# praateekmahajan/moving-mnist-vae

Measured on AMD Instinct MI355X. Metric: frames/sec/GPU VAE train step, 20×64×64 batch; ELBO vs CPU ref, higher is better.
Workload: dtype bf16; 1 GPU; BASELINE configs[1]: 256 clips x 20 frames x 64x64 per GPU per step (=5120 frames), conv-VAE z=128, Gaussian NLL sigma=0.1 + KL (normal_vae_1_kl_0_mmd), Adam, random-init weights, Bernoulli(0.0521) q=2 labels; parallelism=dp1, rccl_ranks=1, grad_exchange=none, bn=per-rank batch statistics

## Files before the change

moving-mnist-vae_amd/csrc/capi.cpp:

```cpp
#include <cstring>
#include <new>

#include "../../include/mmvae.h"
#include "conv_ops.hpp"
#include "pixel_net.hpp"
#include "vae_net.hpp"

namespace mmvae { const char* last_error(); }
using namespace mmvae;

struct mmvae_net { Net* net; };
struct mmvae_comm { Comm* c; };

static inline hipStream_t S(void* s) { return static_cast<hipStream_t>(s); }
static inline hipStream_t S_(void* s) { return static_cast<hipStream_t>(s); }

extern "C" {

int mmvae_abi_version(void) { return MMVAE_ABI_VERSION; }
const char* mmvae_last_error(void) { return last_error(); }

int mmvae_net_create(mmvae_net** out, int in_channels, int z, int out_channels, int image_size, int need_logvar, int dtype) {
  return mmvae_net_create_ex(out, in_channels, z, out_channels, image_size, need_logvar, dtype, 1);
}
// ... 187 lines not shown
  return launch_rsample_fwd(DT_F32, mu, lv, eps, enc, nullptr, (long)n, S(st));
}
int mmvae_rsample_bwd(const float* d_enc, const float* lv, const float* eps, float* d_mu, float* d_lv, int64_t n, void* st) {
  return launch_rsample_bwd(d_enc, lv, eps, d_mu, d_lv, (long)n, S(st));
}
static bool aligned16(const void* p) { return reinterpret_cast<uintptr_t>(p) % 16 == 0; }
int mmvae_kl_fwd_ex(const float* mu, const float* lv, int64_t n, double* acc, double* partials, void* st) {
  if (n > 0 && (!mu || !lv || !acc || !partials)) { set_error("kl_fwd: bad argument"); return MMVAE_ERR_ARG; }
  return launch_kl_fwd(mu, lv, (long)n, acc, partials, S(st));
}
int mmvae_kl_fwd(const float* mu, const float* lv, int64_t n, double* acc, void* st) {
  if (n > 0 && (!mu || !lv || !acc)) { set_error("kl_fwd: bad argument"); return MMVAE_ERR_ARG; }
  return launch_kl_fwd(mu, lv, (long)n, acc, nullptr, S(st));
}
int mmvae_kl_bwd(const float* mu, const float* lv, float coef, const float* gscale, float* d_mu, float* d_lv, int64_t n, void* st) {
  return launch_kl_bwd(mu, lv, coef, gscale, d_mu, d_lv, (long)n, S(st));
}
static int gauss_nll_fwd(const float* r, const float* t, int64_t n, float sigma, double* acc, double* partials, bool need_partials, void* st) {
  if (!(sigma > 0.f)) { set_error("gauss_nll: sigma must be > 0"); return MMVAE_ERR_ARG; }
  if (n > 0 && (!r || !t || !acc || (need_partials && !partials))) { set_error("gauss_nll_fwd: bad argument"); return MMVAE_ERR_ARG; }
  if (n > 0 && (!aligned16(r) || !aligned16(t))) { set_error("gauss_nll_fwd: recon and target must be 16-byte aligned"); return MMVAE_ERR_ARG; }
  return launch_gauss_nll_fwd(r, t, (long)n, sigma, acc, partials, S(st));
}
int mmvae_gauss_nll_fwd_ex(const float* r, const float* t, int64_t n, float sigma, double* acc, double* partials, void* st) {
  return gauss_nll_fwd(r, t, n, sigma, acc, partials, true, st);
}
int mmvae_gauss_nll_fwd(const float* r, const float* t, int64_t n, float sigma, double* acc, void* st) {
  return gauss_nll_fwd(r, t, n, sigma, acc, nullptr, false, st);
}
int mmvae_gauss_nll_bwd(const float* r, const float* t, int64_t n, float sigma, float coef, const float* gscale, float* d_r, void* st) {
  if (!(sigma > 0.f)) { set_error("gauss_nll: sigma must be > 0"); return MMVAE_ERR_ARG; }
  return launch_gauss_nll_bwd(r, t, (long)n, sigma, coef, gscale, d_r, S(st));
}
int mmvae_ce_fwd_ex(const float* r, const int64_t* t, const float* w, int N, int Q, int HW, double* acc, double* partials, void* st) {
  if ((long)N * HW > 0 && (!r || !t || !acc || !partials || Q < 1)) { set_error("ce_fwd: bad argument"); return MMVAE_ERR_ARG; }
  return launch_ce_fwd(r, reinterpret_cast<const long long*>(t), w, N, Q, HW, acc, partials, S(st));
}
int mmvae_ce_fwd(const float* r, const int64_t* t, const float* w, int N, int Q, int HW, double* acc, void* st) {
  if ((long)N * HW > 0 && (!r || !t || !acc || Q < 1)) { set_error("ce_fwd: bad argument"); return MMVAE_ERR_ARG; }
  return launch_ce_fwd(r, reinterpret_cast<const long long*>(t), w, N, Q, HW, acc, nullptr, S(st));
}
int mmvae_ce_bwd(const float* r, const int64_t* t, const float* w, int N, int Q, int HW, float coef, const float* gscale, float* d_r,
                 void* st) {
  return launch_ce_bwd(r, reinterpret_cast<const long long*>(t), w, N, Q, HW, coef, gscale, d_r, S(st));
}
static int mmd_fwd(const float* x, const float* y, int n, int d, float* scratch, double* acc, double* partials, bool need_partials, void* st) {
  if (n > 0 && (!x || !y || !acc || (need_partials && !partials) || d < 1)) { set_error("mmd_fwd: bad argument"); return MMVAE_ERR_ARG; }
  if (n > 0 && scratch && (!aligned16(x) || !aligned16(y))) { set_error("mmd_fwd: x and y must be 16-byte aligned"); return MMVAE_ERR_ARG; }
  return scratch ? launch_mmd_fwd_mfma(x, y, n, d, scratch, acc, partials, S(st)) : launch_mmd_fwd(x, y, n, d, acc, partials, S(st));
}
int mmvae_mmd_fwd_ex(const float* x, const float* y, int n, int d, float* scratch, double* acc, double* partials, void* st) {
  return mmd_fwd(x, y, n, d, scratch, acc, partials, true, st);
}
int mmvae_mmd_fwd(const float* x, const float* y, int n, int d, float* scratch, double* acc, void* st) {
  return mmd_fwd(x, y, n, d, scratch, acc, nullptr, false, st);
}
int mmvae_mmd_bwd(const float* x, const float* y, int n, int d, float coef, const float* gscale, float* d_y, void* st) {
  return launch_mmd_bwd(x, y, n, d, coef, gscale, d_y, S(st));
}
int mmvae_rbf_kernel(const float* x, const float* y, int n, int m, int d, float* out, void* st) {
  if (!x || !y || !out) { set_error("rbf_kernel: bad argument"); return MMVAE_ERR_ARG; }
  return launch_rbf_matrix(x, y, n, m, d, out, S(st));
}
int mmvae_loss_finish(const double* acc, float* out, float nll, float kl_coef, float mmd_coef, float n, void* st) {
  return launch_loss_finish(acc, out, nll, kl_coef, mmd_coef, n, S(st));
}

int mmvae_normalise_labels(const int64_t* labels, int64_t n, float mean, float stdv, float* image, void* st) {
  return launch_normalise(DT_F32, labels, 8, (long)n, mean, stdv, nullptr, image, S(st));
}
int mmvae_quantise_normalise(const uint8_t* frames, int64_t n, const float* centres, int q, float mean, float stdv, int64_t* labels,
                             float* image, void* st) {
  return launch_quantise_normalise(frames, (long)n, centres, q, mean, stdv, reinterpret_cast<long long*>(labels), image, S(st));
}
int mmvae_adam_step(float* p, const float* g, float* m, float* v, int64_t n, float lr, float b1, float b2, float eps, float wd, float bc1,
                    float bc2_sqrt, float grad_scale, void* st) {
  AdamArgs a{p, g, m, v, (long)n, lr, b1, b2, eps, wd, bc1, bc2_sqrt, grad_scale};
  return launch_adam(a, S(st));
}

int mmvae_adam_step_dev(float* p, const float* g, float* m, float* v, int64_t n, float lr, float b1, float b2, float eps, float wd,
                        double* step_dev, float grad_scale, void* st) {
  if (!step_dev) { set_error("adam_step_dev: step counter required"); return MMVAE_ERR_ARG; }
  AdamArgs a{p, g, m, v, (long)n, lr, b1, b2, eps, wd, 1.f, 1.f, grad_scale};
  return launch_adam_dev(a, step_dev, S(st));
}

static inline ConvGeom geom_for(int transposed, int Cin, int Cout, int k, int s, int p) {
  return transposed ? ConvGeom{Cin, Cout, k, s, p} : ConvGeom{Cout, Cin, k, s, p};
}
static inline long numel_w(int Cin, int Cout, int k) { return (long)Cin * Cout * k * k; }
static inline int out_size(int transposed, int H, int k, int s, int p) { return transposed ? (H - 1) * s - 2 * p + k : conv_down_size(H, k, s, p); }

int mmvae_conv2d_fwd(int dt, int transposed, const void* x, const float* w, void* y, int N, int H, int W, int Cin, int Cout, int k,
                     int s, int p, const float* ps, const float* pb, int relu, float* stats, void* scratch, void* st) {
  const ConvGeom g = geom_for(transposed, Cin, Cout, k, s, p);
  const int Ho = out_size(transposed, H, k, s, p), Wo = out_size(transposed, W, k, s, p);
  SecondSrc q;
  if (!transposed && conv3_stream_ok(dt, Cin, Cout, k, s, p, H, W)) {
    if (w) { int rc = op_pack_down(dt, g, w, scratch, S(st)); if (rc < 0) return rc; }
    return launch_conv3_stream(dt, s, x, scratch, nullptr, y, nullptr, ps, pb, relu, stats, nullptr, N, Ho, S(st));
  }
  if (!transposed) {
    q.wfrag = op_deep2_down_ok(dt, g, H, W);
    if (w) { int rc = op_pack_down(dt, g, w, scratch, S(st), 1.f, 0, q.wfrag); if (rc < 0) return rc; }
    return op_run_down(dt, dt, g, scratch, N, x, H, W, y, Ho, Wo, ps, pb, relu, stats, 0, S(st), q);
  }
  if (convT4_stream_ok(dt, Cin, Cout, k, s, p, H, W)) {
    if (w) { int rc = op_pack_up(dt, g, w, scratch, S(st)); if (rc < 0) return rc; }
    return launch_convT4_stream(dt, x, scratch, y, ps, pb, relu, stats, N, H, S(st));
  }
  q.wfrag = op_deep2_up_ok(dt, g, Ho, Wo);
  if (w) { int rc = op_pack_up(dt, g, w, scratch, S(st), 1.f, 0, q.wfrag); if (rc < 0) return rc; }
  return op_run_up(dt, g, scratch, N, x, H, W, y, Ho, Wo, ps, pb, relu, stats, 0, S(st), q);
}
int mmvae_conv2d_dgrad(int dt, int transposed, const void* dy, const float* w, void* dx, int N, int H, int W, int Cin, int Cout, int k,
                       int s, int p, void* scratch, void* st) {
  const ConvGeom g = geom_for(transposed, Cin, Cout, k, s, p);
  const int Ho = out_size(transposed, H, k, s, p), Wo = out_size(transposed, W, k, s, p);
  SecondSrc q;
  if (!transposed && s == 1 && conv3_stream_ok(dt, Cin, Cout, k, s, p, H, W)) {
    PackArgs pf; std::memset(&pf, 0, sizeof(pf));
    pf.src = w; pf.dst = scratch; pf.cols = Cin; pf.K = Cout; pf.ntaps = 9; pf.s_col = 9; pf.s_k = Cin * 9; pf.scale = 1.f;
    for (int t = 0; t < 9; ++t) pf.tap_off[t] = 8 - t;
    int rc = launch_pack(dt, pf, S(st)); if (rc < 0) return rc;
    rc = launch_conv3_stream(dt, 1, dy, scratch, nullptr, dx, nullptr, nullptr, nullptr, 0, nullptr, nullptr, N, H, S(st));
    return rc < 0 ? rc : MMVAE_OK;
  }
  if (!transposed) {
    q.wfrag = op_deep2_up_ok(dt, g, H, W);
    int rc = op_pack_up(dt, g, w, scratch, S(st), 1.f, 0, q.wfrag); if (rc < 0) return rc;
    return op_run_up(dt, g, scratch, N, dy, Ho, Wo, dx, H, W, nullptr, nullptr, 0, nullptr, 0, S(st), q);
  }
  q.wfrag = op_deep2_down_ok(dt, g, Ho, Wo);
  int rc = op_pack_down(dt, g, w, scratch, S(st), 1.f, 0, q.wfrag); if (rc < 0) return rc;
  return op_run_down(dt, dt, g, scratch, N, dy, Ho, Wo, dx, H, W, nullptr, nullptr, 0, nullptr, 0, S(st), q);
}
int mmvae_conv2d_wgrad(int dt, int transposed, const void* x, const void* dy, float* dw, int N, int H, int W, int Cin, int Cout, int k,
                       int s, int p, const float* ps, const float* pb, int relu, void* scratch, void* st) {
  const ConvGeom g = geom_for(transposed, Cin, Cout, k, s, p);
  const int Ho = out_size(transposed, H, k, s, p), Wo = out_size(transposed, W, k, s, p);
  if (!scratch) { set_error("conv2d_wgrad: scratch (MMVAE_WGRAD_SCRATCH_BYTES) required"); return MMVAE_ERR_ARG; }
  static_assert(MMVAE_WGRAD_SCRATCH_BYTES == kWgradScratchBytes, "public scratch size out of sync");
  float* sc = static_cast<float*>(scratch);
  if (!transposed) return op_run_wgrad(dt, g, N, dy, Ho, Wo, nullptr, nullptr, 0, x, H, W, ps, pb, relu, dw, S(st), sc);
  return op_run_wgrad(dt, g, N, x, H, W, ps, pb, relu, dy, Ho, Wo, nullptr, nullptr, 0, dw, S(st), sc);
}
int mmvae_conv2d_wgrad_pair(int dt, const void* x, const void* dy, const void* dy_sc, float* dw, float* dw_sc, int N, int H, int W, int Cin, int Cout,
                            const float* ps, const float* pb, int relu, void* scratch, void* st) {
  if (!scratch || !x || !dy || !dy_sc || !dw || !dw_sc || N < 1) { set_error("conv2d_wgrad_pair: bad argument"); return MMVAE_ERR_ARG; }
  const ConvGeom g = geom_for(0, Cin, Cout, 3, 2, 1), gs = geom_for(0, Cin, Cout, 1, 2, 0);
  const int Ho = out_size(0, H, 3, 2, 1), Wo = out_size(0, W, 3, 2, 1);
  const int rc = op_run_wgrad_pair(dt, g, gs, N, dy, dy_sc, Ho, Wo, x, H, W, ps, pb, relu, dw, dw_sc, S(st), static_cast<float*>(scratch), 1.f, 1.f);
  if (rc == 0) { set_error("conv2d_wgrad_pair: shape not supported (bf16, 32 -> 32 channels, 32x32 -> 16x16)"); return MMVAE_ERR_UNSUPPORTED; }
  return rc < 0 ? rc : MMVAE_OK;
}
int mmvae_convT_bwd_fused(int dt, const void* x, const void* dy, const float* w, float* dw, void* dx, int N, int H, int W, int Cin, int Cout, int k,
                          int s, int p, const float* ps, const float* pb, int relu, const void* x2, const float* w2, float* dw2, void* scratch,
                          void* wscratch, void* st) {
  const ConvGeom g = geom_for(1, Cin, Cout, k, s, p);
  const int Ho = out_size(1, H, k, s, p), Wo = out_size(1, W, k, s, p);
  if (!scratch || !wscratch) { set_error("convT_bwd_fused: scratch buffers required"); return MMVAE_ERR_ARG; }
  if (!op_bwd_fusable(dt, g, N, H, W, Ho, Wo)) { set_error("convT_bwd_fused: shape not supported (bf16, 16 / 32 -> 16 channels, k4 s2 p1, 32x32 -> 64x64 or 16x16 -> 32x32)"); return MMVAE_ERR_UNSUPPORTED; }
  char* sc = static_cast<char*>(scratch);
  int rc = op_pack_down(dt, g, w, sc, S(st)); if (rc < 0) return rc;
  const void* w2p = nullptr;
  if (x2 && w2) {
    PackArgs pa; std::memset(&pa, 0, sizeof(pa));
    pa.src = w2; pa.dst = sc + (size_t)Cin * Cout * k * k * dtype_size(dt); pa.cols = Cin; pa.K = 16; pa.ntaps = 1; pa.s_col = 16; pa.s_k = 1; pa.scale = 1.f; pa.tap_off[0] = 0;
    rc = launch_pack(dt, pa, S(st)); if (rc < 0) return rc;
    w2p = pa.dst;
  }
  if (dw2 && !w2p) { set_error("convT_bwd_fused: dw2 needs x2 and w2"); return MMVAE_ERR_ARG; }
  rc = op_run_bwd_fused(dt, g, N, x, H, W, ps, pb, relu, dy, Ho, Wo, sc, dx, w2p ? x2 : nullptr, w2p, dw, S(st), static_cast<float*>(wscratch), 1.f,
                        nullptr, dw2, 1.f);
  if (rc == 0) { set_error("convT_bwd_fused: not taken"); return MMVAE_ERR_UNSUPPORTED; }
  return rc < 0 ? rc : MMVAE_OK;
}
static_assert(MMVAE_BN_SCRATCH_BYTES >= (1024u * 3 * 512 + 8 * 512) * 4, "BatchNorm scratch: 1024 partial rows x 3 x C<=512 + coefficient rows");
int mmvae_batchnorm_fwd(int dt, const void* y, int64_t npix, int C, const float* gamma, const float* beta, float* rm, float* rv, int64_t* nbt,
                        float momentum, float eps, int relu, void* out, float* save_mean, float* save_istd, void* scratch, void* st) {
  if (!scratch || !save_mean || !save_istd || C < 1 || C > 512 || npix < 1) { set_error("batchnorm_fwd: bad arguments (C <= 512, scratch and save_* required)"); return MMVAE_ERR_ARG; }
  float* part = static_cast<float*>(scratch);
  float* coef = part + 1024L * 3 * 512;
  const int np = launch_chan_stats_nhwc(dt, y, npix, C, part, S(st));
  if (np < 0) return np;
  BnFinalizeArgs f;
  f.partials = part; f.nparts = np; f.C = C; f.count = (double)npix; f.gamma = gamma; f.beta = beta; f.running_mean = rm; f.running_var = rv;
  f.nbt = reinterpret_cast<long long*>(nbt); f.mean = save_mean; f.istd = save_istd; f.scale = coef; f.shift = coef + C; f.momentum = momentum; f.eps = eps;
  int rc = launch_bn_finalize(f, S(st));
  if (rc < 0) return rc;
  return launch_affine_act(dt, y, coef, coef + C, relu, out, npix, C, S(st));
}
int mmvae_batchnorm_bwd(int dt, const void* dout, const void* y, const void* out, int64_t npix, int C, const float* gamma, const float* save_mean,
                        const float* save_istd, void* dy, float* dgamma, float* dbeta, void* scratch, void* st) {
  if (!scratch || C < 1 || C > 512 || npix < 1) { set_error("batchnorm_bwd: bad arguments (C <= 512, scratch required)"); return MMVAE_ERR_ARG; }
  float* part = static_cast<float*>(scratch);
  float* coef = part + 1024L * 3 * 512;
  const int np = launch_bn_bwd_reduce(dt, dout, out, nullptr, nullptr, y, nullptr, npix, C, part, S(st));
  if (np < 0) return np;
  BnBwdFinalizeArgs f; std::memset(&f, 0, sizeof(f));
  f.partials = part; f.nparts = np; f.C = C; f.which = 0; f.ny = 1; f.count = (double)npix; f.gamma = gamma; f.mean = save_mean; f.istd = save_istd;
  f.dgamma = dgamma; f.dbeta = dbeta; f.coefA = coef; f.coefB = coef + C; f.coefC = coef + 2 * C;
  int rc = launch_bn_bwd_finalize(f, S(st));
  if (rc < 0) return rc;
  return launch_bn_bwd_apply(dt, dout, out, nullptr, nullptr, y, coef, coef + C, coef + 2 * C, dy, nullptr, nullptr, nullptr, nullptr, nullptr, npix, C, S(st));
}
int mmvae_stem_fwd(int dt, const void* x, const float* w, void* y, int N, int Sz, float* stats, void* scratch, void* st) {
  if (!scratch || N < 1 || Sz < 9 || Sz > 64) { set_error("stem_fwd: bad arguments"); return MMVAE_ERR_ARG; }
  if (stem_fwd_stream_ok(dt, Sz)) return launch_stem_fwd_stream(dt, x, w, y, stats, N, Sz, S(st));
  const int H1 = (Sz + 4 - 5) / 2 + 1;
  const int cpad = dt == DT_F32 ? 4 : 8;
  PackArgs pa; std::memset(&pa, 0, sizeof(pa));
  pa.src = w; pa.dst = scratch;
  pa.cols = 32; pa.K = cpad; pa.K_valid = 1; pa.ntaps = 25; pa.s_col = 25; pa.s_k = 25; pa.scale = 1.f;
  for (int t = 0; t < 25; ++t) pa.tap_off[t] = t;
  int rc = launch_pack(dt, pa, S(st));
  if (rc < 0) return rc;
  GatherArgs a; std::memset(&a, 0, sizeof(a));
  a.x = x; a.w = scratch; a.y = y; a.stats = stats;
  a.x_planar = 2; a.x_planes = 1;
  a.N = N; a.Hi = Sz; a.Wi = Sz; a.Cin = cpad; a.Ho = H1; a.Wo = H1; a.Cout = 32; a.SI = 2; a.SO = 1;
  a.nphase = 1; a.phases[0] = Phase{0, 0, H1, H1, 25, 0, 0};
  for (int kh = 0; kh < 5; ++kh) for (int kw = 0; kw < 5; ++kw) a.taps[kh * 5 + kw] = Tap{kh - 2, kw - 2};
  return launch_gather_gemm(dt, dt, a, S(st));
}
int mmvae_stem_bwd(int dt, const void* g, const void* y0, const void* x, const float* w, const float* gamma, const float* bn_scale,
                   const float* bn_shift, const float* save_mean, const float* save_istd, float* dw, float* dgamma, float* dbeta, int N, int Sz,
                   void* scratch, void* st) {
  if (!scratch || N < 1) { set_error("stem_bwd: bad arguments"); return MMVAE_ERR_ARG; }
  if (!stem_bwd_fusable(Sz)) { set_error("stem_bwd: image size %d unsupported (64, 32, 16)", Sz); return MMVAE_ERR_UNSUPPORTED; }
  const int H1 = (Sz + 4 - 5) / 2 + 1;
  double* R = static_cast<double*>(scratch);
  float* gram = reinterpret_cast<float*>(R + 1024);
  const long gram_floats = 1024L * stem_bwd_part_floats();
  float* part = gram + gram_floats;
  const long part_floats = (long)(MMVAE_BN_SCRATCH_BYTES - 1024 * 8) / 4 - gram_floats;
  int rc = launch_stem_gram(dt, x, gram, gram_floats, R, N, Sz, H1, H1, S(st));
  if (rc < 0) return rc;
  const int np = launch_stem_bwd(dt, g, y0, x, bn_scale, bn_shift, part, part_floats, N, Sz, H1, H1, S(st));
  if (np < 0) return np;
  return launch_stem_bwd_finalize(part, np, R, w, nullptr, (double)N * H1 * H1, gamma, save_mean, save_istd, dgamma, dbeta, dw, S(st));
}
int mmvae_tail_join_fwd(int dt, const void* y2, const float* s2, const float* b2, const void* ys, const float* ss, const float* bs,
                        const float* w, const float* bias, float* r_raw, float* stats, int N, int H, int W, void* st) {
  return launch_tail_join_fwd(dt, y2, s2, b2, ys, ss, bs, w, bias, r_raw, stats, N, H, W, S(st));
}
int mmvae_tail_join_fwd_stream(int dt, const void* y2, const float* s2, const float* b2, const void* ys, const float* ss, const float* bs,
                               const float* w, const float* bias, float* r_raw, float* stats, int N, int H, int W, void* st) {
  return launch_tail_fwd_stream(dt, y2, s2, b2, ys, ss, bs, w, bias, r_raw, stats, N, H, W, S(st));
}
int mmvae_tail_join_bwd_reduce(int dt, const float* d_raw, const float* w, int oc, const void* y2, const float* s2, const float* b2,
                               const void* ys, const float* ss, const float* bs, float* partials, float* wpartials, int N, int H, int W,
                               void* st) {
  return launch_tail_join_bwd_reduce(dt, d_raw, w, oc, N, H, W, s2, b2, ss, bs, y2, ys, partials, S(st), wpartials);
}
int mmvae_tail_join_bwd_apply(int dt, const float* d_raw, const float* w, int oc, const void* y2, const float* s2, const float* b2,
                              const void* ys, const float* ss, const float* bs, const float* A2, const float* B2, const float* C2,
                              const float* As, const float* Bs, const float* Cs, void* dy2, void* dys, int N, int H, int W, void* st) {
  return launch_tail_join_bwd_apply(dt, d_raw, w, oc, N, H, W, s2, b2, ss, bs, y2, A2, B2, C2, dy2, ys, As, Bs, Cs, dys, S(st));
}
int mmvae_upblock_bwd_fused(const float* d_raw, const float* tw, const void* y2, const float* s2, const float* b2, const void* ys, const float* ss,
                            const float* bs, const float* A2, const float* B2, const float* C2, const float* As, const float* Bs, const float* Cs,
                            const void* y1, const float* s1, const float* b1, const float* w2, float* dw2, void* da1, float* bn1_sums,
                            const void* xin, const float* sx, const float* bx, const float* wu, float* dwu, void* gin, int N, void* scratch, void* st) {
  if (!scratch || !d_raw || !tw || !y2 || !ys || !y1 || !xin || !w2 || !wu || !dw2 || !dwu || !da1 || !gin || !bn1_sums || N < 1 || ((sx != nullptr) != (bx != nullptr))) {
    set_error("upblock_bwd_fused: bad argument"); return MMVAE_ERR_ARG;
  }
  char* sc = static_cast<char*>(scratch);
  const ConvGeom g = geom_for(1, 16, 16, 4, 2, 1);
  int rc = op_pack_down(DT_BF16, g, w2, sc, S(st)); if (rc < 0) return rc;
  rc = op_pack_down(DT_BF16, g, wu, sc + 8192, S(st)); if (rc < 0) return rc;
  float* parts = reinterpret_cast<float*>(sc + 16384);
  JoinBwdLaunch L;
  L.d_raw = d_raw; L.w_tail = tw; L.y2 = y2; L.ys = ys; L.ms2 = s2; L.mb2 = b2; L.mss = ss; L.mbs = bs;
  L.A2 = A2; L.B2 = B2; L.C2 = C2; L.As = As; L.Bs = Bs; L.Cs = Cs;
  L.y1 = y1; L.p1s = s1; L.p1b = b1; L.wd2 = sc; L.da1 = da1; L.part2 = parts; L.bn_part = parts + 2L * 1024 * 4096;
  L.xin = xin; L.pxs = sx; L.pxb = bx; L.wds = sc + 8192; L.gin = gin; L.parts = parts + 1024L * 4096;
  L.N = N;
  const int nb = launch_join_bwd_stream(L, S(st));
  if (nb < 0) return nb;
  for (int k = 0; k < 2; ++k) {
    WgradReduceArgs u; std::memset(&u, 0, sizeof(u));
    u.part = k ? L.parts : L.part2; u.dW = k ? dwu : dw2; u.Ca = 16; u.Cb = 16; u.ntaps = 16; u.nparts = nb;
    u.Ca_valid = 16; u.Cb_valid = 16; u.sA = 16 * 16; u.sB = 16; u.scale = 1.f;
    for (int t = 0; t < 16; ++t) u.tap_off[t] = t;
    rc = launch_wgrad_reduce(u, S(st)); if (rc < 0) return rc;
  }
  return launch_partial_rowsum(L.bn_part, nb, 32, bn1_sums, S(st));
}
int mmvae_upblock_tail_fwd(const void* y1, const float* s1, const float* b1, const float* w2, const void* xin, const float* sx, const float* bx,
                           const float* wu, const float* s2, const float* b2, const float* ss, const float* bs, const float* tw, const float* bias,
                           float* r_raw, float* stats, int N, void* scratch, void* st) {
  if (!scratch || !y1 || !s1 || !b1 || !w2 || !xin || !wu || !s2 || !b2 || !ss || !bs || !tw || !r_raw || N < 1 || ((sx != nullptr) != (bx != nullptr))) {
    set_error("upblock_tail_fwd: bad argument"); return MMVAE_ERR_ARG;
  }
  char* sc = static_cast<char*>(scratch);
  const ConvGeom g = geom_for(1, 16, 16, 4, 2, 1);
  int rc = op_pack_up(DT_BF16, g, w2, sc, S(st)); if (rc < 0) return rc;
  rc = op_pack_up(DT_BF16, g, wu, sc + 8192, S(st)); if (rc < 0) return rc;
  return launch_up5_tail_fwd(y1, s1, b1, sc, xin, sx, bx, sc + 8192, s2, b2, ss, bs, tw, bias, r_raw, stats, N, S(st));
}
int mmvae_conv1x1_bwd_fused(const void* da1, const void* y1, const float* s1, const float* b1, const float* A1, const float* B1, const float* C1,
                            const void* xin, const float* sx, const float* bx, const float* w1, float* dw1, void* gin, int64_t rows, void* scratch,
                            void* st) {
  if (!scratch || !da1 || !y1 || !s1 || !b1 || !A1 || !B1 || !C1 || !xin || !w1 || !dw1 || !gin || rows < 1 || ((sx != nullptr) != (bx != nullptr))) {
    set_error("conv1x1_bwd_fused: bad argument"); return MMVAE_ERR_ARG;
// ... 25 lines not shown
```

moving-mnist-vae_amd/csrc/conv_gemm.hip:

```cpp
#include <stdlib.h>
#include <string.h>

#include <vector>

#include "kernels.hpp"

namespace mmvae {

constexpr int KV = 8;

__device__ __forceinline__ int lds_slot(int row, int kv) { return row * KV + (kv ^ ((row >> 1) & 7)); }

template <typename T> struct Mma;
template <> struct Mma<bf16_t> {
  __device__ static __forceinline__ f32x4 run(const Vec16& a, const Vec16& b, f32x4 c) {
    return __builtin_amdgcn_mfma_f32_16x16x32_bf16(__builtin_bit_cast(bf16x8, a), __builtin_bit_cast(bf16x8, b), c, 0, 0, 0);
  }
};
template <> struct Mma<float> {
  __device__ static __forceinline__ f32x4 run(const Vec16& a, const Vec16& b, f32x4 c) {
#pragma unroll
    for (int j = 0; j < 4; ++j)
      c = __builtin_amdgcn_mfma_f32_16x16x4f32(__uint_as_float(a.w[j]), __uint_as_float(b.w[j]), c, 0, 0, 0);
    return c;
// ... 503 lines not shown
  if (out_dt == DT_F32) return launch_gather_t<bf16_t, float>(a, gx, s);
  return launch_gather_t<bf16_t, bf16_t>(a, gx, s);
}

template <typename T>
__global__ __launch_bounds__(256) void wgrad_kernel(WgradArgs a) {
  constexpr int VE = Elem<T>::kVec;
  constexpr int PK = KV * VE;
  __shared__ Vec16 sP[64 * KV];
  __shared__ Vec16 sG[256 * KV];
  __shared__ int sPix[PK * 3];
  __shared__ float sProP[2 * 256];
  __shared__ float sProG[2 * 256];

  const int t = threadIdx.x, lane = t & 63, wv = t >> 6, g = lane >> 4, r = lane & 15;
  const int TA = a.TA16 * 16, TB = a.TB16 * 16, TG = a.TG;
  const int nb_tiles = (a.Cb + TB - 1) / TB;
  const int a0 = (blockIdx.y / nb_tiles) * TA, b0 = (blockIdx.y % nb_tiles) * TB;
  const int tap0 = blockIdx.z * TG;
  const int tg_n = min(TG, a.ntaps - tap0);
  const T* __restrict__ P = reinterpret_cast<const T*>(a.P);
  const T* __restrict__ G = reinterpret_cast<const T*>(a.G);
  T* sPe = reinterpret_cast<T*>(sP);
  T* sGe = reinterpret_cast<T*>(sG);
  const bool proP = a.proP_scale != nullptr, proG = a.proG_scale != nullptr;
  if (proP) for (int i = t; i < TA; i += 256) {
    const bool ok = a0 + i < a.Ca;
    sProP[i] = ok ? a.proP_scale[a0 + i] : 0.f; sProP[256 + i] = ok ? a.proP_shift[a0 + i] : 0.f;
  }
  if (proG) for (int i = t; i < TB; i += 256) {
    const bool ok = b0 + i < a.Cb;
    sProG[i] = ok ? a.proG_scale[b0 + i] : 0.f; sProG[256 + i] = ok ? a.proG_shift[b0 + i] : 0.f;
  }

  const int units = a.TA16 * a.TB16 * tg_n;
  f32x4 acc[16];
  int rowA[16], rowB[16];
#pragma unroll
  for (int i = 0; i < 16; ++i) {
    acc[i] = (f32x4){0, 0, 0, 0};
    const int u = wv + 4 * i;
    const int tg = u % tg_n, q = u / tg_n;
    const int tb = q % a.TB16, ta = q / a.TB16;
    rowA[i] = 16 * ta + r;
    rowB[i] = tg * TB + 16 * tb + r;
  }

  const long m_begin = (long)blockIdx.x * a.pix_per_block;
  const long m_end = min((long)a.M, m_begin + a.pix_per_block);
  const int HpWp = a.Hp * a.Wp;
  const int pvecs = TA / VE, gvecs = TB / VE;

  for (long m0 = m_begin; m0 < m_end; m0 += PK) {
    __syncthreads();
    if (t < PK) {
      const long m = m0 + t;
      if (m < m_end) {
        const int n = (int)(m / HpWp), rem = (int)(m - (long)n * HpWp);
        const int hp = rem / a.Wp, wp = rem - hp * a.Wp;
        sPix[3 * t] = n * a.Hg * a.Wg;
        sPix[3 * t + 1] = hp * a.stride - a.pad;
        sPix[3 * t + 2] = wp * a.stride - a.pad;
      } else {
        sPix[3 * t] = -1; sPix[3 * t + 1] = 0; sPix[3 * t + 2] = 0;
      }
    }
    __syncthreads();
    for (int v = t; v < PK * pvecs; v += 256) {
      const int pk = v / pvecs, cv = v - pk * pvecs;
      const int ch = cv * VE;
      float f[VE];
      const bool ok = (m0 + pk) < m_end && (a0 + ch) < a.Ca;
      if (ok) {
        const Vec16 q = *reinterpret_cast<const Vec16*>(P + ((m0 + pk) * a.Ca + a0 + ch));
        Elem<T>::unpack(q, f);
        if (proP) {
#pragma unroll
          for (int j = 0; j < VE; ++j) {
            float x = f[j] * sProP[ch + j] + sProP[256 + ch + j];
            f[j] = a.proP_relu ? fmaxf(x, 0.f) : x;
          }
        }
      } else {
#pragma unroll
        for (int j = 0; j < VE; ++j) f[j] = 0.f;
      }
#pragma unroll
      for (int j = 0; j < VE; ++j) {
        const int row = ch + j;
        Elem<T>::store(sPe + (long)lds_slot(row, pk / VE) * VE + (pk % VE), f[j]);
      }
    }
    for (int v = t; v < tg_n * PK * gvecs; v += 256) {
      const int tg = v / (PK * gvecs), rem = v - tg * (PK * gvecs);
      const int pk = rem / gvecs, cv = rem - pk * gvecs;
      const int ch = cv * VE;
      const int tap = tap0 + tg, kh = tap / a.ksz, kw = tap - kh * a.ksz;
      const int base = sPix[3 * pk], hg = sPix[3 * pk + 1] + kh, wg = sPix[3 * pk + 2] + kw;
      const bool ok = base >= 0 && hg >= 0 && hg < a.Hg && wg >= 0 && wg < a.Wg && (b0 + ch) < a.Cb;
      float f[VE];
      if (ok) {
        const Vec16 q = *reinterpret_cast<const Vec16*>(G + ((long)(base + hg * a.Wg + wg) * a.Cb + b0 + ch));
        Elem<T>::unpack(q, f);
        if (proG) {
#pragma unroll
          for (int j = 0; j < VE; ++j) {
            float x = f[j] * sProG[ch + j] + sProG[256 + ch + j];
            f[j] = a.proG_relu ? fmaxf(x, 0.f) : x;
          }
        }
      } else {
#pragma unroll
        for (int j = 0; j < VE; ++j) f[j] = 0.f;
      }
#pragma unroll
      for (int j = 0; j < VE; ++j) {
        const int row = tg * TB + ch + j;
        Elem<T>::store(sGe + (long)lds_slot(row, pk / VE) * VE + (pk % VE), f[j]);
      }
    }
    __syncthreads();
#pragma unroll
    for (int i = 0; i < 16; ++i) {
      const int u = wv + 4 * i;
      if (u < units) {
#pragma unroll
        for (int k2 = 0; k2 < 2; ++k2) {
          const int kvs = 4 * k2 + g;
          const Vec16 af = sP[lds_slot(rowA[i], kvs)];
          const Vec16 bf = sG[lds_slot(rowB[i], kvs)];
          acc[i] = Mma<T>::run(af, bf, acc[i]);
        }
      }
    }
  }
#pragma unroll
  for (int i = 0; i < 16; ++i) {
    const int u = wv + 4 * i;
    if (u < units) {
      const int tg = u % tg_n, q = u / tg_n;
      const int tb = q % a.TB16, ta = q / a.TB16;
      const int bb = b0 + 16 * tb + r;
      if (bb < a.Cb_valid) {
#pragma unroll
        for (int j = 0; j < 4; ++j) {
          const int aa = a0 + 16 * ta + 4 * g + j;
          if (aa < a.Ca) a.scratch[(((long)blockIdx.x * a.ntaps + tap0 + tg) * a.Ca + aa) * a.Cb + bb] = acc[i][j];
        }
      }
    }
  }
}

static int try_wgrad2(int dt, const WgradArgs& a, hipStream_t s) {
  if (a.Ca % 16 || a.Cb % 16 || a.ntaps > 25) return 0;
  if (a.proP_scale && a.proG_scale) return 0;
  if (a.P_planar && (a.Ca != 16 || a.P_planes > 16 || a.proP_scale)) return 0;
  auto pick = [](int c) { return c >= 64 ? 64 : c; };
  int TA = pick(a.Ca), TB = pick(a.Cb);
  if (!(TA == 16 || TA == 32 || TA == 64) || !(TB == 16 || TB == 32 || TB == 64)) return 0;
  if (a.Ca % TA || a.Cb % TB) return 0;
  if (a.ntaps < 4 && TB == 64 && !a.P_planar) {
    Wgrad2Args probe; memset(&probe, 0, sizeof(probe));
    probe.TG = wgrad2_taps_per_block(TA / 16, 4, a.ntaps); probe.nw = 4;
    if (make_tile_geom(probe.g, a.N, a.Hp, a.Wp, a.Hg, a.Wg, a.stride, -a.pad, -a.pad, a.ksz, a.ksz, 128, 1) &&
        (wgrad2_lds_bytes(probe, dt, TA, 64) > kV2MaxLds || wgrad2_patch_slots(probe, dt, 64) > 16)) TB = 32;
  }
  const int ta16 = TA / 16, tb16 = TB / 16;
  Wgrad2Args b; memset(&b, 0, sizeof(b));
  b.P = a.P; b.G = a.G;
  b.proP_scale = a.proP_scale; b.proP_shift = a.proP_shift; b.proP_relu = a.proP_relu;
  b.proG_scale = a.proG_scale; b.proG_shift = a.proG_shift; b.proG_relu = a.proG_relu;
  b.TG = wgrad2_taps_per_block(ta16, tb16, a.ntaps);
  b.nw = 4;
  if (!a.P_planar && ta16 >= 2 && tb16 >= 2 && (a.ntaps == 9 || a.ntaps == 16) && b.TG < a.ntaps &&
      !(a.ntaps == 16 && ta16 * tb16 >= 16)) {
    b.nw = a.ntaps; b.TG = a.ntaps;
  } else if (!a.P_planar && a.ntaps == 16 && ta16 == 4 && tb16 == 4) {
    b.nw = 8; b.TG = 16;
  }
  bool fits = false;
  size_t lds = 0;
  for (int TP = 128; TP >= 32 && !fits; TP >>= 1) {
    if (TP < 128 && a.ntaps < 4) break;
    if (!make_tile_geom(b.g, a.N, a.Hp, a.Wp, a.Hg, a.Wg, a.stride, -a.pad, -a.pad, a.ksz, a.ksz, TP, 1)) continue;
    lds = wgrad2_lds_bytes(b, dt, TA, TB);
    fits = lds <= kV2MaxLds && wgrad2_patch_slots(b, dt, TB) <= (b.nw == 4 ? 16 : 8);
  }
  if (!fits) return 0;
  b.Ca = a.Ca; b.Cb = a.Cb; b.Cb_valid = a.Cb_valid; b.Ca_valid = a.Ca_valid; b.ksz = a.ksz; b.ntaps = a.ntaps;
  b.sA = a.sA; b.sB = a.sB; b.scale = a.scale; b.P_planar = a.P_planar; b.P_planes = a.P_planes;
  for (int t = 0; t < 25; ++t) b.tap_off[t] = a.tap_off[t];
  const int tiles_ab = (a.Ca / TA) * (a.Cb / TB);
  const int zg = (a.ntaps + b.TG - 1) / b.TG;
  const long wsize = (long)a.Ca * a.Cb * a.ntaps;
  const long op_bytes = ((long)a.N * a.Hp * a.Wp * a.Ca + (long)a.N * a.Hg * a.Wg * a.Cb) * (long)dtype_size(dt);
  int occ = (int)((160 * 1024) / lds); if (occ > 6) occ = 6; if (occ < 1) occ = 1;
  long gx = (op_bytes < (200L << 20) ? 176L : 256L * occ) / ((long)tiles_ab * zg); if (gx < 1) gx = 1;
  if (!a.scratch) { set_error("wgrad: the partial-image scratch is required (no atomic flush path)"); return MMVAE_ERR_ARG; }
  {
    long budget = op_bytes > (8L << 20) ? op_bytes : (8L << 20);
    if (budget > (long)kWgradScratchBytes) budget = (long)kWgradScratchBytes;
    const long cap = budget / (wsize * 4);
    if (cap < 1) return 0;
    if (gx > cap) gx = cap;
  }
  if (gx > b.g.ntiles) gx = b.g.ntiles;
  if (gx >= 8) gx &= ~7L;
  b.dW = a.scratch; b.partial = 1;
  const int rc = launch_wgrad2(dt, b, (int)gx, tiles_ab, zg, ta16, tb16, s);
  if (rc < 0) return rc;
  WgradReduceArgs u; memset(&u, 0, sizeof(u));
  u.part = a.scratch; u.dW = a.dW; u.Ca = a.Ca; u.Cb = a.Cb; u.ntaps = a.ntaps; u.nparts = (int)gx;
  u.Ca_valid = a.Ca_valid; u.Cb_valid = a.Cb_valid; u.sA = a.sA; u.sB = a.sB; u.scale = a.scale;
  for (int t = 0; t < 25; ++t) u.tap_off[t] = a.tap_off[t];
  const int rc2 = launch_wgrad_reduce(u, s);
  return rc2 < 0 ? rc2 : 1;
}

#define MM_CHECK_RC(expr) do { const int rc__ = (expr); if (rc__ < 0) return rc__; } while (0)
int launch_wgrad(int dt, WgradArgs a, hipStream_t s) {
  const int VE = dt == DT_F32 ? 4 : 8;
  if (a.Ca % VE != 0 || a.Cb % VE != 0 || a.ntaps > 25 || a.ntaps < 1) {
    set_error("wgrad: unsupported Ca=%d Cb=%d ntaps=%d", a.Ca, a.Cb, a.ntaps);
    return MMVAE_ERR_UNSUPPORTED;
  }
  a.M = a.N * a.Hp * a.Wp;
  note_launch_bytes((double)a.N * ((double)a.Hp * a.Wp * (a.P_planar ? a.P_planes * 4.0 : a.Ca * (double)dtype_size(dt)) +
                                   (double)a.Hg * a.Wg * a.Cb * (double)dtype_size(dt)));
  if (a.Cb_valid <= 0 || a.Cb_valid > a.Cb) a.Cb_valid = a.Cb;
  if (a.Ca_valid <= 0 || a.Ca_valid > a.Ca) a.Ca_valid = a.Ca;
  if (a.M <= 0) return MMVAE_OK;
  {
    const int rcs = try_wgrad_stream(dt, a, s);
    if (rcs != 0) return rcs < 0 ? rcs : MMVAE_OK;
    const int rcp = try_wgrad_pos(dt, a, s);
    if (rcp != 0) return rcp < 0 ? rcp : MMVAE_OK;
    const int rc2 = try_wgrad2(dt, a, s);
    if (rc2 != 0) return rc2 < 0 ? rc2 : MMVAE_OK;
    if (a.P_planar) { set_error("wgrad: planar operands need the patch-tile kernel"); return MMVAE_ERR_UNSUPPORTED; }
  }
  const int TA = a.Ca >= 64 ? 64 : ((a.Ca + 15) / 16) * 16;
  const int TB = a.Cb >= 64 ? 64 : ((a.Cb + 15) / 16) * 16;
  a.TA16 = TA / 16; a.TB16 = TB / 16;
  int tg = 256 / TB;
  const int max_units_tg = 64 / (a.TA16 * a.TB16);
  if (tg > max_units_tg) tg = max_units_tg;
  if (tg > a.ntaps) tg = a.ntaps;
  if (tg < 1) tg = 1;
  a.TG = tg;
  const int tiles = ((a.Ca + TA - 1) / TA) * ((a.Cb + TB - 1) / TB);
  const int zg = (a.ntaps + tg - 1) / tg;
  const int PK = KV * VE;
  const long ksteps = ((long)a.M + PK - 1) / PK;
  long want = 1024 / ((long)tiles * zg);
  const long wsize = (long)a.Ca * a.Cb * a.ntaps;
  if (!a.scratch) { set_error("wgrad: the partial-image scratch is required (no atomic flush path)"); return MMVAE_ERR_ARG; }
  {
    long cap = (long)(kWgradScratchBytes / 4) / (wsize > 0 ? wsize : 1);
    const long cap2 = (16L << 20) / (wsize > 0 ? wsize : 1);
    if (cap > cap2 && cap2 >= 8) cap = cap2;
    if (cap < 1) { set_error("wgrad: one partial image (%ld floats) exceeds the scratch", wsize); return MMVAE_ERR_UNSUPPORTED; }
    if (want > cap) want = cap;
  }
  if (want < 1) want = 1;
  if (want > ksteps) want = ksteps;
  long steps_per = (ksteps + want - 1) / want;
  a.pix_per_block = (int)(steps_per * PK);
  const int gx = (int)(((long)a.M + a.pix_per_block - 1) / a.pix_per_block);
  dim3 grid(gx, tiles, zg), block(256);
  if (dt == DT_F32) hipLaunchKernelGGL((wgrad_kernel<float>), grid, block, 0, s, a);
  else hipLaunchKernelGGL((wgrad_kernel<bf16_t>), grid, block, 0, s, a);
  MM_CHECK_RC(check_launch("wgrad"));
  WgradReduceArgs u; memset(&u, 0, sizeof(u));
  u.part = a.scratch; u.dW = a.dW; u.Ca = a.Ca; u.Cb = a.Cb; u.ntaps = a.ntaps; u.nparts = gx;
  u.Ca_valid = a.Ca_valid; u.Cb_valid = a.Cb_valid; u.sA = a.sA; u.sB = a.sB; u.scale = a.scale;
  for (int t = 0; t < 25; ++t) u.tap_off[t] = a.tap_off[t];
  return launch_wgrad_reduce(u, s);
}

template <typename T>
__device__ __forceinline__ long frag_index(int col, int kk, int Ktot) {
  constexpr int VE = Elem<T>::kVec, CK = 4 * VE;
  const int chunk = kk / CK, in = kk - chunk * CK;
  const int q = col & 31;
  const int blk = 2 * (col >> 5) + ((q >> 2) & 1), r = 4 * (q >> 3) + (q & 3);
  return (((long)blk * (Ktot / CK) + chunk) * 64 + (in / VE) * 16 + r) * VE + (in % VE);
}
__device__ __forceinline__ long frag_index_f8(int col, int kk, int Ktot) {
  const int chunk = kk >> 6, in = kk & 63, half = in >> 5, w = in & 31;
  const int q = col & 31;
  const int blk = 2 * (col >> 5) + ((q >> 2) & 1), r = 4 * (q >> 3) + (q & 3);
  return (((long)blk * (Ktot >> 6) + chunk) * 64 + (w >> 3) * 16 + r) * 16 + half * 8 + (w & 7);
}
template <typename T>
__global__ void pack_kernel(PackArgs a) {
  const long total = (long)a.cols * a.ntaps * a.K;
  for (long i = (long)blockIdx.x * blockDim.x + threadIdx.x; i < total; i += (long)gridDim.x * blockDim.x) {
    const int k = (int)(i % a.K);
    const long q = i / a.K;
    const int tp = (int)(q % a.ntaps);
    const int col = (int)(q / a.ntaps);
    const bool real = (a.cols_valid <= 0 || col < a.cols_valid) && (a.K_valid <= 0 || k < a.K_valid);
    const float v = real ? a.src[(long)col * a.s_col + (long)k * a.s_k + a.tap_off[tp]] * a.scale : 0.f;
    Elem<T>::store(reinterpret_cast<T*>(a.dst) + (a.frag ? frag_index<T>(col, tp * a.K + k, a.ntaps * a.K) : i), v);
  }
}

struct PackJob {
  const float* src; void* dst; int cols, K, ntaps, s_col, s_k, cols_valid, K_valid; float scale; unsigned char tap_off[26]; unsigned char frag; unsigned char fp8;
};
__device__ __forceinline__ unsigned char f32_to_e4m3(float v) {
  v = fminf(fmaxf(v, -448.f), 448.f);
  return (unsigned char)(__builtin_amdgcn_cvt_pk_fp8_f32(v, 0.f, 0, false) & 0xff);
}
constexpr int kPackJobsPerLaunch = 48;
struct PackMulti { int njobs; int pad; PackJob jobs[kPackJobsPerLaunch]; };

template <typename T>
__global__ void pack_multi_kernel(PackMulti m) {
  const PackJob& a = m.jobs[blockIdx.y];
  const long total = (long)a.cols * a.ntaps * a.K;
  for (long i = (long)blockIdx.x * blockDim.x + threadIdx.x; i < total; i += (long)gridDim.x * blockDim.x) {
    const int k = (int)(i % a.K);
    const long q = i / a.K;
    const int tp = (int)(q % a.ntaps);
    const int col = (int)(q / a.ntaps);
    const bool real = (a.cols_valid <= 0 || col < a.cols_valid) && (a.K_valid <= 0 || k < a.K_valid);
    const float v = real ? a.src[(long)col * a.s_col + (long)k * a.s_k + a.tap_off[tp]] * a.scale : 0.f;
    if (a.fp8) reinterpret_cast<unsigned char*>(a.dst)[a.frag ? frag_index_f8(col, tp * a.K + k, a.ntaps * a.K) : i] = f32_to_e4m3(v);
    else Elem<T>::store(reinterpret_cast<T*>(a.dst) + (a.frag ? frag_index<T>(col, tp * a.K + k, a.ntaps * a.K) : i), v);
  }
}

static thread_local bool g_pack_batching = false;
static thread_local int g_pack_n = 0;
static thread_local std::vector<PackJob> g_pack_jobs;

void pack_batch_begin() { g_pack_batching = true; g_pack_n = 0; }

int pack_batch_flush(int dt, hipStream_t s) {
  g_pack_batching = false;
  for (int j0 = 0; j0 < g_pack_n; j0 += kPackJobsPerLaunch) {
    PackMulti m; m.njobs = g_pack_n - j0 < kPackJobsPerLaunch ? g_pack_n - j0 : kPackJobsPerLaunch; m.pad = 0;
    for (int j = 0; j < m.njobs; ++j) m.jobs[j] = g_pack_jobs[j0 + j];
    dim3 grid(128, m.njobs), block(256);
    if (dt == DT_F32) hipLaunchKernelGGL((pack_multi_kernel<float>), grid, block, 0, s, m);
    else hipLaunchKernelGGL((pack_multi_kernel<bf16_t>), grid, block, 0, s, m);
    int rc = check_launch("pack_multi");
    if (rc) { g_pack_n = 0; return rc; }
  }
  g_pack_n = 0;
  return MMVAE_OK;
}

int launch_pack(int dt, const PackArgs& a, hipStream_t s) {
  const long total = (long)a.cols * a.ntaps * a.K;
  if (total <= 0) return MMVAE_OK;
  if (g_pack_batching) {
    if (a.ntaps > 26) { set_error("pack: %d taps > 26", a.ntaps); return MMVAE_ERR_ARG; }
    if ((size_t)g_pack_n >= g_pack_jobs.size()) g_pack_jobs.resize(g_pack_jobs.size() + 256);
    PackJob& j = g_pack_jobs[g_pack_n++];
    j.src = a.src; j.dst = a.dst; j.cols = a.cols; j.K = a.K; j.ntaps = a.ntaps; j.s_col = a.s_col; j.s_k = a.s_k;
    j.cols_valid = a.cols_valid; j.K_valid = a.K_valid; j.scale = a.scale; j.fp8 = (unsigned char)(a.fp8 ? 1 : 0); j.frag = (unsigned char)(a.frag ? 1 : 0);
    for (int t = 0; t < a.ntaps; ++t) j.tap_off[t] = (unsigned char)a.tap_off[t];
    return MMVAE_OK;
  }
  if (a.fp8) { set_error("pack: fp8 packing is available in batched mode only"); return MMVAE_ERR_UNSUPPORTED; }
  int blocks = (int)((total + 255) / 256);
  if (blocks > 2048) blocks = 2048;
// ... 7 lines not shown
```

moving-mnist-vae_amd/csrc/conv_ops.cpp:

```cpp
#include "conv_ops.hpp"

#include <cstdlib>
#include <cstring>

namespace mmvae {

#define MM_TRY(expr)            \
  do {                          \
    int rc__ = (expr);          \
    if (rc__ < 0) return rc__;  \
  } while (0)

struct UpPhase { int ph, pw; int ntaps; int kh[16], kw[16], dh[16], dw[16]; };
static int up_phases(int k, int s, int p, UpPhase* out) {
  int n = 0;
  for (int ph = 0; ph < s; ++ph)
    for (int pw = 0; pw < s; ++pw) {
      UpPhase& u = out[n++];
      u.ph = ph; u.pw = pw; u.ntaps = 0;
      for (int kh = 0; kh < k; ++kh) {
        const int th = ph + p - kh;
        if (((th % s) + s) % s != 0) continue;
        for (int kw = 0; kw < k; ++kw) {
          const int tw = pw + p - kw;
          if (((tw % s) + s) % s != 0) continue;
          u.kh[u.ntaps] = kh; u.kw[u.ntaps] = kw;
          u.dh[u.ntaps] = th / s; u.dw[u.ntaps] = tw / s;
          ++u.ntaps;
        }
      }
    }
  return n;
}


int op_pack_down(int dt, const ConvGeom& g, const float* w, void* dst, hipStream_t s, float scale, int fp8, int frag) {
  PackArgs a; std::memset(&a, 0, sizeof(a));
  const int kk = g.k * g.k;
  if (kk > kMaxTaps) { set_error("pack_down: k=%d too large", g.k); return MMVAE_ERR_UNSUPPORTED; }
  a.src = w; a.dst = dst;
  a.cols = g.D0; a.K = g.D1; a.ntaps = kk; a.s_col = g.D1 * kk; a.s_k = kk; a.scale = scale; a.fp8 = fp8; a.frag = frag;
  for (int t = 0; t < kk; ++t) a.tap_off[t] = t;
  return launch_pack(dt, a, s);
}

int op_pack_up(int dt, const ConvGeom& g, const float* w, void* dst, hipStream_t s, float scale, int fp8, int frag) {
  if (g.s > 2 || g.k * g.k > kMaxTaps) { set_error("pack_up: k=%d s=%d unsupported", g.k, g.s); return MMVAE_ERR_UNSUPPORTED; }
  UpPhase ph[4];
  const int np = up_phases(g.k, g.s, g.p, ph);
  const int kk = g.k * g.k;
  const long e = fp8 ? 1 : (long)dtype_size(dt);
  long off = 0;
  for (int i = 0; i < np; ++i) {
    if (ph[i].ntaps == 0) continue;
    PackArgs a; std::memset(&a, 0, sizeof(a));
    a.src = w; a.dst = static_cast<char*>(dst) + off * e;
    a.cols = g.D1; a.K = g.D0; a.ntaps = ph[i].ntaps; a.s_col = kk; a.s_k = g.D1 * kk; a.scale = scale; a.fp8 = fp8; a.frag = frag;
    for (int t = 0; t < ph[i].ntaps; ++t) a.tap_off[t] = ph[i].kh[t] * g.k + ph[i].kw[t];
    MM_TRY(launch_pack(dt, a, s));
    off += (long)g.D1 * ph[i].ntaps * g.D0;
  }
  return MMVAE_OK;
}

int op_deep2_down_ok(int dt, const ConvGeom& g, int Hl, int Wl, int fp8) {
  const int Hs = conv_down_size(Hl, g.k, g.s, g.p), Ws = conv_down_size(Wl, g.k, g.s, g.p);
  return deep2_shape_ok(dt, g.D1, g.D0, Hs, Ws, Hl, Wl, g.k * g.k, fp8) ? 1 : 0;
}
int op_deep2_up_ok(int dt, const ConvGeom& g, int Hl, int Wl, int allow_empty_phases, int fp8) {
  if (g.s > 2 || g.k * g.k > kMaxTaps) return 0;
  const int Hs = conv_down_size(Hl, g.k, g.s, g.p), Ws = conv_down_size(Wl, g.k, g.s, g.p);
  UpPhase ph[4];
  const int np = up_phases(g.k, g.s, g.p, ph);
  int ntaps = 0;
  for (int i = 0; i < np; ++i) { if (ph[i].ntaps == 0 && !allow_empty_phases) return 0; ntaps += ph[i].ntaps; }
  return deep2_shape_ok(dt, g.D0, g.D1, (Hl + g.s - 1) / g.s, (Wl + g.s - 1) / g.s, Hs, Ws, ntaps, fp8) ? 1 : 0;
}
bool op_pos_fwd_takes(const ConvGeom& g, int Hl, bool transposed) {
  const int Hs = conv_down_size(Hl, g.k, g.s, g.p);
  const int Hi = transposed ? Hs : Hl, Ho = transposed ? Hl : Hs;
  const int Cin = transposed ? g.D0 : g.D1, Cout = transposed ? g.D1 : g.D0;
  if (Cout % 32 != 0 || Cin % 8 != 0 || (Hi >= 8 && Cout < 128)) return false;
  if (transposed && g.s > 1 && g.k < g.s) return false;
  const int nw = Cout / 32 < 8 ? Cout / 32 : 8;
  if ((Cout / 32) % nw != 0 || (64 * nw) % (Cin / 8) != 0) return false;
  return pos_conv_takes(g.k, g.s, g.p, transposed ? 1 : 0, Hi, Ho, Cin);
}

int op_run_down(int dt, int out_dt, const ConvGeom& g, const void* packed, int N, const void* L, int Hl, int Wl, void* S, int Hs, int Ws,
                const float* pro_s, const float* pro_b, int relu, float* stats, int accumulate, hipStream_t s, const SecondSrc& x2) {
  GatherArgs a; std::memset(&a, 0, sizeof(a));
  if (g.k * g.k > kMaxTaps) { set_error("run_down: k=%d too large", g.k); return MMVAE_ERR_UNSUPPORTED; }
  if (x2.x2) { a.x2 = x2.x2; a.w2 = x2.w2; a.Cin2 = x2.Cin2; a.x2_ph = 0; a.x2_pw = 0; }
  a.fp8 = x2.fp8; a.wfrag = x2.wfrag; a.wfrag2 = x2.wfrag2;
  a.x = L; a.w = packed; a.y = S;
  a.pro_scale = pro_s; a.pro_shift = pro_b; a.pro_relu = relu; a.stats = stats; a.accumulate = accumulate;
  a.N = N; a.Hi = Hl; a.Wi = Wl; a.Cin = g.D1; a.Ho = Hs; a.Wo = Ws; a.Cout = g.D0; a.SI = g.s; a.SO = 1;
  a.gk = g.k; a.gs = g.s; a.gp = g.p; a.gup = 1;
  a.nphase = 1;
  a.phases[0] = Phase{0, 0, Hs, Ws, g.k * g.k, 0, 0};
  for (int kh = 0; kh < g.k; ++kh)
    for (int kw = 0; kw < g.k; ++kw) a.taps[kh * g.k + kw] = Tap{kh - g.p, kw - g.p};
  return launch_gather_gemm(dt, out_dt, a, s);
}

int op_run_up(int dt, const ConvGeom& g, const void* packed, int N, const void* S, int Hs, int Ws, void* L, int Hl, int Wl,
              const float* pro_s, const float* pro_b, int relu, float* stats, int accumulate, hipStream_t s, const SecondSrc& x2) {
  if (g.s > 2 || g.k * g.k > kMaxTaps) { set_error("run_up: k=%d s=%d unsupported", g.k, g.s); return MMVAE_ERR_UNSUPPORTED; }
  GatherArgs a; std::memset(&a, 0, sizeof(a));
  if (x2.x2) { a.x2 = x2.x2; a.w2 = x2.w2; a.Cin2 = x2.Cin2; a.x2_ph = 0; a.x2_pw = 0; }
  a.fp8 = x2.fp8; a.wfrag = x2.wfrag; a.wfrag2 = x2.wfrag2;
  a.x = S; a.w = packed; a.y = L;
  a.pro_scale = pro_s; a.pro_shift = pro_b; a.pro_relu = relu; a.stats = stats; a.accumulate = accumulate;
  a.N = N; a.Hi = Hs; a.Wi = Ws; a.Cin = g.D0; a.Ho = Hl; a.Wo = Wl; a.Cout = g.D1; a.SI = 1; a.SO = g.s;
  a.gk = g.k; a.gs = g.s; a.gp = g.p; a.gup = 2;
  UpPhase ph[4];
  const int np = up_phases(g.k, g.s, g.p, ph);
  long off = 0; int tap0 = 0; a.nphase = 0;
  for (int i = 0; i < np; ++i) {
    const int Hq = Hl > ph[i].ph ? (Hl - ph[i].ph + g.s - 1) / g.s : 0;
    const int Wq = Wl > ph[i].pw ? (Wl - ph[i].pw + g.s - 1) / g.s : 0;
    const bool skip = (ph[i].ntaps == 0 && accumulate) || Hq == 0 || Wq == 0;
    if (!skip) {
      a.phases[a.nphase++] = Phase{ph[i].ph, ph[i].pw, Hq, Wq, ph[i].ntaps, tap0, off};
      for (int t = 0; t < ph[i].ntaps; ++t) a.taps[tap0 + t] = Tap{ph[i].dh[t], ph[i].dw[t]};
      tap0 += ph[i].ntaps;
    }
    off += (long)g.D1 * ph[i].ntaps * g.D0;
  }
  if (a.nphase == 0) return 1;
  return launch_gather_gemm(dt, dt, a, s);
}

int op_run_wgrad(int dt, const ConvGeom& g, int N, const void* P, int Hs, int Ws, const float* proP_s, const float* proP_b, int proP_relu,
                 const void* G, int Hl, int Wl, const float* proG_s, const float* proG_b, int proG_relu, float* dW, hipStream_t s,
                 float* scratch, float scale, WgradReduceArgs* defer) {
  WgradArgs a; std::memset(&a, 0, sizeof(a));
  const int kk = g.k * g.k;
  if (kk > 25) { set_error("wgrad: k=%d too large", g.k); return MMVAE_ERR_UNSUPPORTED; }
  if (defer) defer->nparts = 0;
  a.P = P; a.G = G; a.dW = dW; a.scratch = scratch; a.defer = defer;
  a.proP_scale = proP_s; a.proP_shift = proP_b; a.proP_relu = proP_relu;
  a.proG_scale = proG_s; a.proG_shift = proG_b; a.proG_relu = proG_relu;
  a.N = N; a.Hp = Hs; a.Wp = Ws; a.Ca = g.D0; a.Hg = Hl; a.Wg = Wl; a.Cb = g.D1; a.Cb_valid = g.D1;
  a.stride = g.s; a.pad = g.p; a.ksz = g.k; a.sA = g.D1 * kk; a.sB = kk; a.ntaps = kk; a.scale = scale;
  for (int t = 0; t < kk; ++t) a.tap_off[t] = t;
  return launch_wgrad(dt, a, s);
}

static void wgrad_args(WgradArgs& a, const ConvGeom& g, int N, const void* P, int Hs, int Ws, const float* proP_s, const float* proP_b, int proP_relu,
                       const void* G, int Hl, int Wl, const float* proG_s, const float* proG_b, int proG_relu, float* dW, float* scratch, float scale) {
  std::memset(&a, 0, sizeof(a));
  const int kk = g.k * g.k;
  a.P = P; a.G = G; a.dW = dW; a.scratch = scratch;
  a.proP_scale = proP_s; a.proP_shift = proP_b; a.proP_relu = proP_relu;
  a.proG_scale = proG_s; a.proG_shift = proG_b; a.proG_relu = proG_relu;
  a.N = N; a.Hp = Hs; a.Wp = Ws; a.Ca = g.D0; a.Hg = Hl; a.Wg = Wl; a.Cb = g.D1; a.Cb_valid = g.D1; a.Ca_valid = g.D0;
  a.stride = g.s; a.pad = g.p; a.ksz = g.k; a.sA = g.D1 * kk; a.sB = kk; a.ntaps = kk; a.scale = scale;
  for (int t = 0; t < kk && t < 25; ++t) a.tap_off[t] = t;
}

int op_run_wgrad_pair(int dt, const ConvGeom& g, const ConvGeom& gs, int N, const void* P, const void* P2, int Hs, int Ws, const void* G, int Hl, int Wl,
                      const float* proG_s, const float* proG_b, int proG_relu, float* dW, float* dW2, hipStream_t s, float* scratch, float scale,
                      float scale2) {
  if (g.k != 3 || g.p != 1 || gs.k != 1 || gs.p != 0 || gs.s != g.s || gs.D0 != g.D0 || gs.D1 != g.D1) return 0;
  WgradArgs a;
  wgrad_args(a, g, N, P, Hs, Ws, nullptr, nullptr, 0, G, Hl, Wl, proG_s, proG_b, proG_relu, dW, scratch, scale);
  return try_wgrad_stream_pair(dt, a, P2, dW2, scale2, s);
}

bool op_wgrad_is_stream(int dt, const ConvGeom& g, int N, int Hs, int Ws, int Hl, int Wl, bool proP, bool proG) {
  if (g.k * g.k > 25) return false;
  WgradArgs a;
  float dummy = 0.f;
  wgrad_args(a, g, N, nullptr, Hs, Ws, proP ? &dummy : nullptr, proP ? &dummy : nullptr, 1, nullptr, Hl, Wl, proG ? &dummy : nullptr, proG ? &dummy : nullptr, 1,
             nullptr, &dummy, 1.f);
  return wgrad_stream_shape(dt, a);
}

bool op_bwd_fusable(int dt, const ConvGeom& g, int N, int Hs, int Ws, int Hl, int Wl) {
  if (g.k * g.k > 25) return false;
  WgradArgs a;
  float dummy = 0.f;
  wgrad_args(a, g, N, nullptr, Hs, Ws, nullptr, nullptr, 0, nullptr, Hl, Wl, nullptr, nullptr, 0, nullptr, &dummy, 1.f);
  return dgrad_wgrad_stream_shape(dt, a);
}

int op_run_bwd_fused(int dt, const ConvGeom& g, int N, const void* P, int Hs, int Ws, const float* proP_s, const float* proP_b, int proP_relu,
                     const void* G, int Hl, int Wl, const void* packed_down, void* dP, const void* x2, const void* w2_packed, float* dW,
                     hipStream_t s, float* scratch, float scale, float* bn_part, float* dW2, float scale2, const JoinGrad* jg) {
  if (g.k * g.k > 25) return 0;
  WgradArgs a;
  wgrad_args(a, g, N, P, Hs, Ws, proP_s, proP_b, proP_relu, G, Hl, Wl, nullptr, nullptr, 0, dW, scratch, scale);
  a.M = a.N * a.Hp * a.Wp;
  return try_dgrad_wgrad_stream(dt, a, packed_down, dP, x2, w2_packed, bn_part, s, dW2, scale2, jg);
}

bool op_bwd_fusable_jg(int dt, const ConvGeom& g, int N, int Hs, int Ws, int Hl, int Wl, bool proP, bool has_x2, bool bn_sums) {
  if (g.k * g.k > 25) return false;
  WgradArgs a;
  float dummy = 0.f;
  wgrad_args(a, g, N, nullptr, Hs, Ws, proP ? &dummy : nullptr, proP ? &dummy : nullptr, 1, nullptr, Hl, Wl, nullptr, nullptr, 0, nullptr, &dummy, 1.f);
  return dgrad_wgrad_stream_jg_shape(dt, a, has_x2, bn_sums);
}

}
```

moving-mnist-vae_amd/csrc/conv_wgrad.hip:

```cpp
#include <cstdlib>
#include "kernels.hpp"

namespace mmvae {

int launch_wgrad2_bf16(const Wgrad2Args& a, dim3 grid, int ta16, int tb16, int maxg, hipStream_t s);
int launch_wgrad2_f32(const Wgrad2Args& a, dim3 grid, int ta16, int tb16, int maxg, hipStream_t s);

int wgrad2_taps_per_block(int ta16, int tb16, int ntaps) {
  int mt = 12 / (ta16 * tb16); if (mt < 1) mt = 1; if (mt > 4) mt = 4;
  const int tg = ntaps >= 4 ? 4 * mt : mt;
  return tg < ntaps ? tg : ntaps;
}

size_t wgrad2_lds_bytes(const Wgrad2Args& a, int dt, int TA, int TB) {
  const size_t es = dtype_size(dt);
  const size_t stage = (size_t)a.g.TP * TA * es + (size_t)a.g.segs * a.g.PR * a.g.PW * TB * es + 32 * 4;
  const size_t acc1 = (size_t)TA * TB * 4;
  return stage > acc1 ? stage : acc1;
}

int wgrad2_patch_slots(const Wgrad2Args& a, int dt, int TB) {
  const int cvg = TB * (int)dtype_size(dt) / 16;
  const int nt = 64 * (a.nw > 0 ? a.nw : 4);
  const int per_round = nt / cvg;
  const int npatch = a.g.segs * a.g.PR * a.g.PW;
  return (npatch + per_round - 1) / per_round;
}

int launch_wgrad2(int dt, const Wgrad2Args& a, int gx, int tiles_ab, int zg, int ta16, int tb16, hipStream_t s) {
  dim3 grid(gx, tiles_ab, zg);
  const int slots = wgrad2_patch_slots(a, dt, tb16 * 16);
  if (slots > 16) { set_error("wgrad2: %d staging slots > 16", slots); return MMVAE_ERR_UNSUPPORTED; }
  return dt == DT_F32 ? launch_wgrad2_f32(a, grid, ta16, tb16, slots, s) : launch_wgrad2_bf16(a, grid, ta16, tb16, slots, s);
}

template <int LANES>
__global__ __launch_bounds__(256) void wgrad_reduce_kernel(WgradReduceArgs a) {
  constexpr int RG = 256 / LANES;
  __shared__ float4 sSum[256];
  const int ab = a.Ca * a.Cb;
  const long wsize = a.part_stride;
  const int l = threadIdx.x % LANES, rg = threadIdx.x / LANES;
  const float* src = a.part + (long)blockIdx.x * (4 * LANES) + l * 4;
  float4 s[4];
#pragma unroll
  for (int k = 0; k < 4; ++k) s[k] = make_float4(0.f, 0.f, 0.f, 0.f);
  int p = rg;
  for (; p + 3 * RG < a.nparts; p += 4 * RG) {
#pragma unroll
    for (int k = 0; k < 4; ++k) {
      const float4 v = *reinterpret_cast<const float4*>(src + (long)(p + k * RG) * wsize);
      s[k].x += v.x; s[k].y += v.y; s[k].z += v.z; s[k].w += v.w;
    }
  }
  for (; p < a.nparts; p += RG) {
    const float4 v = *reinterpret_cast<const float4*>(src + (long)p * wsize);
    s[0].x += v.x; s[0].y += v.y; s[0].z += v.z; s[0].w += v.w;
  }
  sSum[threadIdx.x] = make_float4((s[0].x + s[1].x) + (s[2].x + s[3].x), (s[0].y + s[1].y) + (s[2].y + s[3].y),
                                  (s[0].z + s[1].z) + (s[2].z + s[3].z), (s[0].w + s[1].w) + (s[2].w + s[3].w));
  __syncthreads();
#pragma unroll
  for (int st = RG / 2; st >= 1; st >>= 1) {
    if (rg < st) {
      const float4 o = sSum[threadIdx.x + st * LANES];
      float4& m = sSum[threadIdx.x];
      m.x += o.x; m.y += o.y; m.z += o.z; m.w += o.w;
    }
    __syncthreads();
  }
  if (rg == 0) {
    const float4 m = sSum[l];
    const float v[4] = {m.x, m.y, m.z, m.w};
#pragma unroll
    for (int j = 0; j < 4; ++j) {
      const long i = (long)blockIdx.x * (4 * LANES) + l * 4 + j;
      const int t = (int)(i / ab), rem = (int)(i - (long)t * ab);
      const int aa = rem / a.Cb, bb = rem - aa * a.Cb;
      if (aa < a.Ca_valid && bb < a.Cb_valid) a.dW[(long)aa * a.sA + (long)bb * a.sB + a.tap_off[t]] += v[j] * a.scale;
    }
  }
}

int launch_wgrad_reduce(WgradReduceArgs a, hipStream_t s) {
  if (a.nparts < 1) return MMVAE_OK;
  bool distinct = true;
  for (int t = 0; t < a.ntaps && distinct; ++t)
    for (int u = 0; u < t; ++u) if (a.tap_off[u] == a.tap_off[t]) { distinct = false; break; }
  if (a.part_stride <= 0) a.part_stride = (long)a.ntaps * a.Ca * a.Cb;
  if (!distinct) {
    for (int t = 1; t < a.ntaps; ++t)
      if (a.tap_off[t] != a.tap_off[0]) { set_error("wgrad_reduce: taps share some destinations but not all"); return MMVAE_ERR_UNSUPPORTED; }
    if (a.part_stride != (long)a.ntaps * a.Ca * a.Cb) { set_error("wgrad_reduce: shared destinations need densely packed partial images"); return MMVAE_ERR_UNSUPPORTED; }
    a.nparts *= a.ntaps; a.ntaps = 1; a.part_stride = (long)a.Ca * a.Cb;
  }
  const long wsize = (long)a.ntaps * a.Ca * a.Cb;
  if (wsize % 256) { set_error("wgrad_reduce: %ld elements not a multiple of 256", wsize); return MMVAE_ERR_ARG; }
  a.exclusive = 1;
  note_launch_bytes((double)a.nparts * a.part_stride * 4.0);
  int lanes = 64;
  while (lanes > 8 && wsize / (4 * lanes) < 256) lanes >>= 1;
  const dim3 grid((unsigned)(wsize / (4 * lanes)));
  switch (lanes) {
    case 64: hipLaunchKernelGGL(wgrad_reduce_kernel<64>, grid, dim3(256), 0, s, a); break;
    case 32: hipLaunchKernelGGL(wgrad_reduce_kernel<32>, grid, dim3(256), 0, s, a); break;
    case 16: hipLaunchKernelGGL(wgrad_reduce_kernel<16>, grid, dim3(256), 0, s, a); break;
    default: hipLaunchKernelGGL(wgrad_reduce_kernel<8>, grid, dim3(256), 0, s, a); break;
  }
  return check_launch("wgrad_reduce");
}

int launch_patch_conv_f32(const PatchArgs& a, int gx, hipStream_t s);
int launch_patch_conv_bf16(const PatchArgs& a, int gx, hipStream_t s);
int launch_patch_conv_bf16_f32(const PatchArgs& a, int gx, hipStream_t s);

size_t patch_conv_lds_bytes(const PatchArgs& a, int dt) {
  const int VE = dt == DT_F32 ? 4 : 8;
  const int cin_vecs = a.Cin / VE;
  int ct16 = (a.Cout + 15) / 16; if (ct16 == 3) ct16 = 4;
  size_t b = (size_t)a.w_vecs * 16 + (size_t)a.g.segs * a.g.PR * a.g.PW * cin_vecs * 16 + (size_t)a.koff_total * 4 + (size_t)8 * ct16 * 16 * 4 +
             (a.uni ? (size_t)4 * a.out_wave_bytes : 0);
  b = (b + 15) & ~(size_t)15;
  if (a.x2) b += (size_t)ct16 * 16 * (a.kvp2 + 1) * 16 + ((size_t)a.g.segs * a.g.qr * a.g.Wq * (a.Cin2 / VE) + 8) * 16;
  return b;
}
void patch_conv_x2_carve(PatchArgs& a, int dt) {
  PatchArgs z = a; z.x2 = nullptr;
  const size_t base = patch_conv_lds_bytes(z, dt);
  int ct16 = (a.Cout + 15) / 16; if (ct16 == 3) ct16 = 4;
  a.w2_vec0 = (int)(base / 16);
  a.x2_vec0 = a.w2_vec0 + ct16 * 16 * (a.kvp2 + 1);
}

int patch_conv_slots(const PatchArgs& a, int dt) {
  const int VE = dt == DT_F32 ? 4 : 8;
  const int npatch = a.g.segs * a.g.PR * a.g.PW;
  const int per_round = a.x_planar ? 256 : 256 / (a.Cin / VE);
  return (npatch + per_round - 1) / per_round;
}

int launch_patch_conv(int dt, int out_dt, const PatchArgs& a, int gx, hipStream_t s) {
  if (dt == DT_F32) return launch_patch_conv_f32(a, gx, s);
  if (out_dt == DT_F32) return launch_patch_conv_bf16_f32(a, gx, s);
  return launch_patch_conv_bf16(a, gx, s);
}

int launch_deep2_conv_f32(const DeepArgs& a, int gx, hipStream_t s);
int launch_deep2_conv_bf16(const DeepArgs& a, int gx, hipStream_t s);
int launch_deep2_conv_bf16_f32(const DeepArgs& a, int gx, hipStream_t s);

size_t deep2_conv_lds_bytes(const DeepArgs& a, int dt) {
  const size_t pitch = a.fp8 ? (size_t)a.Cin + 16 : (size_t)a.Cin * dtype_size(dt) + 32;
  return (size_t)(a.ipt * a.Hi * a.Wi + 1) * pitch + (size_t)a.npt * 16 * 4 + (size_t)a.nw * 64 * 4 + (size_t)a.ntaps_all * a.npt * 16 * 2;
}

int launch_deep2_conv(int dt, int out_dt, const DeepArgs& a, int gx, hipStream_t s) {
  if (dt == DT_F32) return launch_deep2_conv_f32(a, gx, s);
  if (out_dt == DT_F32) return launch_deep2_conv_bf16_f32(a, gx, s);
  return launch_deep2_conv_bf16(a, gx, s);
}

}
```

moving-mnist-vae_amd/csrc/conv_wgrad.inc:

```

namespace mmvae {

template <int TA16, int TB16> struct Wgrad2Cfg {
  static constexpr int kUnits = TA16 * TB16;
  static constexpr int kMaxT = (12 / kUnits) < 1 ? 1 : ((12 / kUnits) > 4 ? 4 : (12 / kUnits));
};

constexpr int kSlotInvalid = 0x40000000;

template <typename T, int VE>
__device__ __forceinline__ Vec16 apply_pro(const Vec16& q, const float* sc, const float* sh, int relu) {
  float f[VE];
  Elem<T>::unpack(q, f);
#pragma unroll
  for (int j = 0; j < VE; ++j) {
    const float x = f[j] * sc[j] + sh[j];
    f[j] = relu ? fmaxf(x, 0.f) : x;
  }
  return Elem<T>::pack(f);
}

template <typename T, int TA16, int TB16, bool TS, int MAXG, bool PPL, int NW = 4>
__global__ __launch_bounds__(64 * NW, NW == 16 ? 4 : (NW == 9 ? 3 : (NW == 8 ? 2 : (MAXG <= 8 ? 3 : 2) - (TA16 * TB16 > 2 ? 1 : 0)))) void wgrad2_kernel(Wgrad2Args a) {
  static_assert(NW == 4 || TS, "one-tap-per-wave blocks are tap-split");
  constexpr int NT = 64 * NW;
  constexpr int VE = Elem<T>::kVec;
  constexpr int ES = sizeof(T);
  constexpr int TA = TA16 * 16, TB = TB16 * 16;
  constexpr int MAXT = NW > 4 ? (NW == 8 ? 2 : 1) : Wgrad2Cfg<TA16, TB16>::kMaxT;
  constexpr int NKS = TS ? 4 : 1;
  constexpr int CVG = TB / VE, PSG = NT / CVG;
  constexpr int CVP = TA / VE, PSP = NT / CVP;
  constexpr int MAXP = (128 + PSP - 1) / PSP;
  extern __shared__ __attribute__((aligned(16))) char smem[];
  const TileGeom g = a.g;
  const int t = threadIdx.x, lane = t & 63, wv = t >> 6, gq = lane >> 4, r = lane & 15;
  const int nb_tiles = a.Cb / TB;
  const int a0 = (blockIdx.y / nb_tiles) * TA, b0 = (blockIdx.y % nb_tiles) * TB;
  const int tap0 = blockIdx.z * a.TG;
  const int tg_n = min(a.TG, a.ntaps - tap0);
  const int npatch = g.segs * g.PR * g.PW;
  char* sP = smem;
  char* sG = sP + g.TP * TA * ES;
  int* sToff = reinterpret_cast<int*>(sG + npatch * TB * ES);
  const T* __restrict__ Pp = reinterpret_cast<const T*>(a.P);
  const T* __restrict__ Gp = reinterpret_cast<const T*>(a.G);
  const bool proP = a.proP_scale != nullptr, proG = a.proG_scale != nullptr;
  const bool multi = g.tiles_per_img == 0;
  if (t < tg_n) {
    const int tap = tap0 + t, kh = tap / a.ksz, kw = tap - kh * a.ksz;
    sToff[t] = (kh * g.PW + kw) * TB * ES;
  }
  const int cvp = t % CVP, pp0 = t / CVP, cvg = t % CVG, gp0 = t / CVG;
  float xsc[VE], xsh[VE];
#pragma unroll
  for (int j = 0; j < VE; ++j) {
    xsc[j] = proP ? a.proP_scale[a0 + cvp * VE + j] : (proG ? a.proG_scale[b0 + cvg * VE + j] : 1.f);
    xsh[j] = proP ? a.proP_shift[a0 + cvp * VE + j] : (proG ? a.proG_shift[b0 + cvg * VE + j] : 0.f);
  }
  int goff[MAXG], gchk[MAXG];
#pragma unroll
  for (int k = 0; k < MAXG; ++k) {
    const int pp = gp0 + k * PSG;
    goff[k] = 0; gchk[k] = kSlotInvalid;
    if (pp < npatch) {
      const int row = pp / g.PW, pc = pp - row * g.PW;
      const int seg = row / g.PR, pr = row - seg * g.PR;
      const int wi = g.ow + pc;
      bool ok = wi >= 0 && wi < g.Wi;
      if (multi) ok = ok && g.oh + pr >= 0 && g.oh + pr < g.Hi;
      goff[k] = ((seg * g.Hi + pr) * g.Wi + wi) * a.Cb + b0 + cvg * VE;
      if (ok) gchk[k] = multi ? seg : pr;
    }
  }
  const unsigned lim = multi ? g.N : g.Hi;
  f32x4 acc[MAXT][TA16][TB16];
#pragma unroll
  for (int tl = 0; tl < MAXT; ++tl)
#pragma unroll
    for (int ta = 0; ta < TA16; ++ta)
#pragma unroll
      for (int tb = 0; tb < TB16; ++tb) acc[tl][ta][tb] = (f32x4){0, 0, 0, 0};
  const int npix_tile = g.segs * g.qr * g.Wq;
  int offP[NKS][2], offG[NKS][2];
  if constexpr (sizeof(T) == 2) {
#pragma unroll
    for (int i = 0; i < NKS; ++i)
#pragma unroll
      for (int b = 0; b < 2; ++b) {
        int p = 32 * (TS ? i : wv) + 16 * b + 4 * gq + (r >> 2);
        offP[i][b] = p * TA * ES + (r & 3) * 8;
        if (p >= npix_tile) p = 0;
        offG[i][b] = patch_index(g, p) * TB * ES + (r & 3) * 8;
      }
  }
  int my_tap[MAXT];
#pragma unroll
  for (int tl = 0; tl < MAXT; ++tl) my_tap[tl] = TS ? wv + NW * tl : tl;

  Vec16 gv[MAXG], pv[MAXP];
  int tb_c = 0, nv_c = 0;
  long m0_c = 0;
  const long pplane = (long)g.Hq * g.Wq;
  auto issue = [&](int tile) {
    int n, hq0;
    tile_origin(g, tile, 0, n, hq0);
    const long m0 = ((long)n * g.Hq + hq0) * g.Wq;
    const long mend = !multi ? ((long)n * g.Hq + min(g.Hq, hq0 + g.qr)) * g.Wq : (long)min(g.N, n + g.segs) * g.Hq * g.Wq;
    nv_c = (int)(mend - m0);
    const int h_base = hq0 * g.SI + g.oh;
    tb_c = multi ? n : h_base;
    const T* gsrc = Gp + ((long)n * g.Hi + h_base) * g.Wi * a.Cb;
#pragma unroll
    for (int k = 0; k < MAXG; ++k) {
      gv[k] = Vec16{{0, 0, 0, 0}};
      if ((unsigned)(tb_c + gchk[k]) < lim) gv[k] = *reinterpret_cast<const Vec16*>(gsrc + goff[k]);
    }
    if constexpr (!PPL) {
      const T* psrc = Pp + m0 * a.Ca + a0 + cvp * VE;
#pragma unroll
      for (int k = 0; k < MAXP; ++k) {
        const int pix = pp0 + k * PSP;
        pv[k] = Vec16{{0, 0, 0, 0}};
        if (pix < nv_c) pv[k] = *reinterpret_cast<const Vec16*>(psrc + (long)pix * a.Ca);
      }
    } else {
      m0_c = m0;
#pragma unroll
      for (int k = 0; k < MAXP; ++k) {
        const int pix = pp0 + k * PSP;
        pv[k] = Vec16{{0, 0, 0, 0}};
        if (pix < nv_c && cvp == 0 && a.P_planes <= 2) {
          long nn = n, rem = (long)hq0 * g.Wq + pix;
          if (multi) { const long m = m0 + pix; nn = m / pplane; rem = m - nn * pplane; }
          const float* src = reinterpret_cast<const float*>(a.P) + nn * a.P_planes * pplane + rem;
          pv[k].w[0] = __float_as_uint(src[0]);
          if (a.P_planes > 1) pv[k].w[1] = __float_as_uint(src[pplane]);
        }
      }
    }
  };
  auto commit = [&]() {
#pragma unroll
    for (int k = 0; k < MAXG; ++k) {
      const int pp = gp0 + k * PSG;
      if (pp < npatch) {
        Vec16 q = gv[k];
        if (proG && (unsigned)(tb_c + gchk[k]) < lim) q = apply_pro<T, VE>(q, xsc, xsh, a.proG_relu);
        reinterpret_cast<Vec16*>(sG)[pp * CVG + cvg] = q;
      }
    }
#pragma unroll
    for (int k = 0; k < MAXP; ++k) {
      const int pix = pp0 + k * PSP;
      if (pix < g.TP) {
        Vec16 q = pv[k];
        if constexpr (PPL) {
          float f[VE];
#pragma unroll
          for (int j = 0; j < VE; ++j) f[j] = 0.f;
          if (pix < nv_c && cvp * VE < a.P_planes) {
            if (a.P_planes <= 2) { f[0] = __uint_as_float(q.w[0]); f[1] = __uint_as_float(q.w[1]); }
            else {
              const long m = m0_c + pix, nn = m / pplane, rem = m - nn * pplane;
              const float* src = reinterpret_cast<const float*>(a.P) + nn * a.P_planes * pplane + rem;
#pragma unroll
              for (int j = 0; j < VE; ++j) if (cvp * VE + j < a.P_planes) f[j] = src[(long)(cvp * VE + j) * pplane];
            }
          }
          q = Elem<T>::pack(f);
        } else { if (proP && pix < nv_c) q = apply_pro<T, VE>(q, xsc, xsh, a.proP_relu); }
        reinterpret_cast<Vec16*>(sP)[pix * CVP + cvp] = q;
      }
    }
  };

  const int nks_tile = g.TP >> 5;
#pragma unroll
  for (int j = 0; j < VE; ++j) {
    asm volatile("" ::"v"(xsc[j])); asm volatile("" ::"v"(xsh[j]));
  }
  const TileWalk walk = xcd_tile_walk(g.ntiles);
  int tile = walk.first;
  if (tile < walk.end) issue(tile);
  for (; tile < walk.end; tile += walk.step) {
    __syncthreads();
    commit();
    __syncthreads();
    if (tile + walk.step < walk.end) issue(tile + walk.step);
    if constexpr (sizeof(T) == 2) {
#pragma unroll
      for (int i = 0; i < NKS; ++i) {
        if (TS && i >= nks_tile) break;
        Vec16 af[TA16];
#pragma unroll
        for (int ta = 0; ta < TA16; ++ta) af[ta] = FragOps<bf16_t>::load(sP, offP[i][0] + ta * 32, offP[i][1] + ta * 32);
#pragma unroll
        for (int tl = 0; tl < MAXT; ++tl) {
          if (my_tap[tl] < tg_n) {
            const int toff = sToff[my_tap[tl]];
#pragma unroll
            for (int tb = 0; tb < TB16; ++tb) {
              const Vec16 bf = FragOps<bf16_t>::load(sG, offG[i][0] + toff + tb * 32, offG[i][1] + toff + tb * 32);
#pragma unroll
              for (int ta = 0; ta < TA16; ++ta) acc[tl][ta][tb] = mma_bf16(af[ta], bf, acc[tl][ta][tb]);
            }
          }
        }
      }
    } else {
      for (int i = 0; i < NKS; ++i) {
        if (TS && i >= nks_tile) break;
        const int ks = TS ? i : wv;
        for (int j = 0; j < 8; ++j) {
          int p = 32 * ks + 4 * j + gq;
          const int oP = p * TA * ES + r * 4;
          if (p >= npix_tile) p = 0;
          const int oG = patch_index(g, p) * TB * ES + r * 4;
          float av[TA16];
#pragma unroll
          for (int ta = 0; ta < TA16; ++ta) av[ta] = *reinterpret_cast<const float*>(sP + oP + ta * 64);
#pragma unroll
          for (int tl = 0; tl < MAXT; ++tl) {
            if (my_tap[tl] < tg_n) {
              const int toff = sToff[my_tap[tl]];
#pragma unroll
              for (int tb = 0; tb < TB16; ++tb) {
                const float bv = *reinterpret_cast<const float*>(sG + oG + toff + tb * 64);
#pragma unroll
                for (int ta = 0; ta < TA16; ++ta)
                  acc[tl][ta][tb] = __builtin_amdgcn_mfma_f32_16x16x4f32(av[ta], bv, acc[tl][ta][tb], 0, 0, 0);
              }
            }
          }
        }
      }
    }
  }
  if (TS && a.partial) {
#pragma unroll
    for (int tl = 0; tl < MAXT; ++tl) {
      if (my_tap[tl] < tg_n) {
        float* dst = a.dW + (((long)blockIdx.x * a.ntaps + tap0 + my_tap[tl]) * a.Ca + a0) * a.Cb + b0;
#pragma unroll
        for (int ta = 0; ta < TA16; ++ta)
#pragma unroll
          for (int tb = 0; tb < TB16; ++tb)
#pragma unroll
            for (int jj = 0; jj < 4; ++jj) dst[(long)(16 * ta + 4 * gq + jj) * a.Cb + 16 * tb + r] = acc[tl][ta][tb][jj];
      }
    }
    return;
  }
  __syncthreads();
  float* sAcc = reinterpret_cast<float*>(smem);
#pragma unroll
  for (int tl = 0; tl < MAXT; ++tl) {
    for (int w = 0; w < (TS ? NW : 1); ++w) {
      const int tap_l = TS ? w + NW * tl : tl;
      if (tap_l >= tg_n) continue;
      for (int src = 0; src < (TS ? 1 : NW); ++src) {
        if (TS ? (wv == w) : (wv == src)) {
#pragma unroll
          for (int ta = 0; ta < TA16; ++ta)
#pragma unroll
            for (int tb = 0; tb < TB16; ++tb)
#pragma unroll
              for (int jj = 0; jj < 4; ++jj) {
                float* q = &sAcc[(16 * ta + 4 * gq + jj) * TB + 16 * tb + r];
                *q = (src == 0 ? 0.f : *q) + acc[tl][ta][tb][jj];
              }
        }
        __syncthreads();
      }
      float* dst = a.dW + (((long)blockIdx.x * a.ntaps + tap0 + tap_l) * a.Ca + a0) * a.Cb + b0;
      for (int i = t; i < TA * TB; i += NT) dst[(long)(i / TB) * a.Cb + (i % TB)] = sAcc[i];
      __syncthreads();
    }
  }
}

template <typename T>
static int launch_wgrad2_t(Wgrad2Args a, int dt, dim3 grid, int ta16, int tb16, int maxg, hipStream_t s) {
  const size_t lds = wgrad2_lds_bytes(a, dt, ta16 * 16, tb16 * 16);
  dim3 block(64 * a.nw);
  const bool ts = a.ntaps >= 4;
  if (a.nw != 4) {
    if (a.nw == 8) {
      if (ta16 != 4 || tb16 != 4 || a.P_planar || !ts || maxg > 8) { set_error("wgrad2: nw=8 needs the 64x64 tile"); return MMVAE_ERR_UNSUPPORTED; }
      if (maxg <= 4) hipLaunchKernelGGL((wgrad2_kernel<T, 4, 4, true, 4, false, 8>), grid, block, lds, s, a);
      else hipLaunchKernelGGL((wgrad2_kernel<T, 4, 4, true, 8, false, 8>), grid, block, lds, s, a);
      return check_launch("wgrad2");
    }
    if (a.P_planar || !ts || maxg > 8 || (a.nw != 9 && a.nw != 16)) { set_error("wgrad2: nw=%d unsupported here", a.nw); return MMVAE_ERR_UNSUPPORTED; }
#define MMVAE_W2N(A_, B_) do { \
    if (a.nw == 9) { if (maxg <= 4) hipLaunchKernelGGL((wgrad2_kernel<T, A_, B_, true, 4, false, 9>), grid, block, lds, s, a); \
                     else hipLaunchKernelGGL((wgrad2_kernel<T, A_, B_, true, 8, false, 9>), grid, block, lds, s, a); } \
    else { if (maxg <= 4) hipLaunchKernelGGL((wgrad2_kernel<T, A_, B_, true, 4, false, 16>), grid, block, lds, s, a); \
           else hipLaunchKernelGGL((wgrad2_kernel<T, A_, B_, true, 8, false, 16>), grid, block, lds, s, a); } } while (0)
    if (ta16 == 4 && tb16 == 4) MMVAE_W2N(4, 4);
    else if (ta16 == 4 && tb16 == 2) MMVAE_W2N(4, 2);
    else if (ta16 == 2 && tb16 == 4) MMVAE_W2N(2, 4);
    else if (ta16 == 2 && tb16 == 2) MMVAE_W2N(2, 2);
    else { set_error("wgrad2: tile %dx%d unsupported with nw=%d", ta16, tb16, a.nw); return MMVAE_ERR_UNSUPPORTED; }
#undef MMVAE_W2N
    return check_launch("wgrad2");
  }
#define MMVAE_W2G(A_, B_, G_) do { if (ts) hipLaunchKernelGGL((wgrad2_kernel<T, A_, B_, true, G_, false>), grid, block, lds, s, a); \
                                   else hipLaunchKernelGGL((wgrad2_kernel<T, A_, B_, false, G_, false>), grid, block, lds, s, a); } while (0)
#define MMVAE_W2(A_, B_) do { if (maxg <= 8) MMVAE_W2G(A_, B_, 8); else MMVAE_W2G(A_, B_, 16); } while (0)
  if (a.P_planar) {
    if (ta16 != 1 || tb16 != 1 || !ts) { set_error("wgrad2: planar P needs the 16x16 tap-split tile"); return MMVAE_ERR_UNSUPPORTED; }
    if (maxg <= 8) hipLaunchKernelGGL((wgrad2_kernel<T, 1, 1, true, 8, true>), grid, block, lds, s, a);
    else hipLaunchKernelGGL((wgrad2_kernel<T, 1, 1, true, 16, true>), grid, block, lds, s, a);
  } else if (ta16 == 1 && tb16 == 1) MMVAE_W2(1, 1);
  else if (ta16 == 1 && tb16 == 2) MMVAE_W2(1, 2);
  else if (ta16 == 2 && tb16 == 1) MMVAE_W2(2, 1);
  else if (ta16 == 2 && tb16 == 2) MMVAE_W2(2, 2);
  else if (ta16 == 4 && tb16 == 2) MMVAE_W2(4, 2);
  else if (ta16 == 2 && tb16 == 4) MMVAE_W2(2, 4);
  else if (ta16 == 4 && tb16 == 4) MMVAE_W2(4, 4);
  else if (ta16 == 4 && tb16 == 1) MMVAE_W2(4, 1);
  else if (ta16 == 1 && tb16 == 4) MMVAE_W2(1, 4);
  else { set_error("wgrad2: tile %dx%d unsupported", ta16, tb16); return MMVAE_ERR_UNSUPPORTED; }
#undef MMVAE_W2
#undef MMVAE_W2G
  return check_launch("wgrad2");
}

}
```

moving-mnist-vae_amd/csrc/conv_wpos.hip:

```cpp
#include <cstdlib>
#include <cstring>

#include "kernels.hpp"
#include "tile_common.hpp"

namespace mmvae {

typedef __attribute__((ext_vector_type(16))) float f32x16;

struct WposArgs {
  const void* P; const void* G; float* part;
  const float* proP_scale; const float* proP_shift; int proP_relu;
  const float* proG_scale; const float* proG_shift; int proG_relu;
  int N, Ca, Cb, HS, HL, K, S, Pd;
  int nsplit, imgs_per_split;
  int nb, prow, grow;
};

template <int KI, int NTHR, int kMaxV, int NFB>
__global__ __launch_bounds__(NTHR, 1) void wgrad_pos_kernel(WposArgs a) {
  extern __shared__ __attribute__((aligned(16))) char smem[];
  constexpr int nthr = NTHR;
  constexpr int TB = 32 * NFB, PXG = TB * 2, VG = TB / 8;
  const int t = threadIdx.x, lane = t & 63, wv = __builtin_amdgcn_readfirstlane(t >> 6);
  const int npos = a.HS * a.HS, npix = a.HL * a.HL;
  const int nPb = a.prow * a.HS, nGb = a.grow * a.HL;
  const int ipP = ((nPb * 128 + 191) & ~255) + 64, ipG = ((nGb * PXG + 191) & ~255) + 64;
  const int stageB = KI * (ipP + ipG);
  const int tiles_b = a.Cb / TB;
  const int a0 = (blockIdx.y / tiles_b) << 6, b0 = (blockIdx.y % tiles_b) * TB;
  const int n_begin = blockIdx.x * a.imgs_per_split;
  const int n_end = min(a.N, n_begin + a.imgs_per_split);
  const bf16_t* __restrict__ Pp = reinterpret_cast<const bf16_t*>(a.P);
  const bf16_t* __restrict__ Gp = reinterpret_cast<const bf16_t*>(a.G);
  const int kh = wv / a.K, kw = wv - kh * a.K;
  auto win0 = [&](int band) {
    int g = band * a.prow * a.S - a.Pd;
    g = g < 0 ? 0 : g;
    return g > a.HL - a.grow ? a.HL - a.grow : g;
  };

  const int slots = nPb * 8 + nGb * VG;
  const int ipr = nthr / slots;
  const bool active = t < ipr * slots;
  const int img_r = t / slots, rem = t - img_r * slots;
  const bool isP = rem < nPb * 8;
  const int px = isP ? rem >> 3 : (rem - nPb * 8) / VG, cg = isP ? rem & 7 : (rem - nPb * 8) % VG;
  const bool pro = isP ? a.proP_scale != nullptr : a.proG_scale != nullptr;
  float* sPro = reinterpret_cast<float*>(smem + 2 * stageB);
  if (t < 128) {
    const bool p = a.proP_scale != nullptr;
    const int c = t & 63, nc = p ? 64 : TB;
    const float* sc = p ? a.proP_scale + a0 : a.proG_scale ? a.proG_scale + b0 : nullptr;
    const float* sh = p ? a.proP_shift + a0 : a.proG_scale ? a.proG_shift + b0 : nullptr;
    sPro[t] = (!sc || c >= nc) ? (t < 64 ? 1.f : 0.f) : t < 64 ? sc[c] : sh[c];
  }
  const float lo = (isP ? a.proP_relu : a.proG_relu) ? 0.f : -__builtin_inff();
  const long istride = isP ? (long)npos * a.Ca : (long)npix * a.Cb;
  const bf16_t* src0 = isP ? Pp + (long)px * a.Ca + a0 + cg * 8 : Gp + (long)px * a.Cb + b0 + cg * 8;
  const int ip_t = isP ? ipP : ipG;
  const int dst0 = (isP ? 0 : KI * ipP) + img_r * ip_t + px * (isP ? 128 : PXG) + cg * 16;
  Vec16 q[kMaxV];
  auto fetch = [&](int n0, int band) {
    const long boff = isP ? (long)band * nPb * a.Ca : (long)win0(band) * a.HL * a.Cb;
#pragma unroll
    for (int k = 0; k < kMaxV; ++k) {
      const int img = k * ipr + img_r;
      q[k] = Vec16{{0, 0, 0, 0}};
      if (active && img < KI && n0 + img < n_end) {
        q[k] = *reinterpret_cast<const Vec16*>(src0 + (long)(n0 + img) * istride + boff);
        if (pro) {
          float f[8];
          Elem<bf16_t>::unpack(q[k], f);
          const float4 s0 = *reinterpret_cast<const float4*>(sPro + cg * 8), s1 = *reinterpret_cast<const float4*>(sPro + cg * 8 + 4);
          const float4 h0 = *reinterpret_cast<const float4*>(sPro + 64 + cg * 8), h1 = *reinterpret_cast<const float4*>(sPro + 64 + cg * 8 + 4);
          const float sc[8] = {s0.x, s0.y, s0.z, s0.w, s1.x, s1.y, s1.z, s1.w}, sh[8] = {h0.x, h0.y, h0.z, h0.w, h1.x, h1.y, h1.z, h1.w};
#pragma unroll
          for (int j = 0; j < 8; ++j) f[j] = fmaxf(f[j] * sc[j] + sh[j], lo);
          q[k] = Elem<bf16_t>::pack(f);
        }
      }
    }
  };
  auto commit = [&](char* buf) {
#pragma unroll
    for (int k = 0; k < kMaxV; ++k)
      if (active && k * ipr + img_r < KI) *reinterpret_cast<Vec16*>(buf + dst0 + k * ipr * ip_t) = q[k];
  };

  f32x16 acc[2][NFB];
#pragma unroll
  for (int i = 0; i < 2; ++i)
#pragma unroll
    for (int j = 0; j < NFB; ++j)
#pragma unroll
      for (int e = 0; e < 16; ++e) acc[i][j][e] = 0.f;

  const int li = lane & 15;
  const int lrow = ((lane >> 5) << 3) + (li >> 2);
  const int lcol = (((lane >> 4) & 1) << 5) + ((li & 3) << 3);
  __syncthreads();
  const int nchunk = (n_end - n_begin + KI - 1) / KI, nstage = nchunk * a.nb;
  fetch(n_begin, 0);
  commit(smem);
  __syncthreads();
  int cur = 0, band = 0, n0 = n_begin;
  for (int st = 0; st < nstage; ++st) {
    int bn = band + 1, nn = n0;
    if (bn == a.nb) { bn = 0; nn = n0 + KI; }
    const bool more = st + 1 < nstage;
    if (more) fetch(nn, bn);
    const char* sP = smem + cur * stageB;
    const char* sG = sP + KI * ipP;
    const int g0 = win0(band);
    for (int hr = 0; hr < a.prow; ++hr) {
      const int hs = band * a.prow + hr;
      const int hl = hs * a.S - a.Pd + kh;
      if (hl < g0 || hl >= g0 + a.grow || hl < 0 || hl >= a.HL) continue;
      for (int ws = 0; ws < a.HS; ++ws) {
        const int wl = ws * a.S - a.Pd + kw;
        if (wl < 0 || wl >= a.HL) continue;
        const char* pb = sP + (hr * a.HS + ws) * 128 + lcol;
        const char* gb = sG + ((hl - g0) * a.HL + wl) * PXG + lcol;
#pragma unroll
        for (int ks = 0; ks < KI / 16; ++ks) {
          bf16x8 fa[2], fb[NFB];
          typedef __attribute__((ext_vector_type(8))) short s16x8;
#pragma unroll
          for (int f = 0; f < 2; ++f) {
            const char* pa = pb + (ks * 16 + lrow) * ipP + f * 64;
            const s16x4 a_lo = __builtin_amdgcn_ds_read_tr16_b64_v4i16((__attribute__((address_space(3))) s16x4*)(pa));
            const s16x4 a_hi = __builtin_amdgcn_ds_read_tr16_b64_v4i16((__attribute__((address_space(3))) s16x4*)(pa + 4 * ipP));
            fa[f] = __builtin_bit_cast(bf16x8, (s16x8)__builtin_shufflevector(a_lo, a_hi, 0, 1, 2, 3, 4, 5, 6, 7));
          }
#pragma unroll
          for (int f = 0; f < NFB; ++f) {
            const char* pg = gb + (ks * 16 + lrow) * ipG + f * 64;
            const s16x4 g_lo = __builtin_amdgcn_ds_read_tr16_b64_v4i16((__attribute__((address_space(3))) s16x4*)(pg));
            const s16x4 g_hi = __builtin_amdgcn_ds_read_tr16_b64_v4i16((__attribute__((address_space(3))) s16x4*)(pg + 4 * ipG));
            fb[f] = __builtin_bit_cast(bf16x8, (s16x8)__builtin_shufflevector(g_lo, g_hi, 0, 1, 2, 3, 4, 5, 6, 7));
          }
#pragma unroll
          for (int i = 0; i < 2; ++i)
#pragma unroll
            for (int j = 0; j < NFB; ++j) acc[i][j] = __builtin_amdgcn_mfma_f32_32x32x16_bf16(fa[i], fb[j], acc[i][j], 0, 0, 0);
        }
      }
    }
    if (more) commit(smem + (cur ^ 1) * stageB);
    __syncthreads();
    cur ^= 1; band = bn; n0 = nn;
  }
  const int ntaps = a.K * a.K;
  float* out = a.part + (((long)blockIdx.x * ntaps + wv) * a.Ca + a0) * a.Cb + b0;
#pragma unroll
  for (int i = 0; i < 2; ++i)
#pragma unroll
    for (int j = 0; j < NFB; ++j)
#pragma unroll
      for (int v = 0; v < 16; ++v) {
        const int row = 32 * i + 8 * (v >> 2) + 4 * (lane >> 5) + (v & 3), col = 32 * j + (lane & 31);
        out[(long)row * a.Cb + col] = acc[i][j][v];
      }
}

int try_wgrad_pos(int dt, const WgradArgs& a, hipStream_t s) {
  if (dt != DT_BF16 || a.P_planar || !a.scratch || (a.proP_scale && a.proG_scale)) return 0;
  if (a.Hp != a.Wp || a.Hg != a.Wg || a.Hp < 1 || a.Hp > 4 || a.Hg > 8 || a.Ca % 64 != 0 || a.Cb % 32 != 0) return 0;
  if (a.ksz < 1 || a.ksz > 4 || a.ntaps != a.ksz * a.ksz || a.ksz * a.ksz < 4) return 0;
  if ((a.Ca_valid && a.Ca_valid != a.Ca) || (a.Cb_valid && a.Cb_valid != a.Cb)) return 0;
  for (int t = 0; t < a.ntaps; ++t) if (a.tap_off[t] != t) return 0;
  const int npos = a.Hp * a.Hp, npix = a.Hg * a.Hg;
  if (npos + npix < 8) return 0;
  const int nthr = 64 * a.ntaps;
  const int nfb = (a.Cb % 64 == 0 && (a.Ca / 64) * (a.Cb / 64) >= 8) ? 2 : 1;
  const int TB = 32 * nfb, VG = TB / 8;
  const int tiles = (a.Ca / 64) * (a.Cb / TB);
  int KI = 16, nb = 0, prow = 0, grow = 0, rounds = 0;
  size_t stageB = 0;
  const int maxv = nthr == 1024 ? 4 : 8;
  for (int cand = 1; cand <= a.Hp && !nb; cand *= 2) {
    if (a.Hp % cand) continue;
    const int pr = a.Hp / cand;
    int gr = (pr - 1) * a.stride + a.ksz; if (gr > a.Hg) gr = a.Hg;
    const int nPb = pr * a.Hp, nGb = gr * a.Hg;
    const int ipP = ((nPb * 128 + 191) & ~255) + 64, ipG = ((nGb * TB * 2 + 191) & ~255) + 64;
    const int slots = nPb * 8 + nGb * VG;
    const int ipr = nthr / slots;
    if (ipr < 1) continue;
    for (int ki = (cand == 1 && npos + npix <= 8) ? 32 : 16; ki >= 16; ki -= 16) {
      const size_t sb = (size_t)ki * (ipP + ipG);
      const int rd = (ki + ipr - 1) / ipr;
      if (2 * sb + 512 <= 160 * 1024 && rd <= maxv) { KI = ki; nb = cand; prow = pr; grow = gr; stageB = sb; rounds = rd; break; }
    }
  }
  if (!nb) return 0;
  WposArgs b; std::memset(&b, 0, sizeof(b));
  b.P = a.P; b.G = a.G; b.part = a.scratch;
  b.proP_scale = a.proP_scale; b.proP_shift = a.proP_shift; b.proP_relu = a.proP_relu;
  b.proG_scale = a.proG_scale; b.proG_shift = a.proG_shift; b.proG_relu = a.proG_relu;
  b.N = a.N; b.Ca = a.Ca; b.Cb = a.Cb; b.HS = a.Hp; b.HL = a.Hg; b.K = a.ksz; b.S = a.stride; b.Pd = a.pad;
  b.nb = nb; b.prow = prow; b.grow = grow;
  const long wsize = (long)a.Ca * a.Cb * a.ntaps;
  int nsplit = (256 + tiles - 1) / tiles;
  const int max_split = wsize * 4 * 64 <= (32L << 20) ? 64 : 32;
  if (nsplit > max_split) nsplit = max_split;
  const long cap = (long)(kWgradScratchBytes / 4) / wsize;
  if (cap < 1) return 0;
  if (nsplit > cap) nsplit = (int)cap;
  int per = (a.N + nsplit - 1) / nsplit;
  per = ((per + KI - 1) / KI) * KI;
  if (per < 2 * KI) per = 2 * KI;
  nsplit = (a.N + per - 1) / per;
  b.nsplit = nsplit; b.imgs_per_split = per;
  const size_t lds = 2 * stageB + 512;
  dim3 grid(nsplit, tiles), block(nthr);
  bool launched = false;
#define MMVAE_WPOS(KI_, NT_, MV_, NF_) \
  if (!launched && KI == KI_ && nthr == NT_ && nfb == NF_ && (MV_ == 8 || rounds <= 4)) { \
    static bool attr_set = false; \
    if (!attr_set) { \
      if (hipFuncSetAttribute(reinterpret_cast<const void*>(&wgrad_pos_kernel<KI_, NT_, MV_, NF_>), hipFuncAttributeMaxDynamicSharedMemorySize, 160 * 1024) != hipSuccess) { \
        set_error("wgrad_pos: hipFuncSetAttribute"); return MMVAE_ERR_HIP; } \
      attr_set = true; } \
    hipLaunchKernelGGL((wgrad_pos_kernel<KI_, NT_, MV_, NF_>), grid, block, lds, s, b); launched = true; }
  MMVAE_WPOS(32, 256, 8, 2) MMVAE_WPOS(32, 576, 4, 2) MMVAE_WPOS(32, 576, 8, 2) MMVAE_WPOS(32, 1024, 4, 2)
  MMVAE_WPOS(16, 256, 8, 2) MMVAE_WPOS(16, 576, 4, 2) MMVAE_WPOS(16, 576, 8, 2) MMVAE_WPOS(16, 1024, 4, 2)
  MMVAE_WPOS(16, 256, 8, 1) MMVAE_WPOS(16, 576, 4, 1) MMVAE_WPOS(16, 576, 8, 1) MMVAE_WPOS(16, 1024, 4, 1)
#undef MMVAE_WPOS
  if (!launched) return 0;
  const int rc = check_launch("wgrad_pos");
  if (rc) return rc;
  WgradReduceArgs u; std::memset(&u, 0, sizeof(u));
  u.part = a.scratch; u.dW = a.dW; u.Ca = a.Ca; u.Cb = a.Cb; u.ntaps = a.ntaps; u.nparts = nsplit;
  u.Ca_valid = a.Ca; u.Cb_valid = a.Cb; u.sA = a.sA; u.sB = a.sB; u.scale = a.scale;
  for (int t = 0; t < 25; ++t) u.tap_off[t] = a.tap_off[t];
  const int rr = launch_wgrad_reduce(u, s);
  return rr < 0 ? rr : 1;
}

}
```

moving-mnist-vae_amd/csrc/conv_wstream.hip:

```cpp
#include <hip/hip_runtime.h>

#include <stdlib.h>
#include <string.h>

#include "kernels.hpp"
#include "tile_common.hpp"

namespace mmvae {

struct WStreamArgs {
  const void* P; const void* G; float* part;
  const float* proP_scale; const float* proP_shift; int proP_relu;
  const float* proG_scale; const float* proG_shift; int proG_relu;
  int N, Hp, Hg, Wg;
  int HS;
  int nunits;
  const void* wd;
  void* dx;
  const void* x2; const void* w2;
  float* bn_part;
  const void* P2;
  const void* Jy; const float* jA; const float* jB; const float* jC;
};

// ... 359 lines not shown
        for (int ca = 0; ca < CA16; ++ca)
#pragma unroll
          for (int cb = 0; cb < CB16; ++cb)
#pragma unroll
            for (int j = 0; j < 4; ++j) {
              float* p = img + (k * CA + ca * 16 + 4 * gq + j) * CB + cb * 16 + r;
              *p = (w == 0 ? 0.f : *p) + acc[k][ca][cb][j];
            }
      if constexpr (X2) {
#pragma unroll
        for (int ca = 0; ca < CA16; ++ca)
#pragma unroll
          for (int j = 0; j < 4; ++j) {
            float* p = img + NT * CA * CB + (4 * gq + j) * CA + ca * 16 + r;
            *p = (w == 0 ? 0.f : *p) + acc2[ca][j];
          }
      }
      if constexpr (P2) {
#pragma unroll
        for (int ca = 0; ca < CA16; ++ca)
#pragma unroll
          for (int cb = 0; cb < CB16; ++cb)
#pragma unroll
            for (int j = 0; j < 4; ++j) {
              float* p = img + (NT * CA + ca * 16 + 4 * gq + j) * CB + cb * 16 + r;
              *p = (w == 0 ? 0.f : *p) + accD[ca][cb][j];
            }
      }
    }
    __syncthreads();
  }
  if constexpr (ST) {
    float* sb = img + WSIZE;
#pragma unroll
    for (int j = 0; j < 4; ++j) { bs0[j] = row16_sum(bs0[j]); bs1[j] = row16_sum(bs1[j]); }
    if (r == 0) {
#pragma unroll
      for (int j = 0; j < 4; ++j) { sb[wv * 32 + 4 * gq + j] = bs0[j]; sb[wv * 32 + 16 + 4 * gq + j] = bs1[j]; }
    }
    __syncthreads();
    if (t < 32) {
      float sum = sb[t];
      for (int w = 1; w < NW; ++w) sum += sb[w * 32 + t];
      a.bn_part[(long)blockIdx.x * 32 + t] = sum;
    }
  }
  float* dst = a.part + (long)blockIdx.x * WSIZE;
  for (int i = t; i < WSIZE / 4; i += 64 * NW) reinterpret_cast<float4*>(dst)[i] = reinterpret_cast<const float4*>(img)[i];
}

template <int KS, int S, int PAD, int WP, int CA16, int CB16, bool PRO_P, bool PRO_G, bool DG, bool X2, bool ST = false, int NW = 4, bool P2 = false, bool JG = false>
static int launch_wstream_t(const WStreamArgs& a, int gx, hipStream_t s) {
  constexpr int RP = 32 / WP;
  constexpr int WL = S * (WP - 1) + KS;
  constexpr int NSLOT = S * (RP - 1) + KS + S * RP;
  constexpr size_t rings = NW * (size_t)(NSLOT * WL * CB16 * 32 + 32 * CA16 * 32 + (X2 ? 32 * 32 : 0) + (ST ? 32 * CA16 * 32 : 0) + (P2 ? 32 * CA16 * 32 : 0)) +
                           ((DG && CA16 > 1) ? CA16 * (KS * KS / 2) * 1024 : 0) + (JG ? 3 * CB16 * 16 * 4 : 0) + ((PRO_G && P2) ? 2 * CB16 * 16 * 4 : 0);
  constexpr size_t flush = ((size_t)KS * KS * CA16 * 16 * CB16 * 16 + (X2 ? 16 * CA16 * 16 : 0) + (P2 ? CA16 * 16 * CB16 * 16 : 0)) * 4 + 512;
  constexpr size_t lds = rings > flush ? rings : flush;
  static_assert(lds <= 160 * 1024, "one block must fit the CU's LDS");
  auto kern = &wgrad_stream_kernel<KS, S, PAD, WP, CA16, CB16, PRO_P, PRO_G, DG, X2, ST, NW, P2, JG>;
  static bool attr_set = false;
  if (!attr_set) {
    const hipError_t e = hipFuncSetAttribute(reinterpret_cast<const void*>(kern), hipFuncAttributeMaxDynamicSharedMemorySize, 160 * 1024);
    if (e != hipSuccess) { set_error("wgrad_stream: hipFuncSetAttribute: %s", hipGetErrorString(e)); return MMVAE_ERR_HIP; }
    attr_set = true;
  }
  hipLaunchKernelGGL(kern, dim3(gx), dim3(64 * NW), lds, s, a);
  return check_launch("wgrad_stream");
}

static int wstream_kind(int dt, const WgradArgs& a) {
  if (dt != DT_BF16 || a.P_planar || !a.scratch) return 0;
  if (a.ntaps != a.ksz * a.ksz || a.Cb_valid != a.Cb || a.Ca_valid != a.Ca) return 0;
  for (int t = 0; t < a.ntaps; ++t) if (a.tap_off[t] != t) return 0;
  if (a.Wg != a.stride * a.Wp || a.Hg != a.stride * a.Hp || a.Hp != a.Wp) return 0;
  if (a.ksz == 4 && a.stride == 2 && a.pad == 1 && a.Cb == 16 && (a.Ca == 16 || a.Ca == 32)) return a.Wp == 32 ? 1 : (a.Wp == 16 ? 2 : 0);
  if (a.ksz == 3 && a.pad == 1 && a.Wp == 16 && a.Ca == 32 && a.Cb == 32 && !(a.proP_scale && a.proG_scale)) return a.stride == 1 ? 3 : (a.stride == 2 ? 4 : 0);
  return 0;
}
static int wstream_fill(const WgradArgs& a, WStreamArgs& b, int kind, bool x2 = false, bool p2 = false) {
  memset(&b, 0, sizeof(b));
  b.P = a.P; b.G = a.G; b.part = a.scratch;
  b.proP_scale = a.proP_scale; b.proP_shift = a.proP_shift; b.proP_relu = a.proP_relu;
  b.proG_scale = a.proG_scale; b.proG_shift = a.proG_shift; b.proG_relu = a.proG_relu;
  b.N = a.N; b.Hp = a.Hp; b.Hg = a.Hg; b.Wg = a.Wg;
  b.HS = a.Hp % 16 == 0 ? 16 : a.Hp;
  b.nunits = a.N * (a.Hp / b.HS);
  const int nw = kind == 4 ? 2 : 4;
  int gx = kind == 4 ? 768 : 512;
  while (gx > 8 && (long)gx * nw > b.nunits) gx -= 8;
  const int wsize = (a.ntaps + ((x2 || p2) ? 1 : 0)) * a.Ca * a.Cb;
  if ((size_t)gx * wsize * 4 > kWgradScratchBytes) return 0;
  return gx;
}
static int wstream_reduce(const WgradArgs& a, int gx, hipStream_t s, bool x2 = false, float* dW2 = nullptr, float scale2 = 1.f) {
  WgradReduceArgs u; memset(&u, 0, sizeof(u));
  u.part = a.scratch; u.dW = a.dW; u.Ca = a.Ca; u.Cb = a.Cb; u.ntaps = a.ntaps; u.nparts = gx;
  u.Ca_valid = a.Ca_valid; u.Cb_valid = a.Cb_valid; u.sA = a.sA; u.sB = a.sB; u.scale = a.scale;
  u.part_stride = (long)a.ntaps * a.Ca * a.Cb + (x2 ? 16L * a.Ca : 0);
  for (int t = 0; t < 25; ++t) u.tap_off[t] = a.tap_off[t];
  if (a.defer && !x2) { *a.defer = u; return 0; }
  const int rc = launch_wgrad_reduce(u, s);
  if (rc < 0 || !x2 || !dW2) return rc;
  WgradReduceArgs v; memset(&v, 0, sizeof(v));
  v.part = a.scratch + (long)a.ntaps * a.Ca * a.Cb; v.part_stride = u.part_stride; v.dW = dW2; v.Ca = 16; v.Cb = a.Ca; v.ntaps = 1; v.nparts = gx;
  v.Ca_valid = 16; v.Cb_valid = a.Ca; v.sA = a.Ca; v.sB = 1; v.scale = scale2;
  return launch_wgrad_reduce(v, s);
}

bool wgrad_stream_shape(int dt, const WgradArgs& a) {
  return wstream_kind(dt, a) != 0 && !(a.proP_scale && a.proG_scale);
}

int try_wgrad_stream(int dt, const WgradArgs& a, hipStream_t s) {
  const int kind = wstream_kind(dt, a);
  if (!kind) return 0;
  WStreamArgs b;
  const int gx = wstream_fill(a, b, kind);
  if (gx <= 0) return 0;
  const bool pp = a.proP_scale != nullptr, pg = a.proG_scale != nullptr;
  int rc = 0;
#define MMVAE_WS(KS, S, WP, CA, CB, NW)                                                                                      \
  rc = pp ? (pg ? 0 : launch_wstream_t<KS, S, 1, WP, CA, CB, true, false, false, false, false, NW>(b, gx, s))                \
          : (pg ? launch_wstream_t<KS, S, 1, WP, CA, CB, false, true, false, false, false, NW>(b, gx, s)                     \
                : launch_wstream_t<KS, S, 1, WP, CA, CB, false, false, false, false, false, NW>(b, gx, s))
  if (pp && pg) return 0;
  if (kind == 1) { if (a.Ca == 16) MMVAE_WS(4, 2, 32, 1, 1, 4); else MMVAE_WS(4, 2, 32, 2, 1, 4); }
  else if (kind == 2) { if (a.Ca == 16) MMVAE_WS(4, 2, 16, 1, 1, 4); else MMVAE_WS(4, 2, 16, 2, 1, 4); }
  else if (kind == 3) MMVAE_WS(3, 1, 16, 2, 2, 4);
  else MMVAE_WS(3, 2, 16, 2, 2, 2);
#undef MMVAE_WS
  if (rc < 0) return rc;
  const int rc2 = wstream_reduce(a, gx, s);
  return rc2 < 0 ? rc2 : 1;
}

int try_wgrad_stream_pair(int dt, const WgradArgs& a, const void* P2, float* dW2, float scale2, hipStream_t s) {
  const int kind = wstream_kind(dt, a);
  if (kind != 4 || a.proP_scale || !P2 || !dW2) return 0;
  WStreamArgs b;
  const int gx = wstream_fill(a, b, kind, false, true);
  if (gx <= 0) return 0;
  b.P2 = P2;
  note_launch_bytes((double)a.N * 2.0 * ((double)a.Hp * a.Wp * 2 * a.Ca + (double)a.Hg * a.Wg * a.Cb));
  const int rc = a.proG_scale ? launch_wstream_t<3, 2, 1, 16, 2, 2, false, true, false, false, false, 2, true>(b, gx, s)
                              : launch_wstream_t<3, 2, 1, 16, 2, 2, false, false, false, false, false, 2, true>(b, gx, s);
  if (rc < 0) return rc;
  WgradReduceArgs u; memset(&u, 0, sizeof(u));
  u.part = a.scratch; u.dW = a.dW; u.Ca = a.Ca; u.Cb = a.Cb; u.ntaps = a.ntaps; u.nparts = gx;
  u.Ca_valid = a.Ca_valid; u.Cb_valid = a.Cb_valid; u.sA = a.sA; u.sB = a.sB; u.scale = a.scale;
  u.part_stride = (long)(a.ntaps + 1) * a.Ca * a.Cb;
  for (int t = 0; t < 25; ++t) u.tap_off[t] = a.tap_off[t];
  int rc2 = launch_wgrad_reduce(u, s);
  if (rc2 < 0) return rc2;
  WgradReduceArgs v; memset(&v, 0, sizeof(v));
  v.part = a.scratch + (long)a.ntaps * a.Ca * a.Cb; v.part_stride = u.part_stride; v.dW = dW2; v.Ca = a.Ca; v.Cb = a.Cb; v.ntaps = 1; v.nparts = gx;
  v.Ca_valid = a.Ca; v.Cb_valid = a.Cb; v.sA = a.Cb; v.sB = 1; v.scale = scale2;
  rc2 = launch_wgrad_reduce(v, s);
  return rc2 < 0 ? rc2 : 1;
}

bool dgrad_wgrad_stream_shape(int dt, const WgradArgs& a) {
  const int kind = wstream_kind(dt, a);
  return (kind == 1 || kind == 2) && !a.proG_scale;
}
bool dgrad_wgrad_stream_jg_shape(int dt, const WgradArgs& a, bool has_x2, bool bn_sums) {
  if (!dgrad_wgrad_stream_shape(dt, a) || wstream_kind(dt, a) != 2) return false;
  return (a.Ca == 16 && a.proP_scale && bn_sums && !has_x2) || (a.Ca == 32 && !a.proP_scale && has_x2 && !bn_sums);
}
int try_dgrad_wgrad_stream(int dt, const WgradArgs& a, const void* wd, void* dx, const void* x2, const void* w2, float* bn_part, hipStream_t s,
                           float* dW2, float scale2, const JoinGrad* jg) {
  if (!dgrad_wgrad_stream_shape(dt, a) || !wd || !dx || ((x2 != nullptr) != (w2 != nullptr))) return 0;
  if (jg && !dgrad_wgrad_stream_jg_shape(dt, a, x2 != nullptr, bn_part != nullptr)) { set_error("dgrad_wgrad_stream: no join-gradient form of this shape"); return MMVAE_ERR_UNSUPPORTED; }
  if (bn_part && (x2 || !a.proP_scale || a.Ca != 16)) { set_error("dgrad_wgrad_stream: BatchNorm sums need the prologue'd 16-channel P and no second source"); return MMVAE_ERR_ARG; }
  const int kind = wstream_kind(dt, a);
  WStreamArgs b;
  const int gx = wstream_fill(a, b, kind, x2 != nullptr);
  if (gx <= 0) return 0;
  b.wd = wd; b.dx = dx; b.x2 = x2; b.w2 = w2; b.bn_part = bn_part;
  if (jg) { b.Jy = jg->y; b.jA = jg->A; b.jB = jg->B; b.jC = jg->C; }
  note_launch_bytes((double)a.N * 2.0 * ((double)a.Hp * a.Wp * (2 * a.Ca + (x2 ? 16 : 0)) + (double)a.Hg * a.Wg * a.Cb * (jg ? 2 : 1)));
  const bool pp = a.proP_scale != nullptr;
  int rc;
#define MMVAE_WSD(WP, CA)                                                                                                    \
  do {                                                                                                                        \
    if (x2) rc = pp ? launch_wstream_t<4, 2, 1, WP, CA, 1, true, false, true, true>(b, gx, s)                                 \
                    : launch_wstream_t<4, 2, 1, WP, CA, 1, false, false, true, true>(b, gx, s);                               \
    else rc = pp ? launch_wstream_t<4, 2, 1, WP, CA, 1, true, false, true, false>(b, gx, s)                                   \
                 : launch_wstream_t<4, 2, 1, WP, CA, 1, false, false, true, false>(b, gx, s);                                 \
  } while (0)
  if (jg) rc = bn_part ? launch_wstream_t<4, 2, 1, 16, 1, 1, true, false, true, false, true, 4, false, true>(b, gx, s)
                       : launch_wstream_t<4, 2, 1, 16, 2, 1, false, false, true, true, false, 4, false, true>(b, gx, s);
  else if (bn_part) rc = kind == 1 ? launch_wstream_t<4, 2, 1, 32, 1, 1, true, false, true, false, true>(b, gx, s)
                              : launch_wstream_t<4, 2, 1, 16, 1, 1, true, false, true, false, true>(b, gx, s);
  else if (kind == 1) { if (a.Ca == 16) MMVAE_WSD(32, 1); else MMVAE_WSD(32, 2); }
  else { if (a.Ca == 16) MMVAE_WSD(16, 1); else MMVAE_WSD(16, 2); }
#undef MMVAE_WSD
  if (rc < 0) return rc;
  const int rc2 = wstream_reduce(a, gx, s, x2 != nullptr, dW2, scale2);
  return rc2 < 0 ? rc2 : gx;
}

}
```

moving-mnist-vae_amd/csrc/kernels.hpp:

```cpp
#pragma once
#include "common.hpp"

namespace mmvae {

enum DType : int { DT_F32 = 0, DT_BF16 = 1 };
inline size_t dtype_size(int dt) { return dt == DT_F32 ? 4 : 2; }

struct Tap { int dh, dw; };
constexpr int kMaxTaps = 25;
constexpr int kMaxPhases = 4;
struct Phase { int ph, pw, Hq, Wq, ntaps, tap0; long w_off;  };
struct GatherArgs {
  const void* x; const void* w; void* y;
  const float* pro_scale; const float* pro_shift; int pro_relu;
  const float* bias;
  float* stats;
  int accumulate;
  int N, Hi, Wi, Cin, Ho, Wo, Cout;
  int SI, SO;
  int nphase; Phase phases[kMaxPhases]; Tap taps[kMaxTaps];
  int cin_vecs;
  int x_planar, x_planes;
  int y_planes;
  const void* x2; const void* w2; int Cin2, x2_ph, x2_pw;
  int fp8;
  int wfrag, wfrag2;
  int gk, gs, gp, gup;
};
bool deep2_shape_ok(int dt, int Cin, int Cout, int Hq, int Wq, int Hi, int Wi, int ntaps_all, int fp8 = 0);
int launch_gather_gemm(int dt, int out_dt, GatherArgs a, hipStream_t s);
constexpr int kGatherMaxGridX = 1024;

struct WgradArgs {
  const void* P; const void* G; float* dW;
  const float* proP_scale; const float* proP_shift; int proP_relu;
  const float* proG_scale; const float* proG_shift; int proG_relu;
  int N, Hp, Wp, Ca, Hg, Wg, Cb;
  int Cb_valid;
  int Ca_valid;
  int P_planar, P_planes;
  float* scratch;
  int stride, pad, ksz;
  int sA, sB; int ntaps; int tap_off[25];
  float scale;
  int M, pix_per_block;
  int TA16, TB16, TG;
  struct WgradReduceArgs* defer;
};
int launch_wgrad(int dt, WgradArgs a, hipStream_t s);
int try_wgrad_pos(int dt, const WgradArgs& a, hipStream_t s);
bool wgrad_stream_shape(int dt, const WgradArgs& a);
int try_wgrad_stream(int dt, const WgradArgs& a, hipStream_t s);
int try_wgrad_stream_pair(int dt, const WgradArgs& a, const void* P2, float* dW2, float scale2, hipStream_t s);
bool dgrad_wgrad_stream_shape(int dt, const WgradArgs& a);
struct JoinGrad { const void* y; const float* A; const float* B; const float* C; };
bool dgrad_wgrad_stream_jg_shape(int dt, const WgradArgs& a, bool has_x2, bool bn_sums);
int try_dgrad_wgrad_stream(int dt, const WgradArgs& a, const void* wd, void* dx, const void* x2, const void* w2, float* bn_part, hipStream_t s,
                           float* dW2 = nullptr, float scale2 = 1.f, const JoinGrad* jg = nullptr);

struct JoinBwdLaunch {
  const float* d_raw; const float* w_tail; const void* y2; const void* ys;
  const float* ms2; const float* mb2; const float* mss; const float* mbs;
  const float* A2; const float* B2; const float* C2; const float* As; const float* Bs; const float* Cs;
  const void* y1; const float* p1s; const float* p1b; const void* wd2; void* da1; float* part2; float* bn_part;
  const void* xin; const float* pxs; const float* pxb; const void* wds; void* gin; float* parts;
  int N;
  int f8in = 0;
};
bool join_bwd_stream_ok(int dt, int OC, int C, int Hp, int Hg);
int launch_join_bwd_stream(const JoinBwdLaunch& L, hipStream_t s);
struct Conv1BwdLaunch {
  const void* da1; const void* y1; const float* ms; const float* mb; const float* A; const float* B; const float* C;
  const void* xin; const float* pxs; const float* pxb; const void* w1u; void* gin; float* part; long nrows;
  int mask_out = 0;
};
int launch_conv1_bwd_stream(const Conv1BwdLaunch& L, hipStream_t s);
bool join_conv1_fwd_ok(int dt, int C, int Cout_next, long npix);
int launch_join_conv1_fwd(int C, const void* y2, const float* s2, const float* b2, const void* ys, const float* ss, const float* bs, const void* w1_down,
                          void* out, void* y1, float* stats, long npix, hipStream_t s);

struct TileGeom { int N, Hq, Wq, Hi, Wi, SI, oh, ow, segs, qr, PR, PW, tiles_per_img, ntiles, TP, sub, sub_j, sub_seg, sub_pix; };
bool make_tile_geom(TileGeom& g, int N, int Hq, int Wq, int Hi, int Wi, int SI, int oh, int ow, int span_h, int span_w, int TP = 128,
                    int sub = 1);
struct Wgrad2Args {
  const void* P; const void* G; float* dW;
  const float* proP_scale; const float* proP_shift; int proP_relu;
  const float* proG_scale; const float* proG_shift; int proG_relu;
  TileGeom g;
  int Ca, Cb, Cb_valid, Ca_valid, ksz, ntaps, TG;
  int sA, sB; int tap_off[25]; float scale;
  int P_planar, P_planes;
  int nw;
  int partial;
};
size_t wgrad2_lds_bytes(const Wgrad2Args& a, int dt, int TA, int TB);
int wgrad2_patch_slots(const Wgrad2Args& a, int dt, int TB);
int wgrad2_taps_per_block(int ta16, int tb16, int ntaps);
int launch_wgrad2(int dt, const Wgrad2Args& a, int gx, int tiles_ab, int zg, int ta16, int tb16, hipStream_t s);
size_t gather3_lds_bytes(const GatherArgs& a, int dt, int CT);
int launch_gather3(int dt, int out_dt, const GatherArgs& a, int gx, hipStream_t s);
struct WgradReduceArgs { const float* part; float* dW; int Ca, Cb, ntaps, nparts, Ca_valid, Cb_valid, sA, sB; int tap_off[25]; float scale; int exclusive;
                         long part_stride;  };
int launch_wgrad_reduce(WgradReduceArgs a, hipStream_t s);
constexpr size_t kWgradScratchBytes = 64u << 20;
struct PatchPhase { int ph, pw, Hq, Wq, ntaps, tap0; long w_off; int w_vec0, koff0; };
struct PatchArgs {
  const void* x; const void* w; void* y;
  const float* pro_scale; const float* pro_shift; int pro_relu;
  const float* bias; float* stats; int accumulate;
  int Cin, Cout, Ho, Wo, SO;
  TileGeom g;
  int nphase; PatchPhase phases[kMaxPhases]; Tap taps[kMaxTaps];
  int w_vecs, koff_total;
  int x_planar, x_planes, y_planes;
  int npt, wq_shift;
  int uni, out_wave_bytes;
  int phase_of[4];
  unsigned x_bytes;
  const void* x2; const void* w2; int Cin2, x2_phase, kvp2, w2_vec0, x2_vec0, x2_slots; unsigned x2_bytes;
};
size_t patch_conv_lds_bytes(const PatchArgs& a, int dt);
void patch_conv_x2_carve(PatchArgs& a, int dt);
int patch_conv_slots(const PatchArgs& a, int dt);
int launch_patch_conv(int dt, int out_dt, const PatchArgs& a, int gx, hipStream_t s);
struct DeepPhase { int ph, pw, Hq, Wq, ntaps, tap0; long w_off; };
struct DeepArgs {
  const void* x; const void* w; void* y;
  const float* pro_scale; const float* pro_shift; int pro_relu;
  const float* bias; float* stats; int accumulate;
  int N, Hi, Wi, Cin, Ho, Wo, Cout, SI, SO;
  int Hq, Wq;
  int nphase; DeepPhase phases[kMaxPhases]; Tap taps[kMaxTaps]; int ntaps_all;
  int ipt, ntiles;
  int ct16, npt;
  int fp8;
  int nw, cpt_log2;
  int wfrag;
};
size_t deep2_conv_lds_bytes(const DeepArgs& a, int dt);
int launch_deep2_conv(int dt, int out_dt, const DeepArgs& a, int gx, hipStream_t s);
struct PosArgs {
  const void* x; const void* w; void* y;
  const float* pro_scale; const float* pro_shift; int pro_relu;
  float* stats; int accumulate;
  int N, Cout;
  int nw;
  int ntiles;
};
int launch_pos_conv(int K, int S, int P, int up, int HI, int HO, int CIN, const PosArgs& a, hipStream_t s);
bool pos_conv_takes(int K, int S, int P, int up, int HI, int HO, int CIN);

struct PackArgs {
  const float* src; void* dst; int cols, K, ntaps; int s_col, s_k; int tap_off[kMaxTaps]; float scale;
  int cols_valid, K_valid;
  int fp8;
  int frag;
};
int launch_pack(int dt, const PackArgs& a, hipStream_t s);
void pack_batch_begin();
int pack_batch_flush(int dt, hipStream_t s);

int launch_stem_im2col(int dt, const void* x, void* col, int N, int H, int W, int Ho, int Wo, hipStream_t s);

bool stem_bwd_fusable(int S);
bool conv3_stream_ok(int dt, int Cin, int Cout, int k, int s, int p, int Hin, int Win);
int launch_conv3_stream_bwd(int dt, const void* dy, const void* w_flipped, void* dx, const void* ym, const float* ms, const float* mb, float* sums,
                            int N, int H, hipStream_t s);
int launch_conv3_stream(int dt, int stride, const void* x, const void* w, const void* wsc, void* y, void* ysc, const float* pro_scale,
                        const float* pro_shift, int pro_relu, float* stats, float* stats_sc, int N, int Ho, hipStream_t s);
bool convT4_stream_ok(int dt, int Cin, int Cout, int k, int s, int p, int Hin, int Win);
int launch_convT4_stream(int dt, const void* x, const void* w_up, void* y, const float* pro_scale, const float* pro_shift, int pro_relu, float* stats,
                         int N, int Hin, hipStream_t s, int f8out = 0);
bool tail_fwd_stream_ok(int dt, int OC, int H, int W);
int launch_tail_fwd_stream(int dt, const void* y2, const float* s2, const float* b2, const void* ys, const float* ss, const float* bs, const float* w,
                           const float* bias, float* r_raw, float* stats, int N, int H, int W, hipStream_t s, int f8in = 0);
bool up5_tail_fwd_ok(int dt, int OC, int C, int Cin, int Hin, int Hout);
int launch_up5_tail_fwd(const void* y1, const float* p1s, const float* p1b, const void* w2_up, const void* xin, const float* pxs, const float* pxb,
                        const void* wu_up, const float* s2, const float* b2, const float* ss, const float* bs, const float* w, const float* bias,
                        float* r_raw, float* stats, int N, hipStream_t s);
bool stem_fwd_stream_ok(int dt, int S);
int launch_stem_fwd_stream(int dt, const void* x, const float* w, void* y, float* stats, int N, int S, hipStream_t s);
int stem_bwd_part_floats();
int launch_stem_gram(int dt, const void* x, float* scratch, long scratch_cap_floats, double* R, int N, int S, int Ho, int Wo, hipStream_t s);
int launch_stem_bwd(int dt, const void* g, const void* y0, const void* x, const float* ms, const float* mb, float* partials,
                    long partials_cap_floats, int N, int S, int Ho, int Wo, hipStream_t s);
bool stem_bwd_dg_ok(int dt, int S);
int launch_stem_bwd_dg(const void* dy1, const void* dys, const void* wd1, const void* wds, const void* y0, const void* x, const float* ms, const float* mb,
                       float* partials, long partials_cap_floats, int N, int S, int Ho, int Wo, hipStream_t s);
int launch_stem_bwd_finalize(const float* partials, int nparts, const double* R, const float* w, const float* global_sums, double count,
                             const float* gamma, const float* mean, const float* istd, float* dgamma, float* dbeta, float* dW, hipStream_t s);

int launch_chan_stats_nhwc(int dt, const void* y, long npix, int C, float* partials, hipStream_t s);
int chan_stats_parts(long npix, int C);
struct BnFinalizeArgs {
  float in_scale = 1.f;
  const float* partials; int nparts; int C; double count;
  const float* gamma; const float* beta; float* running_mean; float* running_var; long long* nbt;
  float* mean; float* istd; float* scale; float* shift; float momentum, eps;
};
int launch_bn_finalize(const BnFinalizeArgs& a, hipStream_t s);
int launch_partial_rowsum(const float* partials, int nparts, int width, float* out, hipStream_t s, int row_stride = 0);
struct BnFoldEntry { int g_off, b_off, rm_off, rv_off, scale_off, shift_off, C; float in_scale; };
constexpr int kBnFoldMax = 96;
struct BnFoldTable { BnFoldEntry e[kBnFoldMax]; };
int launch_bn_fold_eval(const BnFoldEntry* entries, int n, const float* params, const float* bnbuf, float* bnws, float eps, hipStream_t s);
int launch_join_fwd(int dt, const void* a, const float* sa, const float* ba, const void* b, const float* sb, const float* bb,
                    void* out, long npix, int C, hipStream_t s);
int launch_affine_act(int dt, const void* a, const float* sa, const float* ba, int relu, void* out, long npix, int C,
                      hipStream_t s);
int launch_bn_bwd_reduce(int dt, const void* dout, const void* out, const float* msk_scale, const float* msk_shift,
                         const void* y0, const void* y1, long npix, int C, float* partials, hipStream_t s,
                         const float* msk_scale1 = nullptr, const float* msk_shift1 = nullptr);
struct BnBwdFinalizeArgs {
  const float* partials; int nparts; int C; int which ; int ny; double count;
  const float* gamma; const float* mean; const float* istd; float* dgamma; float* dbeta; float* coefA; float* coefB; float* coefC;
  float* dbias_conv = nullptr; float dbias_scale = 1.f;
};
int launch_bn_bwd_finalize(const BnBwdFinalizeArgs& a, hipStream_t s);
int launch_bn_bwd_finalize2(const BnBwdFinalizeArgs& a0, const BnBwdFinalizeArgs& a1, hipStream_t s);
int launch_bn_bwd_apply(int dt, const void* dout, const void* out, const float* msk_scale, const float* msk_shift,
                        const void* y0, const float* A0, const float* B0, const float* C0, void* dy0,
                        const void* y1, const float* A1, const float* B1, const float* C1, void* dy1,
                        long npix, int C, hipStream_t s, const float* msk_scale1 = nullptr, const float* msk_shift1 = nullptr);
bool tail_join_fusable(int dt, int OC, int N, int H, int W);
int launch_tail_join_bwd_reduce(int dt, const float* d_raw, const float* w, int OC, int N, int H, int W, const float* ms, const float* mb,
                                const float* ms1, const float* mb1, const void* y0, const void* y1, float* partials, hipStream_t s,
                                float* wpartials = nullptr, int f8in = 0);
int launch_tail_wgrad_finalize(const float* wpartials, int nparts, float* dW, hipStream_t s);
int launch_tail_join_bwd_apply(int dt, const float* d_raw, const float* w, int OC, int N, int H, int W, const float* ms, const float* mb,
                               const float* ms1, const float* mb1, const void* y0, const float* A0, const float* B0, const float* C0, void* dy0,
                               const void* y1, const float* A1, const float* B1, const float* C1, void* dy1, hipStream_t s);
bool tail_fwd_fusable(int dt, int OC, int N, int H, int W);
int launch_tail_join_fwd(int dt, const void* y0, const float* ms, const float* mb, const void* y1, const float* ms1, const float* mb1,
                         const float* w, const float* bias, float* r_raw, float* stats, int N, int H, int W, hipStream_t s);
int launch_affine_nchw(const float* raw, const float* scale, const float* shift, float* out, int N, int C, int HW, hipStream_t s);
int launch_bn_bwd_reduce_nchw(const float* dout, const float* y, int N, int C, int HW, float* partials, hipStream_t s);
int launch_bn_bwd_apply_nchw(const float* dout, const float* y, const float* A, const float* B, const float* Cc, float* dy,
                             int N, int C, int HW, hipStream_t s);
int launch_gauss_tail_reduce(const float* raw, const float* target, const float* scale, const float* shift, float sigma, float coef, const float* gscale,
                             int N, int C, int HW, float* partials, hipStream_t s);
int launch_gauss_tail_apply(const float* raw, const float* target, const float* scale, const float* shift, float sigma, float coef, const float* gscale,
                            const float* A, const float* B, const float* Cc, float* dy, int N, int C, int HW, hipStream_t s);

int launch_inorm_planar_fwd(int dt, const float* x, void* xn16, float* stats, int N, int C, int HW, hipStream_t s);
int launch_inorm_planar2_fwd(int dt, const float* xa, int Ca, const float* xb, int Cb, void* xn16, float* stats, int N, int HW, hipStream_t s);
int launch_inorm_planar_bwd(int dt, const void* g16, const float* x, const float* stats, float* dx, int N, int C, int HW, hipStream_t s);
int launch_inorm_nhwc_fwd(int dt, const void* h, void* a, float* stats, int N, int C, int HW, int relu, hipStream_t s);
int launch_inorm_nhwc_bwd(int dt, const void* g, const void* h, const float* stats, void* dh, int N, int C, int HW, int relu, hipStream_t s);
int launch_nhwc16_to_planar(int dt, const void* o16, float* out, int N, int C, int HW, hipStream_t s);
int launch_planar_to_nhwc16(int dt, const float* in, void* o16, int N, int C, int HW, hipStream_t s);
int launch_planar_to_nhwc16(int dt, const void* in, int in_dt, void* o16, int N, int C, int HW, hipStream_t s);

struct PixelHeadArgs {
  const void* a;
  const void* w;
// ... 39 lines not shown
```

moving-mnist-vae_amd/csrc/vae_net.cpp:

```cpp
#include "vae_net.hpp"

#include <algorithm>
#include <cmath>
#include <cstdlib>
#include <cstring>

#include "conv_ops.hpp"

namespace mmvae {

#define MM_TRY(expr)            \
  do {                          \
    int rc__ = (expr);          \
    if (rc__ < 0) return rc__;  \
  } while (0)

static inline long align_up(long v, long a) { return (v + a - 1) / a * a; }
static inline int down_size(int H, int k, int s, int p) { return conv_down_size(H, k, s, p); }

void Net::add_entry(const std::string& name, std::initializer_list<int> shape, int kind, long off) {
  Entry e; e.name = name; e.ndim = (int)shape.size(); e.kind = kind; e.offset = off;
  int i = 0; for (int d : shape) e.shape[i++] = d;
  for (; i < 4; ++i) e.shape[i] = 1;
  entries.push_back(e);
// ... 120 lines not shown
  tail = add_conv("decoder.conv2.weight", c.out_ch, 16, 3, 1, 1, false);
  tail_bias = n_params; add_entry("decoder.conv2.bias", {c.out_ch}, EK_PARAM, n_params); n_params += c.out_ch;
  bn_out = add_bn("decoder.bn2", c.out_ch);
}

Net::~Net() {
  if (side_state_ != 1) return;
  if (side_) { (void)hipStreamSynchronize(side_); (void)hipStreamDestroy(side_); }
  for (hipEvent_t e : ev_) if (e) (void)hipEventDestroy(e);
  for (hipEvent_t e : blk_ev_) if (e) (void)hipEventDestroy(e);
  if (gram_ev_) (void)hipEventDestroy(gram_ev_);
  (void)hipGetLastError();
}

size_t Net::workspace_bytes(int N) { return plan(N).bytes; }

const Plan& Net::plan(int N) {
  if (plan_.N == N) return plan_;
  Plan P; P.N = N;
  long cur = 0, maxact = 0;
  const long e = (long)esz();
  auto take = [&](long bytes) { long o = cur; cur = align_up(cur + std::max(bytes, 16L), 256); return o; };
  auto act = [&](long elems) { maxact = std::max(maxact, elems * e); return take(elems * e); };
  P.x_t = act((long)N * cfg.in_ch * cfg.S * cfg.S);
  P.y0 = act((long)N * H1 * W1 * 32);
  for (Block& B : enc) {
    const long n = (long)N * B.Hout * B.Wout * B.C;
    B.y1 = act(n); B.y2 = act(n); B.ys = B.identity ? 0 : act(n); B.out = act(n);
  }
  P.enc_t = act((long)N * cfg.z);
  P.y0d = act((long)N * 4 * 128);
  P.act0d = cfg.blocks > 1 ? act((long)N * 4 * 128) : 0;
  for (Block& B : dec) {
    const long n = (long)N * B.Hout * B.Wout * B.C;
    B.y1 = act((long)N * B.Hin * B.Win * B.C); B.y2 = act(n); B.ys = B.identity ? 0 : act(n); B.out = act(n);
  }
  P.cvec = take(512 * 4);
  P.r_raw = take((long)N * cfg.out_ch * Sd * Sd * 4);
  P.d_raw = take((long)N * cfg.out_ch * Sd * Sd * 4);
  P.col = act(cfg.in_ch == 1 ? (long)N * H1 * W1 * 32 : (long)N * cfg.S * cfg.S * 16);
  P.packed = take(n_packed * e);
  P.bnws = take(n_bnws * 4);
  P.partials = take(2 * kPartialFloats * 4);
  P.syncbuf = take(2 * 1024 * 4);
  for (int i = 0; i < 2; ++i) P.g[i] = take(maxact);
  for (int i = 0; i < 2; ++i) { P.dy1[i] = take(maxact); P.dy2[i] = take(maxact); P.dys[i] = take(maxact); }
  for (int i = 0; i < 2; ++i) {
    const Block& B = enc[enc.size() - 2 + i];
    const long nb = (long)N * B.Hout * B.Wout * B.C * e;
    P.edy1[i] = take(nb); P.edy2[i] = take(nb); P.edys[i] = take(nb);
  }
  P.da1 = take(maxact);
  P.dh = take((long)N * 2 * cfg.z * e);
  P.wscratch = take((long)kWgradScratchBytes);
  P.wscratch2 = take(2L * 1024 * 4096 * 4);
  P.stem_R = take(1024 * 8);
  P.stem_gram = take(1024L * stem_bwd_part_floats() * 4);
  P.bytes = (size_t)cur;
  plan_ = P;
  return plan_;
}

int Net::fill_consts(char* base, hipStream_t s) {
  float* c = reinterpret_cast<float*>(base + plan_.cvec);
  MM_TRY(launch_fill_f32(c, 1.f, 256, s));
  return launch_fill_f32(c + 256, 0.f, 256, s);
}

float* Net::bnf(const Bn& bn, char* base, int which) const {
  return reinterpret_cast<float*>(base + plan_.bnws) + bn.ws + (long)which * align_up(bn.C, 4);
}

static inline ConvGeom geom(const ConvW& w) { return ConvGeom{w.D0, w.D1, w.k, w.s, w.p}; }

int Net::frag_down(const ConvW& w) const { return w.Hl > 0 ? op_deep2_down_ok(dt(), geom(w), w.Hl, w.Hl, (w.fp8 && !w.tr) ? 1 : 0) : 0; }
int Net::frag_up(const ConvW& w) const { return w.Hl > 0 ? op_deep2_up_ok(dt(), geom(w), w.Hl, w.Hl, 1, (w.fp8 && w.tr) ? 1 : 0) : 0; }
int Net::pack_down(const ConvW& w, const float* params, char* base, hipStream_t s) {
  return op_pack_down(dt(), geom(w), params + w.off, base + plan_.packed + w.packD * (long)esz(), s, w.wscale, (w.fp8 && !w.tr) ? 1 : 0,
                      frag_down(w));
}
int Net::pack_up(const ConvW& w, const float* params, char* base, hipStream_t s) {
  return op_pack_up(dt(), geom(w), params + w.off, base + plan_.packed + w.packU * (long)esz(), s, w.wscale, (w.fp8 && w.tr) ? 1 : 0,
                    frag_up(w));
}
int Net::run_down(const ConvW& w, char* base, int N, const void* L, int Hl, int Wl, void* S, int Hs, int Ws,
                  const float* pro_s, const float* pro_b, int relu, float* stats, int accumulate, int out_dt, hipStream_t s,
                  const ConvW* w2, const void* x2) {
  SecondSrc q;
  if (w2) { q.x2 = x2; q.w2 = base + plan_.packed + w2->packU * (long)esz(); q.Cin2 = w2->D0; }
  q.fp8 = (w.fp8 && !w.tr) ? 1 : 0;
  q.wfrag = frag_down(w); q.wfrag2 = w2 ? frag_up(*w2) : 0;
  return op_run_down(dt(), out_dt, geom(w), base + plan_.packed + w.packD * (long)esz(), N, L, Hl, Wl, S, Hs, Ws, pro_s, pro_b, relu,
                     stats, accumulate, s, q);
}
int Net::run_up(const ConvW& w, char* base, int N, const void* S, int Hs, int Ws, void* L, int Hl, int Wl,
                const float* pro_s, const float* pro_b, int relu, float* stats, int accumulate, hipStream_t s,
                const ConvW* w2, const void* x2) {
  SecondSrc q;
  if (w2) { q.x2 = x2; q.w2 = base + plan_.packed + w2->packU * (long)esz(); q.Cin2 = w2->D0; }
  q.fp8 = (w.fp8 && w.tr) ? 1 : 0;
  q.wfrag = frag_up(w); q.wfrag2 = w2 ? frag_up(*w2) : 0;
  return op_run_up(dt(), geom(w), base + plan_.packed + w.packU * (long)esz(), N, S, Hs, Ws, L, Hl, Wl, pro_s, pro_b, relu, stats,
                   accumulate, s, q);
}
hipStream_t Net::wgrad_stream(hipStream_t s) {
  if (side_state_ == 0) {
    side_state_ = 1;
    bool ok = hipStreamCreateWithFlags(&side_, hipStreamNonBlocking) == hipSuccess;
    for (int i = 0; i < kForkEvents && ok; ++i) ok = hipEventCreateWithFlags(&ev_[i], hipEventDisableTiming) == hipSuccess;
    for (int i = 0; i < 16 && ok; ++i) ok = hipEventCreateWithFlags(&blk_ev_[i], hipEventDisableTiming) == hipSuccess;
    if (ok) ok = hipEventCreateWithFlags(&gram_ev_, hipEventDisableTiming) == hipSuccess;
    if (!ok) { (void)hipGetLastError(); side_state_ = -1; }
  }
  return side_state_ == 1 ? side_ : s;
}
int Net::side_fork(hipStream_t s) {
  if (wgrad_stream(s) == s) return MMVAE_OK;
  hipEvent_t e = ev_[evi_++ % kForkEvents];
  bool ok = hipEventRecord(e, s) == hipSuccess && hipStreamWaitEvent(side_, e, 0) == hipSuccess;
  if (!ok) { set_error("side stream fork failed"); return MMVAE_ERR_HIP; }
  return MMVAE_OK;
}
int Net::side_join(hipStream_t s) {
  if (wgrad_stream(s) == s) return MMVAE_OK;
  hipEvent_t e = ev_[evi_++ % kForkEvents];
  bool ok = hipEventRecord(e, side_) == hipSuccess && hipStreamWaitEvent(s, e, 0) == hipSuccess;
  if (!ok) { set_error("side stream join failed"); return MMVAE_ERR_HIP; }
  return MMVAE_OK;
}

bool Net::stem_bwd_fused() const {
  return cfg.in_ch == 1 && stem_bwd_fusable(cfg.S);
}

int Net::side_mark(int slot) {
  if (side_state_ != 1) return MMVAE_OK;
  bool ok = hipEventRecord(blk_ev_[slot & 15], side_) == hipSuccess;
  if (!ok) { set_error("side stream mark failed"); return MMVAE_ERR_HIP; }
  return MMVAE_OK;
}
int Net::side_wait_mark(int slot, hipStream_t s) {
  if (side_state_ != 1) return MMVAE_OK;
  bool ok = hipStreamWaitEvent(s, blk_ev_[slot & 15], 0) == hipSuccess;
  if (!ok) { set_error("side stream wait failed"); return MMVAE_ERR_HIP; }
  return MMVAE_OK;
}

int Net::run_wgrad(const ConvW& w, int N, const void* P, int Hs, int Ws, const float* proP_s, const float* proP_b,
                   const void* G, int Hl, int Wl, const float* proG_s, const float* proG_b, float* grads, hipStream_t s) {
  return op_run_wgrad(dt(), geom(w), N, P, Hs, Ws, proP_s, proP_b, 1, G, Hl, Wl, proG_s, proG_b, 1, grads + w.off, s, wscratch_, w.wscale);
}

static bool wgrad_pair_ok(int dt, const ConvGeom& g, const ConvGeom& gs, int Hout, int Hin) {
  return dt == DT_BF16 && g.k == 3 && g.s == 2 && g.p == 1 && gs.k == 1 && gs.s == 2 && gs.p == 0 && g.D0 == 32 && g.D1 == 32 && gs.D0 == 32 &&
         gs.D1 == 32 && Hout == 16 && Hin == 32;
}

bool Net::l1_dgrad_stream() const {
  if (enc.empty()) return false;
  const Block& B = enc[0];
  return !B.identity && !B.c2.fp8 && conv3_stream_ok(dt(), B.C, B.C, B.c2.k, B.c2.s, B.c2.p, B.Hout, B.Wout);
}

bool Net::stem_dg_fused() const {
  if (enc.empty() || !stem_bwd_fused() || !stem_bwd_dg_ok(dt(), cfg.S)) return false;
  const Block& B = enc[0];
  return !B.identity && B.Cin == 32 && B.C == 32 && B.c1.k == 3 && B.c1.s == 2 && B.c1.p == 1 && B.cs.k == 1 && B.cs.s == 2 && B.cs.p == 0 &&
         !B.c1.fp8 && !B.cs.fp8 && B.c1.wscale == 1.f && B.cs.wscale == 1.f && frag_up(B.c1) == 0 && frag_up(B.cs) == 0 && H1 == 32 && B.Hout == 16;
}

bool Net::tail_fwd_fused() const {
  return !dec.empty() && dec.back().C == 16 && tail_fwd_fusable(dt(), cfg.out_ch, 1, Sd, Sd) &&
         tail_join_fusable(dt(), cfg.out_ch, 1, Sd, Sd);
}

int Net::sync_rows(char* base, const float* partials, int nparts, int width, hipStream_t s, float** out, int row_stride) {
  if (width > 1024) { set_error("sync_bn: %d statistics per BatchNorm > 1024", width); return MMVAE_ERR_UNSUPPORTED; }
  float* buf = reinterpret_cast<float*>(base + plan_.syncbuf) + (s == side_ ? 1024 : 0);
  MM_TRY(launch_partial_rowsum(partials, nparts, width, buf, s, row_stride));
  if (comm_) MM_TRY(comm_allreduce_sum((s == side_ && comm_side_) ? comm_side_ : comm_, buf, width, s));
  else if (ar_fn_(buf, width, s, ar_user_) != 0) { set_error("sync_bn: the all-reduce callback failed"); return MMVAE_ERR_ARG; }
  *out = buf;
  return MMVAE_OK;
}

int Net::bn_train(const Bn& bn, const float* params, float* bnbuf, long long* nbt, char* base, int nparts, double count, hipStream_t s,
                  long part_off, float in_scale) {
  BnFinalizeArgs a;
  a.in_scale = in_scale;
  a.partials = reinterpret_cast<const float*>(base + plan_.partials) + part_off; a.nparts = nparts; a.C = bn.C; a.count = count;
  if (sync_bn_on()) {
    float* row = nullptr;
    MM_TRY(sync_rows(base, a.partials, nparts, 2 * bn.C, s, &row));
    a.partials = row; a.nparts = 1; a.count = count * ar_world_;
  }
  a.gamma = params + bn.g_off; a.beta = params + bn.b_off;
  a.running_mean = bnbuf ? bnbuf + bn.rm_off : nullptr; a.running_var = bnbuf ? bnbuf + bn.rv_off : nullptr;
  a.nbt = nbt ? nbt + bn.nbt_idx : nullptr;
  a.mean = bnf(bn, base, 0); a.istd = bnf(bn, base, 1); a.scale = bnf(bn, base, 2); a.shift = bnf(bn, base, 3);
  a.momentum = 0.1f; a.eps = 1e-5f;
  return launch_bn_finalize(a, s);
}

int Net::fold_bn_eval(int which, const float* params, const float* bnbuf, char* base, hipStream_t s) {
  std::vector<BnFoldEntry> tab;
  auto add = [&](const Bn& bn, float in_scale) {
    BnFoldEntry e;
    e.g_off = (int)bn.g_off; e.b_off = (int)bn.b_off; e.rm_off = (int)bn.rm_off; e.rv_off = (int)bn.rv_off;
    e.scale_off = (int)(bn.ws + 2L * align_up(bn.C, 4)); e.shift_off = (int)(bn.ws + 3L * align_up(bn.C, 4)); e.C = bn.C; e.in_scale = in_scale;
    tab.push_back(e);
  };
  if (which == 0) add(bn0, 1.f); else add(dbn0, dstem.wscale);
  for (const Block& B : which == 0 ? enc : dec) {
    add(B.b1, B.c1.wscale); add(B.b2, B.c2.wscale);
    if (!B.identity) add(B.bs, B.cs.wscale);
  }
  if (which == 1) add(bn_out, 1.f);
  MM_TRY(launch_bn_fold_eval(tab.data(), (int)tab.size(), params, bnbuf, reinterpret_cast<float*>(base + plan_.bnws), 1e-5f, s));
  eval_folded_ = true;
  return MMVAE_OK;
}

int Net::bn_eval(const Bn&, const float*, const float*, char*, hipStream_t, float) {
  if (eval_folded_) return MMVAE_OK;
  set_error("bn_eval: the entry point did not fold its BatchNorms"); return MMVAE_ERR_ARG;
}

BnBwdFinalizeArgs Net::bwd_finalize_args(const Bn& bn, const float* params, float* grads, char* base, const float* partials, int nparts, int ny,
                                         int which, double count) const {
  const Net& net = *this;
  BnBwdFinalizeArgs a;
  a.partials = partials; a.nparts = nparts; a.C = bn.C; a.which = which; a.ny = ny;
  a.count = count; a.gamma = params + bn.g_off; a.mean = net.bnf(bn, base, 0); a.istd = net.bnf(bn, base, 1);
  a.dgamma = grads + bn.g_off; a.dbeta = grads + bn.b_off;
  a.coefA = net.bnf(bn, base, 4); a.coefB = net.bnf(bn, base, 5); a.coefC = net.bnf(bn, base, 6);
  return a;
}
int Net::bn_backward_coefs(const Bn& bn, const float* params, float* grads, char* base, int nparts, int ny, int which, double count,
                           hipStream_t s, float* dbias_conv) {
  const float* part = reinterpret_cast<const float*>(base + plan_.partials);
  BnBwdFinalizeArgs l = bwd_finalize_args(bn, params, grads, base, part, nparts, ny, which, count);
  if (!sync_bn_on()) l.dbias_conv = dbias_conv;
  MM_TRY(launch_bn_bwd_finalize(l, s));
  if (!sync_bn_on()) return MMVAE_OK;
  float* row = nullptr;
  MM_TRY(sync_rows(base, part, nparts, (1 + ny) * bn.C, s, &row));
  BnBwdFinalizeArgs g = bwd_finalize_args(bn, params, grads, base, row, 1, ny, which, count * ar_world_);
  g.dgamma = nullptr; g.dbeta = nullptr;
  g.dbias_conv = dbias_conv; g.dbias_scale = 1.f / (float)ar_world_;
  return launch_bn_bwd_finalize(g, s);
}
int Net::bn_backward_coefs_join(const Bn& b2, const Bn& bs, const float* params, float* grads, char* base, int nparts, double count,
                                hipStream_t s) {
  const float* part = reinterpret_cast<const float*>(base + plan_.partials);
  MM_TRY(launch_bn_bwd_finalize2(bwd_finalize_args(b2, params, grads, base, part, nparts, 2, 0, count),
                                 bwd_finalize_args(bs, params, grads, base, part, nparts, 2, 1, count), s));
  if (!sync_bn_on()) return MMVAE_OK;
  float* row = nullptr;
  MM_TRY(sync_rows(base, part, nparts, 3 * b2.C, s, &row));
  BnBwdFinalizeArgs g2 = bwd_finalize_args(b2, params, grads, base, row, 1, 2, 0, count * ar_world_);
  BnBwdFinalizeArgs gs = bwd_finalize_args(bs, params, grads, base, row, 1, 2, 1, count * ar_world_);
  g2.dgamma = g2.dbeta = gs.dgamma = gs.dbeta = nullptr;
  return launch_bn_bwd_finalize2(g2, gs, s);
}

int Net::packs_enc_fwd(const float* params, char* base, hipStream_t s) {
  const Plan& P = plan_;
  {
    const int cpad = dt() == DT_F32 ? 4 : 8;
    PackArgs pa; std::memset(&pa, 0, sizeof(pa));
    pa.src = params + stem.off; pa.dst = base + P.packed + stem_pack * (long)esz();
    pa.cols = 32; pa.K = cpad; pa.K_valid = cfg.in_ch; pa.ntaps = 25; pa.s_col = 25 * cfg.in_ch; pa.s_k = 25; pa.scale = 1.f;
    for (int t = 0; t < 25; ++t) pa.tap_off[t] = t;
    MM_TRY(launch_pack(dt(), pa, s));
  }
  for (const Block& B : enc) {
    MM_TRY(pack_down(B.c1, params, base, s));
    MM_TRY(pack_down(B.c2, params, base, s));
    if (!B.identity) MM_TRY(pack_down(B.cs, params, base, s));
  }
  const int nt = Hf * Wf;
  for (int h = 0; h < (cfg.need_logvar ? 2 : 1); ++h) {
    const ConvW& hw = h == 0 ? head_mu : head_lv;
    const long poff = h == 0 ? head_pack_mu : head_pack_lv;
    PackArgs pa; std::memset(&pa, 0, sizeof(pa));
    pa.src = params + hw.off; pa.dst = base + P.packed + poff * (long)esz();
    pa.cols = cfg.z; pa.K = 256; pa.ntaps = nt; pa.s_col = 256; pa.s_k = 1; pa.scale = 1.0f / nt;
    MM_TRY(launch_pack(dt(), pa, s));
  }
  return MMVAE_OK;
}

int Net::packs_enc_bwd(const float* params, char* base, hipStream_t s) {
  const Plan& P = plan_;
  const int Ch = cfg.need_logvar ? 2 * cfg.z : cfg.z;
  PackArgs pa; std::memset(&pa, 0, sizeof(pa));
  pa.src = params + head_mu.off; pa.dst = base + P.packed + head_pack_dg * (long)esz();
  pa.cols = 256; pa.K = Ch; pa.ntaps = 1; pa.s_col = 1; pa.s_k = 256; pa.scale = 1.0f / (Hf * Wf);
  MM_TRY(launch_pack(dt(), pa, s));
  for (const Block& B : enc) {
    MM_TRY(pack_up(B.c2, params, base, s));
    MM_TRY(pack_up(B.c1, params, base, s));
    if (!B.identity) MM_TRY(pack_up(B.cs, params, base, s));
  }
  if (l1_dgrad_stream()) {
    const ConvW& w = enc[0].c2;
    PackArgs pf; std::memset(&pf, 0, sizeof(pf));
    pf.src = params + w.off; pf.dst = base + P.packed + l1c2_flip * (long)esz();
// ... 627 lines not shown
```

Measured before the change: 849,600 frames/s.

## Fuse shortcut 1x1 wgrad into 3x3 wgrad kernels for deeper encoder blocks

Extends the paired weight-gradient path, which computes the 3x3 stride-2 conv's gradient and the 1x1 shortcut's gradient in one pass over the output gradient, from the first encoder block to the deeper blocks. It adds pair variants of the tiled wgrad2 kernel (an extra wave reading a second input tile) and of the positional wgrad kernel (an extra tap). The reduce kernel gains a second destination, so the stream pair path drops its separate reduce launch. This saves a second read of the output gradient and extra launches, at the cost of more LDS per block, lower occupancy bounds and new template instances.

```diff
diff --git a/moving-mnist-vae_amd/csrc/capi.cpp b/moving-mnist-vae_amd/csrc/capi.cpp
--- a/moving-mnist-vae_amd/csrc/capi.cpp
+++ b/moving-mnist-vae_amd/csrc/capi.cpp
@@ -363,7 +363,7 @@
   const ConvGeom g = geom_for(0, Cin, Cout, 3, 2, 1), gs = geom_for(0, Cin, Cout, 1, 2, 0);
   const int Ho = out_size(0, H, 3, 2, 1), Wo = out_size(0, W, 3, 2, 1);
   const int rc = op_run_wgrad_pair(dt, g, gs, N, dy, dy_sc, Ho, Wo, x, H, W, ps, pb, relu, dw, dw_sc, S(st), static_cast<float*>(scratch), 1.f, 1.f);
-  if (rc == 0) { set_error("conv2d_wgrad_pair: shape not supported (bf16, 32 -> 32 channels, 32x32 -> 16x16)"); return MMVAE_ERR_UNSUPPORTED; }
+  if (rc == 0) { set_error("conv2d_wgrad_pair: shape not supported (bf16; Cin -> Cout on HxH: 32 -> 32 on 32x32, 32 -> 64 on 16x16, 64 -> 128 on 8x8, 128 -> 256 on 4x4)"); return MMVAE_ERR_UNSUPPORTED; }
   return rc < 0 ? rc : MMVAE_OK;
 }
 int mmvae_convT_bwd_fused(int dt, const void* x, const void* dy, const float* w, float* dw, void* dx, int N, int H, int W, int Cin, int Cout, int k,
diff --git a/moving-mnist-vae_amd/csrc/conv_gemm.hip b/moving-mnist-vae_amd/csrc/conv_gemm.hip
--- a/moving-mnist-vae_amd/csrc/conv_gemm.hip
+++ b/moving-mnist-vae_amd/csrc/conv_gemm.hip
@@ -679,7 +679,10 @@
   }
 }
 
-static int try_wgrad2(int dt, const WgradArgs& a, hipStream_t s) {
+static int wgrad2_run(int dt, const WgradArgs& a, const void* P2, float* dW2, float scale2, hipStream_t s) {
+  const int pair = P2 ? 1 : 0;
+  if (pair && (dt != DT_BF16 || !dW2 || a.ksz != 3 || a.ntaps != 9 || a.stride != 2 || a.pad != 1 || a.proP_scale || a.P_planar || 2 * a.Hp != a.Hg ||
+               2 * a.Wp != a.Wg || a.Ca_valid != a.Ca || a.Cb_valid != a.Cb)) return 0;
   if (a.Ca % 16 || a.Cb % 16 || a.ntaps > 25) return 0;
   if (a.proP_scale && a.proG_scale) return 0;
   if (a.P_planar && (a.Ca != 16 || a.P_planes > 16 || a.proP_scale)) return 0;
@@ -706,13 +709,18 @@
   } else if (!a.P_planar && a.ntaps == 16 && ta16 == 4 && tb16 == 4) {
     b.nw = 8; b.TG = 16;
   }
+  if (pair) {
+    if (b.nw != 9 || ta16 != 4 || tb16 != 2) return 0;
+    for (int t = 0; t < 9; ++t) if (a.tap_off[t] != t) return 0;
+    b.nw = 10; b.P2 = P2;
+  }
   bool fits = false;
   size_t lds = 0;
   for (int TP = 128; TP >= 32 && !fits; TP >>= 1) {
     if (TP < 128 && a.ntaps < 4) break;
     if (!make_tile_geom(b.g, a.N, a.Hp, a.Wp, a.Hg, a.Wg, a.stride, -a.pad, -a.pad, a.ksz, a.ksz, TP, 1)) continue;
     lds = wgrad2_lds_bytes(b, dt, TA, TB);
-    fits = lds <= kV2MaxLds && wgrad2_patch_slots(b, dt, TB) <= (b.nw == 4 ? 16 : 8);
+    fits = lds <= (pair ? 96 * 1024 : kV2MaxLds) && wgrad2_patch_slots(b, dt, TB) <= (b.nw == 4 ? 16 : pair ? 4 : 8);
   }
   if (!fits) return 0;
   b.Ca = a.Ca; b.Cb = a.Cb; b.Cb_valid = a.Cb_valid; b.Ca_valid = a.Ca_valid; b.ksz = a.ksz; b.ntaps = a.ntaps;
@@ -720,7 +728,7 @@
   for (int t = 0; t < 25; ++t) b.tap_off[t] = a.tap_off[t];
   const int tiles_ab = (a.Ca / TA) * (a.Cb / TB);
   const int zg = (a.ntaps + b.TG - 1) / b.TG;
-  const long wsize = (long)a.Ca * a.Cb * a.ntaps;
+  const long wsize = (long)a.Ca * a.Cb * (a.ntaps + pair);
   const long op_bytes = ((long)a.N * a.Hp * a.Wp * a.Ca + (long)a.N * a.Hg * a.Wg * a.Cb) * (long)dtype_size(dt);
   int occ = (int)((160 * 1024) / lds); if (occ > 6) occ = 6; if (occ < 1) occ = 1;
   long gx = (op_bytes < (200L << 20) ? 176L : 256L * occ) / ((long)tiles_ab * zg); if (gx < 1) gx = 1;
@@ -735,14 +743,21 @@
   if (gx > b.g.ntiles) gx = b.g.ntiles;
   if (gx >= 8) gx &= ~7L;
   b.dW = a.scratch; b.partial = 1;
+  if (pair) note_launch_bytes((double)a.N * 2.0 * ((double)a.Hp * a.Wp * 2 * a.Ca + (double)a.Hg * a.Wg * a.Cb));
   const int rc = launch_wgrad2(dt, b, (int)gx, tiles_ab, zg, ta16, tb16, s);
   if (rc < 0) return rc;
   WgradReduceArgs u; memset(&u, 0, sizeof(u));
   u.part = a.scratch; u.dW = a.dW; u.Ca = a.Ca; u.Cb = a.Cb; u.ntaps = a.ntaps; u.nparts = (int)gx;
   u.Ca_valid = a.Ca_valid; u.Cb_valid = a.Cb_valid; u.sA = a.sA; u.sB = a.sB; u.scale = a.scale;
   for (int t = 0; t < 25; ++t) u.tap_off[t] = a.tap_off[t];
+  if (pair) { u.dW2 = dW2; u.sA2 = a.Cb; u.sB2 = 1; u.scale2 = scale2; }
   const int rc2 = launch_wgrad_reduce(u, s);
   return rc2 < 0 ? rc2 : 1;
+}
+static int try_wgrad2(int dt, const WgradArgs& a, hipStream_t s) { return wgrad2_run(dt, a, nullptr, nullptr, 1.f, s); }
+int try_wgrad2_pair(int dt, const WgradArgs& a, const void* P2, float* dW2, float scale2, hipStream_t s) {
+  if (!P2 || !dW2 || !a.scratch) return 0;
+  return wgrad2_run(dt, a, P2, dW2, scale2, s);
 }
 
 #define MM_CHECK_RC(expr) do { const int rc__ = (expr); if (rc__ < 0) return rc__; } while (0)
diff --git a/moving-mnist-vae_amd/csrc/conv_ops.cpp b/moving-mnist-vae_amd/csrc/conv_ops.cpp
--- a/moving-mnist-vae_amd/csrc/conv_ops.cpp
+++ b/moving-mnist-vae_amd/csrc/conv_ops.cpp
@@ -166,7 +166,11 @@
   if (g.k != 3 || g.p != 1 || gs.k != 1 || gs.p != 0 || gs.s != g.s || gs.D0 != g.D0 || gs.D1 != g.D1) return 0;
   WgradArgs a;
   wgrad_args(a, g, N, P, Hs, Ws, nullptr, nullptr, 0, G, Hl, Wl, proG_s, proG_b, proG_relu, dW, scratch, scale);
-  return try_wgrad_stream_pair(dt, a, P2, dW2, scale2, s);
+  if (a.Ca_valid <= 0 || a.Ca_valid > a.Ca) a.Ca_valid = a.Ca;
+  int rc = try_wgrad_stream_pair(dt, a, P2, dW2, scale2, s);
+  if (rc == 0) rc = try_wgrad_pos_pair(dt, a, P2, dW2, scale2, s);
+  if (rc == 0) rc = try_wgrad2_pair(dt, a, P2, dW2, scale2, s);
+  return rc;
 }
 
 bool op_wgrad_is_stream(int dt, const ConvGeom& g, int N, int Hs, int Ws, int Hl, int Wl, bool proP, bool proG) {
diff --git a/moving-mnist-vae_amd/csrc/conv_wgrad.hip b/moving-mnist-vae_amd/csrc/conv_wgrad.hip
--- a/moving-mnist-vae_amd/csrc/conv_wgrad.hip
+++ b/moving-mnist-vae_amd/csrc/conv_wgrad.hip
@@ -14,7 +14,7 @@
 
 size_t wgrad2_lds_bytes(const Wgrad2Args& a, int dt, int TA, int TB) {
   const size_t es = dtype_size(dt);
-  const size_t stage = (size_t)a.g.TP * TA * es + (size_t)a.g.segs * a.g.PR * a.g.PW * TB * es + 32 * 4;
+  const size_t stage = (size_t)a.g.TP * TA * es * (a.P2 ? 2 : 1) + (size_t)a.g.segs * a.g.PR * a.g.PW * TB * es + 32 * 4;
   const size_t acc1 = (size_t)TA * TB * 4;
   return stage > acc1 ? stage : acc1;
 }
@@ -77,7 +77,8 @@
       const long i = (long)blockIdx.x * (4 * LANES) + l * 4 + j;
       const int t = (int)(i / ab), rem = (int)(i - (long)t * ab);
       const int aa = rem / a.Cb, bb = rem - aa * a.Cb;
-      if (aa < a.Ca_valid && bb < a.Cb_valid) a.dW[(long)aa * a.sA + (long)bb * a.sB + a.tap_off[t]] += v[j] * a.scale;
+      if (t >= a.ntaps) a.dW2[(long)aa * a.sA2 + (long)bb * a.sB2] += v[j] * a.scale2;
+      else if (aa < a.Ca_valid && bb < a.Cb_valid) a.dW[(long)aa * a.sA + (long)bb * a.sB + a.tap_off[t]] += v[j] * a.scale;
     }
   }
 }
@@ -87,14 +88,16 @@
   bool distinct = true;
   for (int t = 0; t < a.ntaps && distinct; ++t)
     for (int u = 0; u < t; ++u) if (a.tap_off[u] == a.tap_off[t]) { distinct = false; break; }
-  if (a.part_stride <= 0) a.part_stride = (long)a.ntaps * a.Ca * a.Cb;
+  const int planes = a.ntaps + (a.dW2 ? 1 : 0);
+  if (a.part_stride <= 0) a.part_stride = (long)planes * a.Ca * a.Cb;
+  if (!distinct && a.dW2) { set_error("wgrad_reduce: a second destination needs distinct taps"); return MMVAE_ERR_UNSUPPORTED; }
   if (!distinct) {
     for (int t = 1; t < a.ntaps; ++t)
       if (a.tap_off[t] != a.tap_off[0]) { set_error("wgrad_reduce: taps share some destinations but not all"); return MMVAE_ERR_UNSUPPORTED; }
     if (a.part_stride != (long)a.ntaps * a.Ca * a.Cb) { set_error("wgrad_reduce: shared destinations need densely packed partial images"); return MMVAE_ERR_UNSUPPORTED; }
     a.nparts *= a.ntaps; a.ntaps = 1; a.part_stride = (long)a.Ca * a.Cb;
   }
-  const long wsize = (long)a.ntaps * a.Ca * a.Cb;
+  const long wsize = (long)(a.dW2 ? planes : a.ntaps) * a.Ca * a.Cb;
   if (wsize % 256) { set_error("wgrad_reduce: %ld elements not a multiple of 256", wsize); return MMVAE_ERR_ARG; }
   a.exclusive = 1;
   note_launch_bytes((double)a.nparts * a.part_stride * 4.0);
diff --git a/moving-mnist-vae_amd/csrc/conv_wgrad.inc b/moving-mnist-vae_amd/csrc/conv_wgrad.inc
--- a/moving-mnist-vae_amd/csrc/conv_wgrad.inc
+++ b/moving-mnist-vae_amd/csrc/conv_wgrad.inc
@@ -20,9 +20,10 @@
   return Elem<T>::pack(f);
 }
 
-template <typename T, int TA16, int TB16, bool TS, int MAXG, bool PPL, int NW = 4>
-__global__ __launch_bounds__(64 * NW, NW == 16 ? 4 : (NW == 9 ? 3 : (NW == 8 ? 2 : (MAXG <= 8 ? 3 : 2) - (TA16 * TB16 > 2 ? 1 : 0)))) void wgrad2_kernel(Wgrad2Args a) {
+template <typename T, int TA16, int TB16, bool TS, int MAXG, bool PPL, int NW = 4, bool PAIR = false>
+__global__ __launch_bounds__(64 * NW, NW == 16 ? 4 : (NW == 10 ? 2 : (NW == 9 ? 3 : (NW == 8 ? 2 : (MAXG <= 8 ? 3 : 2) - (TA16 * TB16 > 2 ? 1 : 0))))) void wgrad2_kernel(Wgrad2Args a) {
   static_assert(NW == 4 || TS, "one-tap-per-wave blocks are tap-split");
+  static_assert(PAIR == (NW == 10) && (!PAIR || !PPL), "the pair form is the 9-tap block plus one wave");
   constexpr int NT = 64 * NW;
   constexpr int VE = Elem<T>::kVec;
   constexpr int ES = sizeof(T);
@@ -39,10 +40,12 @@
   const int a0 = (blockIdx.y / nb_tiles) * TA, b0 = (blockIdx.y % nb_tiles) * TB;
   const int tap0 = blockIdx.z * a.TG;
   const int tg_n = min(a.TG, a.ntaps - tap0);
+  const int tg_w = tg_n + (PAIR ? 1 : 0);
   const int npatch = g.segs * g.PR * g.PW;
   char* sP = smem;
   char* sG = sP + g.TP * TA * ES;
   int* sToff = reinterpret_cast<int*>(sG + npatch * TB * ES);
+  char* sP2 = reinterpret_cast<char*>(sToff + 32);
   const T* __restrict__ Pp = reinterpret_cast<const T*>(a.P);
   const T* __restrict__ Gp = reinterpret_cast<const T*>(a.G);
   const bool proP = a.proP_scale != nullptr, proG = a.proG_scale != nullptr;
@@ -51,6 +54,7 @@
     const int tap = tap0 + t, kh = tap / a.ksz, kw = tap - kh * a.ksz;
     sToff[t] = (kh * g.PW + kw) * TB * ES;
   }
+  if (PAIR && t == tg_n) sToff[t] = ((a.ksz >> 1) * g.PW + (a.ksz >> 1)) * TB * ES;
   const int cvp = t % CVP, pp0 = t / CVP, cvg = t % CVG, gp0 = t / CVG;
   float xsc[VE], xsh[VE];
 #pragma unroll
@@ -98,7 +102,7 @@
 #pragma unroll
   for (int tl = 0; tl < MAXT; ++tl) my_tap[tl] = TS ? wv + NW * tl : tl;
 
-  Vec16 gv[MAXG], pv[MAXP];
+  Vec16 gv[MAXG], pv[MAXP], pv2[PAIR ? MAXP : 1];
   int tb_c = 0, nv_c = 0;
   long m0_c = 0;
   const long pplane = (long)g.Hq * g.Wq;
@@ -124,6 +128,15 @@
         pv[k] = Vec16{{0, 0, 0, 0}};
         if (pix < nv_c) pv[k] = *reinterpret_cast<const Vec16*>(psrc + (long)pix * a.Ca);
       }
+      if constexpr (PAIR) {
+        const T* psrc2 = reinterpret_cast<const T*>(a.P2) + m0 * a.Ca + a0 + cvp * VE;
+#pragma unroll
+        for (int k = 0; k < MAXP; ++k) {
+          const int pix = pp0 + k * PSP;
+          pv2[k] = Vec16{{0, 0, 0, 0}};
+          if (pix < nv_c) pv2[k] = *reinterpret_cast<const Vec16*>(psrc2 + (long)pix * a.Ca);
+        }
+      }
     } else {
       m0_c = m0;
 #pragma unroll
@@ -171,6 +184,7 @@
           q = Elem<T>::pack(f);
         } else { if (proP && pix < nv_c) q = apply_pro<T, VE>(q, xsc, xsh, a.proP_relu); }
         reinterpret_cast<Vec16*>(sP)[pix * CVP + cvp] = q;
+        if constexpr (PAIR) reinterpret_cast<Vec16*>(sP2)[pix * CVP + cvp] = pv2[k];
       }
     }
   };
@@ -193,11 +207,12 @@
       for (int i = 0; i < NKS; ++i) {
         if (TS && i >= nks_tile) break;
         Vec16 af[TA16];
-#pragma unroll
-        for (int ta = 0; ta < TA16; ++ta) af[ta] = FragOps<bf16_t>::load(sP, offP[i][0] + ta * 32, offP[i][1] + ta * 32);
+        const char* sPw = (PAIR && wv == NW - 1) ? sP2 : sP;
+#pragma unroll
+        for (int ta = 0; ta < TA16; ++ta) af[ta] = FragOps<bf16_t>::load(sPw, offP[i][0] + ta * 32, offP[i][1] + ta * 32);
 #pragma unroll
         for (int tl = 0; tl < MAXT; ++tl) {
-          if (my_tap[tl] < tg_n) {
+          if (my_tap[tl] < tg_w) {
             const int toff = sToff[my_tap[tl]];
 #pragma unroll
             for (int tb = 0; tb < TB16; ++tb) {
@@ -240,8 +255,8 @@
   if (TS && a.partial) {
 #pragma unroll
     for (int tl = 0; tl < MAXT; ++tl) {
-      if (my_tap[tl] < tg_n) {
-        float* dst = a.dW + (((long)blockIdx.x * a.ntaps + tap0 + my_tap[tl]) * a.Ca + a0) * a.Cb + b0;
+      if (my_tap[tl] < tg_w) {
+        float* dst = a.dW + (((long)blockIdx.x * (a.ntaps + (PAIR ? 1 : 0)) + tap0 + my_tap[tl]) * a.Ca + a0) * a.Cb + b0;
 #pragma unroll
         for (int ta = 0; ta < TA16; ++ta)
 #pragma unroll
@@ -291,6 +306,19 @@
       if (maxg <= 4) hipLaunchKernelGGL((wgrad2_kernel<T, 4, 4, true, 4, false, 8>), grid, block, lds, s, a);
       else hipLaunchKernelGGL((wgrad2_kernel<T, 4, 4, true, 8, false, 8>), grid, block, lds, s, a);
       return check_launch("wgrad2");
+    }
+    if (a.nw == 10) {
+      if constexpr (sizeof(T) == 2) {
+        if (ta16 != 4 || tb16 != 2 || a.P_planar || !a.P2 || a.ntaps != 9 || !a.partial || maxg > 4) { set_error("wgrad2: no pair form of this tile"); return MMVAE_ERR_UNSUPPORTED; }
+        static bool attr_set = false;
+        if (!attr_set) {
+          if (hipFuncSetAttribute(reinterpret_cast<const void*>(&wgrad2_kernel<T, 4, 2, true, 4, false, 10, true>), hipFuncAttributeMaxDynamicSharedMemorySize, 96 * 1024) != hipSuccess) {
+            set_error("wgrad2: hipFuncSetAttribute"); return MMVAE_ERR_HIP; }
+          attr_set = true;
+        }
+        hipLaunchKernelGGL((wgrad2_kernel<T, 4, 2, true, 4, false, 10, true>), grid, block, lds, s, a);
+        return check_launch("wgrad2");
+      } else { set_error("wgrad2: the pair form is bf16 only"); return MMVAE_ERR_UNSUPPORTED; }
     }
     if (a.P_planar || !ts || maxg > 8 || (a.nw != 9 && a.nw != 16)) { set_error("wgrad2: nw=%d unsupported here", a.nw); return MMVAE_ERR_UNSUPPORTED; }
 #define MMVAE_W2N(A_, B_) do { \
diff --git a/moving-mnist-vae_amd/csrc/conv_wpos.hip b/moving-mnist-vae_amd/csrc/conv_wpos.hip
--- a/moving-mnist-vae_amd/csrc/conv_wpos.hip
+++ b/moving-mnist-vae_amd/csrc/conv_wpos.hip
@@ -15,9 +15,10 @@
   int N, Ca, Cb, HS, HL, K, S, Pd;
   int nsplit, imgs_per_split;
   int nb, prow, grow;
+  const void* P2;
 };
 
-template <int KI, int NTHR, int kMaxV, int NFB>
+template <int KI, int NTHR, int kMaxV, int NFB, bool PAIR = false>
 __global__ __launch_bounds__(NTHR, 1) void wgrad_pos_kernel(WposArgs a) {
   extern __shared__ __attribute__((aligned(16))) char smem[];
   constexpr int nthr = NTHR;
@@ -26,26 +27,30 @@
   const int npos = a.HS * a.HS, npix = a.HL * a.HL;
   const int nPb = a.prow * a.HS, nGb = a.grow * a.HL;
   const int ipP = ((nPb * 128 + 191) & ~255) + 64, ipG = ((nGb * PXG + 191) & ~255) + 64;
-  const int stageB = KI * (ipP + ipG);
+  const int stageB = KI * (ipP * (PAIR ? 2 : 1) + ipG);
   const int tiles_b = a.Cb / TB;
   const int a0 = (blockIdx.y / tiles_b) << 6, b0 = (blockIdx.y % tiles_b) * TB;
   const int n_begin = blockIdx.x * a.imgs_per_split;
   const int n_end = min(a.N, n_begin + a.imgs_per_split);
   const bf16_t* __restrict__ Pp = reinterpret_cast<const bf16_t*>(a.P);
   const bf16_t* __restrict__ Gp = reinterpret_cast<const bf16_t*>(a.G);
-  const int kh = wv / a.K, kw = wv - kh * a.K;
+  const bool second = PAIR && wv == a.K * a.K;
+  const int tapw = second ? a.Pd * a.K + a.Pd : wv;
+  const int kh = tapw / a.K, kw = tapw - kh * a.K;
   auto win0 = [&](int band) {
     int g = band * a.prow * a.S - a.Pd;
     g = g < 0 ? 0 : g;
     return g > a.HL - a.grow ? a.HL - a.grow : g;
   };
 
-  const int slots = nPb * 8 + nGb * VG;
+  const int slots = nPb * 8 * (PAIR ? 2 : 1) + nGb * VG;
   const int ipr = nthr / slots;
   const bool active = t < ipr * slots;
   const int img_r = t / slots, rem = t - img_r * slots;
-  const bool isP = rem < nPb * 8;
-  const int px = isP ? rem >> 3 : (rem - nPb * 8) / VG, cg = isP ? rem & 7 : (rem - nPb * 8) % VG;
+  const bool isP2 = PAIR && rem >= nPb * 8 + nGb * VG;
+  const int remP = isP2 ? rem - nPb * 8 - nGb * VG : rem;
+  const bool isP = isP2 || rem < nPb * 8;
+  const int px = isP ? remP >> 3 : (rem - nPb * 8) / VG, cg = isP ? remP & 7 : (rem - nPb * 8) % VG;
   const bool pro = isP ? a.proP_scale != nullptr : a.proG_scale != nullptr;
   float* sPro = reinterpret_cast<float*>(smem + 2 * stageB);
   if (t < 128) {
@@ -57,9 +62,9 @@
   }
   const float lo = (isP ? a.proP_relu : a.proG_relu) ? 0.f : -__builtin_inff();
   const long istride = isP ? (long)npos * a.Ca : (long)npix * a.Cb;
-  const bf16_t* src0 = isP ? Pp + (long)px * a.Ca + a0 + cg * 8 : Gp + (long)px * a.Cb + b0 + cg * 8;
+  const bf16_t* src0 = isP ? (isP2 ? reinterpret_cast<const bf16_t*>(a.P2) : Pp) + (long)px * a.Ca + a0 + cg * 8 : Gp + (long)px * a.Cb + b0 + cg * 8;
   const int ip_t = isP ? ipP : ipG;
-  const int dst0 = (isP ? 0 : KI * ipP) + img_r * ip_t + px * (isP ? 128 : PXG) + cg * 16;
+  const int dst0 = (isP2 ? KI * (ipP + ipG) : isP ? 0 : KI * ipP) + img_r * ip_t + px * (isP ? 128 : PXG) + cg * 16;
   Vec16 q[kMaxV];
   auto fetch = [&](int n0, int band) {
     const long boff = isP ? (long)band * nPb * a.Ca : (long)win0(band) * a.HL * a.Cb;
@@ -110,8 +115,8 @@
     if (bn == a.nb) { bn = 0; nn = n0 + KI; }
     const bool more = st + 1 < nstage;
     if (more) fetch(nn, bn);
-    const char* sP = smem + cur * stageB;
-    const char* sG = sP + KI * ipP;
+    const char* sG = smem + cur * stageB + KI * ipP;
+    const char* sP = second ? sG + KI * ipG : sG - KI * ipP;
     const int g0 = win0(band);
     for (int hr = 0; hr < a.prow; ++hr) {
       const int hs = band * a.prow + hr;
@@ -151,7 +156,7 @@
     __syncthreads();
     cur ^= 1; band = bn; n0 = nn;
   }
-  const int ntaps = a.K * a.K;
+  const int ntaps = a.K * a.K + (PAIR ? 1 : 0);
   float* out = a.part + (((long)blockIdx.x * ntaps + wv) * a.Ca + a0) * a.Cb + b0;
 #pragma unroll
   for (int i = 0; i < 2; ++i)
@@ -164,7 +169,9 @@
       }
 }
 
-int try_wgrad_pos(int dt, const WgradArgs& a, hipStream_t s) {
+static int wgrad_pos_run(int dt, const WgradArgs& a, const void* P2, float* dW2, float scale2, hipStream_t s) {
+  const int pair = P2 ? 1 : 0;
+  if (pair && (!dW2 || a.ksz != 3 || a.stride != 2 || a.pad != 1 || a.proP_scale || 2 * a.Hp != a.Hg)) return 0;
   if (dt != DT_BF16 || a.P_planar || !a.scratch || (a.proP_scale && a.proG_scale)) return 0;
   if (a.Hp != a.Wp || a.Hg != a.Wg || a.Hp < 1 || a.Hp > 4 || a.Hg > 8 || a.Ca % 64 != 0 || a.Cb % 32 != 0) return 0;
   if (a.ksz < 1 || a.ksz > 4 || a.ntaps != a.ksz * a.ksz || a.ksz * a.ksz < 4) return 0;
@@ -172,7 +179,7 @@
   for (int t = 0; t < a.ntaps; ++t) if (a.tap_off[t] != t) return 0;
   const int npos = a.Hp * a.Hp, npix = a.Hg * a.Hg;
   if (npos + npix < 8) return 0;
-  const int nthr = 64 * a.ntaps;
+  const int nthr = 64 * (a.ntaps + pair);
   const int nfb = (a.Cb % 64 == 0 && (a.Ca / 64) * (a.Cb / 64) >= 8) ? 2 : 1;
   const int TB = 32 * nfb, VG = TB / 8;
   const int tiles = (a.Ca / 64) * (a.Cb / TB);
@@ -185,11 +192,11 @@
     int gr = (pr - 1) * a.stride + a.ksz; if (gr > a.Hg) gr = a.Hg;
     const int nPb = pr * a.Hp, nGb = gr * a.Hg;
     const int ipP = ((nPb * 128 + 191) & ~255) + 64, ipG = ((nGb * TB * 2 + 191) & ~255) + 64;
-    const int slots = nPb * 8 + nGb * VG;
+    const int slots = nPb * 8 * (1 + pair) + nGb * VG;
     const int ipr = nthr / slots;
     if (ipr < 1) continue;
     for (int ki = (cand == 1 && npos + npix <= 8) ? 32 : 16; ki >= 16; ki -= 16) {
-      const size_t sb = (size_t)ki * (ipP + ipG);
+      const size_t sb = (size_t)ki * (ipP * (1 + pair) + ipG);
       const int rd = (ki + ipr - 1) / ipr;
       if (2 * sb + 512 <= 160 * 1024 && rd <= maxv) { KI = ki; nb = cand; prow = pr; grow = gr; stageB = sb; rounds = rd; break; }
     }
@@ -200,8 +207,8 @@
   b.proP_scale = a.proP_scale; b.proP_shift = a.proP_shift; b.proP_relu = a.proP_relu;
   b.proG_scale = a.proG_scale; b.proG_shift = a.proG_shift; b.proG_relu = a.proG_relu;
   b.N = a.N; b.Ca = a.Ca; b.Cb = a.Cb; b.HS = a.Hp; b.HL = a.Hg; b.K = a.ksz; b.S = a.stride; b.Pd = a.pad;
-  b.nb = nb; b.prow = prow; b.grow = grow;
-  const long wsize = (long)a.Ca * a.Cb * a.ntaps;
+  b.nb = nb; b.prow = prow; b.grow = grow; b.P2 = P2;
+  const long wsize = (long)a.Ca * a.Cb * (a.ntaps + pair);
   int nsplit = (256 + tiles - 1) / tiles;
   const int max_split = wsize * 4 * 64 <= (32L << 20) ? 64 : 32;
   if (nsplit > max_split) nsplit = max_split;
@@ -216,17 +223,19 @@
   const size_t lds = 2 * stageB + 512;
   dim3 grid(nsplit, tiles), block(nthr);
   bool launched = false;
+  if (pair) note_launch_bytes((double)a.N * 2.0 * ((double)npos * 2 * a.Ca + (double)npix * a.Cb));
 #define MMVAE_WPOS(KI_, NT_, MV_, NF_) \
   if (!launched && KI == KI_ && nthr == NT_ && nfb == NF_ && (MV_ == 8 || rounds <= 4)) { \
     static bool attr_set = false; \
     if (!attr_set) { \
-      if (hipFuncSetAttribute(reinterpret_cast<const void*>(&wgrad_pos_kernel<KI_, NT_, MV_, NF_>), hipFuncAttributeMaxDynamicSharedMemorySize, 160 * 1024) != hipSuccess) { \
+      if (hipFuncSetAttribute(reinterpret_cast<const void*>(&wgrad_pos_kernel<KI_, NT_, MV_, NF_, (NT_ == 640)>), hipFuncAttributeMaxDynamicSharedMemorySize, 160 * 1024) != hipSuccess) { \
         set_error("wgrad_pos: hipFuncSetAttribute"); return MMVAE_ERR_HIP; } \
       attr_set = true; } \
-    hipLaunchKernelGGL((wgrad_pos_kernel<KI_, NT_, MV_, NF_>), grid, block, lds, s, b); launched = true; }
+    hipLaunchKernelGGL((wgrad_pos_kernel<KI_, NT_, MV_, NF_, (NT_ == 640)>), grid, block, lds, s, b); launched = true; }
   MMVAE_WPOS(32, 256, 8, 2) MMVAE_WPOS(32, 576, 4, 2) MMVAE_WPOS(32, 576, 8, 2) MMVAE_WPOS(32, 1024, 4, 2)
   MMVAE_WPOS(16, 256, 8, 2) MMVAE_WPOS(16, 576, 4, 2) MMVAE_WPOS(16, 576, 8, 2) MMVAE_WPOS(16, 1024, 4, 2)
   MMVAE_WPOS(16, 256, 8, 1) MMVAE_WPOS(16, 576, 4, 1) MMVAE_WPOS(16, 576, 8, 1) MMVAE_WPOS(16, 1024, 4, 1)
+  MMVAE_WPOS(16, 640, 8, 2) MMVAE_WPOS(16, 640, 8, 1)
 #undef MMVAE_WPOS
   if (!launched) return 0;
   const int rc = check_launch("wgrad_pos");
@@ -235,8 +244,15 @@
   u.part = a.scratch; u.dW = a.dW; u.Ca = a.Ca; u.Cb = a.Cb; u.ntaps = a.ntaps; u.nparts = nsplit;
   u.Ca_valid = a.Ca; u.Cb_valid = a.Cb; u.sA = a.sA; u.sB = a.sB; u.scale = a.scale;
   for (int t = 0; t < 25; ++t) u.tap_off[t] = a.tap_off[t];
+  if (pair) { u.dW2 = dW2; u.sA2 = a.Cb; u.sB2 = 1; u.scale2 = scale2; }
   const int rr = launch_wgrad_reduce(u, s);
   return rr < 0 ? rr : 1;
 }
 
-}
+int try_wgrad_pos(int dt, const WgradArgs& a, hipStream_t s) { return wgrad_pos_run(dt, a, nullptr, nullptr, 1.f, s); }
+int try_wgrad_pos_pair(int dt, const WgradArgs& a, const void* P2, float* dW2, float scale2, hipStream_t s) {
+  if (!P2 || !dW2) return 0;
+  return wgrad_pos_run(dt, a, P2, dW2, scale2, s);
+}
+
+}
diff --git a/moving-mnist-vae_amd/csrc/conv_wstream.hip b/moving-mnist-vae_amd/csrc/conv_wstream.hip
--- a/moving-mnist-vae_amd/csrc/conv_wstream.hip
+++ b/moving-mnist-vae_amd/csrc/conv_wstream.hip
@@ -535,12 +535,8 @@
   u.Ca_valid = a.Ca_valid; u.Cb_valid = a.Cb_valid; u.sA = a.sA; u.sB = a.sB; u.scale = a.scale;
   u.part_stride = (long)(a.ntaps + 1) * a.Ca * a.Cb;
   for (int t = 0; t < 25; ++t) u.tap_off[t] = a.tap_off[t];
-  int rc2 = launch_wgrad_reduce(u, s);
-  if (rc2 < 0) return rc2;
-  WgradReduceArgs v; memset(&v, 0, sizeof(v));
-  v.part = a.scratch + (long)a.ntaps * a.Ca * a.Cb; v.part_stride = u.part_stride; v.dW = dW2; v.Ca = a.Ca; v.Cb = a.Cb; v.ntaps = 1; v.nparts = gx;
-  v.Ca_valid = a.Ca; v.Cb_valid = a.Cb; v.sA = a.Cb; v.sB = 1; v.scale = scale2;
-  rc2 = launch_wgrad_reduce(v, s);
+  u.dW2 = dW2; u.sA2 = a.Cb; u.sB2 = 1; u.scale2 = scale2;
+  const int rc2 = launch_wgrad_reduce(u, s);
   return rc2 < 0 ? rc2 : 1;
 }
 
diff --git a/moving-mnist-vae_amd/csrc/kernels.hpp b/moving-mnist-vae_amd/csrc/kernels.hpp
--- a/moving-mnist-vae_amd/csrc/kernels.hpp
+++ b/moving-mnist-vae_amd/csrc/kernels.hpp
@@ -48,7 +48,9 @@
   struct WgradReduceArgs* defer;
 };
 int launch_wgrad(int dt, WgradArgs a, hipStream_t s);
+int try_wgrad2_pair(int dt, const WgradArgs& a, const void* P2, float* dW2, float scale2, hipStream_t s);
 int try_wgrad_pos(int dt, const WgradArgs& a, hipStream_t s);
+int try_wgrad_pos_pair(int dt, const WgradArgs& a, const void* P2, float* dW2, float scale2, hipStream_t s);
 bool wgrad_stream_shape(int dt, const WgradArgs& a);
 int try_wgrad_stream(int dt, const WgradArgs& a, hipStream_t s);
 int try_wgrad_stream_pair(int dt, const WgradArgs& a, const void* P2, float* dW2, float scale2, hipStream_t s);
@@ -92,6 +94,7 @@
   int P_planar, P_planes;
   int nw;
   int partial;
+  const void* P2;
 };
 size_t wgrad2_lds_bytes(const Wgrad2Args& a, int dt, int TA, int TB);
 int wgrad2_patch_slots(const Wgrad2Args& a, int dt, int TB);
@@ -100,7 +103,8 @@
 size_t gather3_lds_bytes(const GatherArgs& a, int dt, int CT);
 int launch_gather3(int dt, int out_dt, const GatherArgs& a, int gx, hipStream_t s);
 struct WgradReduceArgs { const float* part; float* dW; int Ca, Cb, ntaps, nparts, Ca_valid, Cb_valid, sA, sB; int tap_off[25]; float scale; int exclusive;
-                         long part_stride;  };
+                         long part_stride;
+                         float* dW2; int sA2, sB2; float scale2; };
 int launch_wgrad_reduce(WgradReduceArgs a, hipStream_t s);
 constexpr size_t kWgradScratchBytes = 64u << 20;
 struct PatchPhase { int ph, pw, Hq, Wq, ntaps, tap0; long w_off; int w_vec0, koff0; };
diff --git a/moving-mnist-vae_amd/csrc/vae_net.cpp b/moving-mnist-vae_amd/csrc/vae_net.cpp
--- a/moving-mnist-vae_amd/csrc/vae_net.cpp
+++ b/moving-mnist-vae_amd/csrc/vae_net.cpp
@@ -296,8 +296,10 @@
 }
 
 static bool wgrad_pair_ok(int dt, const ConvGeom& g, const ConvGeom& gs, int Hout, int Hin) {
-  return dt == DT_BF16 && g.k == 3 && g.s == 2 && g.p == 1 && gs.k == 1 && gs.s == 2 && gs.p == 0 && g.D0 == 32 && g.D1 == 32 && gs.D0 == 32 &&
-         gs.D1 == 32 && Hout == 16 && Hin == 32;
+  if (dt != DT_BF16 || g.k != 3 || g.s != 2 || g.p != 1 || gs.k != 1 || gs.s != 2 || gs.p != 0 || gs.D0 != g.D0 || gs.D1 != g.D1 || 2 * Hout != Hin)
+    return false;
+  return (g.D1 == 32 && g.D0 == 32 && Hin == 32) || (g.D1 == 32 && g.D0 == 64 && Hin == 16) || (g.D1 == 64 && g.D0 == 128 && Hin == 8) ||
+         (g.D1 == 128 && g.D0 == 256 && Hin == 4);
 }
 
 bool Net::l1_dgrad_stream() const {
```

Measured after the change: 856,100 frames/s, median of 6. About the same (+0.8%).
